# AnthonyDickson/HIVE

Measured on AMD Instinct MI355X. Metric: frames/sec (depth+TSDF integrate) @640x480, 512^3 vol, higher is better.
Workload: dtype bf16; 1 GPU; synthetic 640x480x150 RGB (seeded room trajectory), host-resident uint8 frames uploaded in the timed region, DPT-Hybrid depth (seeded random weights: depth 1-7 m, bf16, hip engine) + 512x512x512 TSDF integrate, 107 frames/step; frames_total=4066, volume=512x512x512, tsdf_overlap=True, scaling_mode=weak

## Files before the change

### hive_amd/_lib.py

```python
import atexit
import ctypes
import os
import sys
import threading

import numpy as np

_HERE = os.path.dirname(os.path.abspath(__file__))
LIB_PATH = os.environ.get("HIVE_AMD_LIB") or os.path.join(_HERE, "lib", "libhive_mi355x.so")

OK, ERR_INVALID, ERR_DEVICE, ERR_NOMEM, ERR_EMPTY, ERR_STATE = 0, -1, -2, -3, -4, -5
MEM_HOST, MEM_DEVICE = 0, 1
ROUND_HALF_EVEN, ROUND_HALF_AWAY = 0, 1
F32, F16, BF16 = 0, 1, 2
ABI_VERSION = 2

c_void_p, c_int, c_int64, c_float, c_double = ctypes.c_void_p, ctypes.c_int, ctypes.c_int64, ctypes.c_float, ctypes.c_double
P = ctypes.POINTER

SIGNATURES = {
    "hive_abi_version": (c_int, []),
    "hive_ctx_create": (c_int, [c_int, c_void_p, P(c_void_p)]),
    "hive_ctx_destroy": (c_int, [c_void_p]),
    "hive_ctx_get_stream": (c_int, [c_void_p, P(c_void_p)]),
# ... 40 lines not shown
    "hive_view_frustum": (c_int, [c_void_p, c_void_p, c_int, c_int, c_void_p, c_void_p, c_int, c_void_p]),
    "hive_view_frustum_batch": (c_int, [c_void_p, c_void_p, c_int, c_int, c_int, c_void_p, c_void_p, c_int, c_void_p]),
    "hive_depth_apply_mask": (c_int, [c_void_p, c_void_p, c_void_p, c_int, c_int, c_int, c_int, c_int, c_int, c_void_p]),
    "hive_depth_mm_to_m": (c_int, [c_void_p, c_void_p, c_int64, c_float, c_float, c_void_p]),
    "hive_unproject": (c_int, [c_void_p, c_void_p, c_void_p, c_void_p, c_int, c_int, c_void_p, c_void_p, c_void_p, c_int,
                               c_void_p, c_void_p, c_int64, P(c_int64)]),
    "hive_image2world": (c_int, [c_void_p, c_void_p, c_void_p, c_int64, c_void_p, c_void_p, c_void_p, c_double, c_int, c_void_p]),
    "hive_project": (c_int, [c_void_p, c_void_p, c_int64, c_void_p, c_void_p, c_void_p, c_double, c_int, c_void_p, c_void_p,
                             c_void_p]),
    "hive_project_bbox": (c_int, [c_void_p, c_void_p, c_int64, c_void_p, c_void_p, c_void_p, c_int, c_int, c_int, c_void_p]),
    "hive_grid_mesh": (c_int, [c_void_p, c_void_p, c_void_p, c_int, c_int, c_double, c_double, c_int, c_void_p, c_int64, P(c_int64), P(c_int64)]),
    "hive_fg_frame_mesh": (c_int, [c_void_p, c_void_p, c_void_p, c_int, c_int, c_void_p, c_void_p, c_void_p, c_void_p, c_double, c_double, c_void_p, c_int64, c_void_p, c_int64,
                                   c_void_p, P(c_int64), P(c_int64), c_void_p]),
    "hive_mesh_cleanup_cc": (c_int, [c_void_p, c_void_p, c_int64, c_int64, c_int, c_double, c_int, c_void_p, c_void_p, P(c_int64), P(c_int64)]),
    "hive_fg_frame_mesh_cc": (c_int, [c_void_p, c_void_p, c_void_p, c_int, c_int, c_void_p, c_void_p, c_void_p, c_void_p, c_double, c_double, c_int, c_double, c_void_p,
                                      c_int64, c_void_p, c_int64, c_void_p, P(c_int64), P(c_int64), c_void_p, c_void_p]),
    "hive_mesh_decimate": (c_int, [c_void_p, c_void_p, c_int64, c_void_p, c_int64, c_int64, c_double, c_int, c_void_p, c_void_p, P(c_int64), P(c_int64), c_void_p]),
    "hive_fg_frame_mesh_dec": (c_int, [c_void_p, c_void_p, c_void_p, c_int, c_int, c_void_p, c_void_p, c_void_p, c_void_p, c_double, c_double, c_int64, c_double, c_int,
                                       c_int, c_double, c_void_p, c_int64, c_void_p, c_int64, c_void_p, P(c_int64), P(c_int64), c_void_p, c_void_p, c_void_p, c_void_p]),
    "hive_filter_faces": (c_int, [c_void_p, c_void_p, c_void_p, c_int64, c_void_p, c_int64, c_double, c_double, c_int, c_void_p, P(c_int64)]),
    "hive_texture_window": (c_int, [c_void_p, c_void_p, c_int64, c_void_p, c_void_p, c_void_p, c_double, c_int, c_void_p, c_void_p]),
    "hive_fg_billboard": (c_int, [c_void_p, c_void_p, c_int64, c_void_p, c_void_p, P(c_double)]),
    "hive_fg_centroids": (c_int, [c_void_p, c_void_p, c_void_p, c_int, c_int, c_int, c_void_p, c_void_p, c_void_p]),
    "hive_fts_optimise": (c_int, [c_void_p, c_void_p, c_void_p, c_void_p, c_int, c_void_p, c_void_p, c_int, c_double, c_int, c_void_p, c_void_p]),
    "hive_dilate_mask": (c_int, [c_void_p, c_void_p, c_int, c_int, c_int, c_int, c_void_p]),
    "hive_dilate_mask_se": (c_int, [c_void_p, c_void_p, c_int, c_int, c_void_p, c_int, c_int, c_int, c_int, c_void_p]),
    "hive_inpaint_telea": (c_int, [c_void_p, c_void_p, c_int, c_int, c_int, c_int, c_void_p, c_int, c_int, c_void_p]),
    "hive_inpaint_frames": (c_int, [c_void_p, c_void_p, c_void_p, c_void_p, c_int, c_int, c_int, c_int, c_int, c_int, c_int, c_void_p, c_void_p, c_void_p]),
    "hive_depth_apply_mask_se": (c_int, [c_void_p, c_void_p, c_void_p, c_int, c_int, c_int, c_void_p, c_int, c_int, c_int, c_int, c_int, c_void_p]),
    "hive_vit_create": (c_int, [c_void_p, c_int, c_int, c_int, c_int, c_int, c_float, c_void_p, P(c_void_p)]),
    "hive_vit_weights_modified": (c_int, [c_void_p]),
    "hive_vit_destroy": (c_int, [c_void_p]),
    "hive_vit_forward": (c_int, [c_void_p, c_void_p, c_int, c_int, c_void_p, c_int, c_void_p]),
    "hive_vit_layernorm": (c_int, [c_void_p, c_void_p, c_int, c_void_p, c_void_p, c_void_p, c_int, c_int, c_float]),
    "hive_vit_linear": (c_int, [c_void_p, c_void_p, c_int, c_void_p, c_void_p, c_void_p, c_void_p, c_int, c_int, c_int, c_int]),
    "hive_vit_qkv": (c_int, [c_void_p, c_void_p, c_int, c_void_p, c_void_p, c_void_p, c_void_p, c_int, c_int, c_int, c_int]),
    "hive_vit_attention": (c_int, [c_void_p, c_void_p, c_int, c_void_p, c_void_p, c_int, c_int, c_int, c_int, c_int]),
    "hive_dpt_preprocess": (c_int, [c_void_p, c_void_p, c_int64, c_float, c_float, c_int, c_void_p]),
    "hive_dpt_head_tail": (c_int, [c_void_p, c_void_p, c_int, c_int64, c_int, c_void_p, c_int, c_void_p, c_float, c_int, c_int, c_float,
                                   c_float, c_void_p, c_float, c_float, c_void_p, c_void_p]),
    "hive_dpt_head_fused": (c_int, [c_void_p, c_void_p, c_void_p, c_int, c_int, c_int, c_int, c_int, c_int, c_void_p, c_void_p, c_void_p, c_float,
                                    c_int, c_int, c_float, c_float, c_void_p, c_float, c_float, c_void_p, c_void_p]),
    "hive_nhwc_group_norm": (c_int, [c_void_p, c_void_p, c_int, c_int, c_int, c_int, c_int, c_void_p, c_void_p, c_float, c_void_p, c_int,
                                     c_void_p]),
    "hive_nhwc_bias_act": (c_int, [c_void_p, c_void_p, c_int, c_int64, c_int, c_void_p, c_int, c_void_p, c_void_p, c_void_p, c_void_p]),
    "hive_nhwc_upsample2x": (c_int, [c_void_p, c_void_p, c_void_p, c_int, c_int, c_int, c_int, c_int, c_void_p]),
    "hive_nhwc_conv3x3": (c_int, [c_void_p, c_void_p, c_int, c_int, c_int, c_int, c_int, c_int, c_void_p, c_void_p, c_int, c_void_p, c_void_p,
                                  c_void_p, c_void_p]),
    "hive_nhwc_conv": (c_int, [c_void_p, c_void_p, c_int, c_int, c_int, c_int, c_int, c_int, c_int, c_int, c_int, c_int, c_int, c_int, c_void_p, c_void_p,
                               c_int, c_void_p, c_void_p, c_void_p, c_void_p]),
    "hive_nhwc_conv_gn_partial_floats": (c_int64, [c_int64, c_int]),
    "hive_nhwc_conv_gn": (c_int, [c_void_p, c_void_p, c_int, c_int, c_int, c_int, c_int, c_int, c_int, c_int, c_int, c_int, c_int, c_int, c_void_p, c_void_p,
                                  c_int, c_void_p, c_void_p, c_void_p, c_void_p, c_void_p, c_int64, P(c_int)]),
    "hive_nhwc_conv_gn_apply": (c_int, [c_void_p, c_void_p, c_int, c_int, c_int, c_int, c_int, c_int, c_int, c_int, c_int, c_int, c_int, c_int, c_void_p, c_int,
                                        c_void_p, c_void_p, c_float, c_void_p, c_int, c_void_p, c_void_p, c_int64, P(c_int)]),
    "hive_nhwc_group_norm_stats": (c_int, [c_void_p, c_void_p, c_int, c_int, c_int, c_int, c_int, c_void_p, c_void_p, c_float, c_void_p, c_int,
                                           c_void_p, c_void_p, c_int]),
    "hive_gn_gram_table_floats": (c_int64, [c_int, c_int]),
    "hive_gn_gram_prepare": (c_int, [c_void_p, c_void_p, c_int, c_int, c_int, c_int, c_void_p]),
    "hive_gn_gram_parts": (c_int, [c_void_p, c_int, c_int, c_int, c_int]),
    "hive_gn_gram_stats": (c_int, [c_void_p, c_void_p, c_int, c_int, c_int, c_int, c_int, c_int, c_int, c_int, c_int, c_int, c_void_p, c_float, c_void_p, c_void_p,
                                   c_void_p]),
    "hive_nhwc_conv_gn_apply_gram": (c_int, [c_void_p, c_void_p, c_int, c_int, c_int, c_int, c_int, c_int, c_int, c_int, c_int, c_void_p, c_void_p, c_int, c_void_p,
                                             c_void_p, c_float, c_void_p, c_int, c_void_p, c_void_p, c_int64, P(c_int)]),
    "hive_patch_rows": (c_int, [c_void_p, c_void_p, c_int, c_int, c_int, c_int, c_int, c_int, c_void_p]),
    "hive_nhwc_pixel_shuffle_bias": (c_int, [c_void_p, c_void_p, c_void_p, c_int, c_int, c_int, c_int, c_int, c_int, c_void_p]),
    "hive_resnet_stem_conv": (c_int, [c_void_p, c_void_p, c_int, c_int, c_int, c_int, c_void_p, c_void_p]),
    "hive_nhwc_maxpool3x3s2": (c_int, [c_void_p, c_void_p, c_int, c_int, c_int, c_int, c_int, c_void_p]),
    "hive_bneck_gn_conv3x3": (c_int, [c_void_p, c_void_p, c_int, c_int, c_int, c_int, c_int, c_void_p, c_int, c_void_p, c_void_p, c_float, c_void_p, c_void_p, c_void_p,
                                      c_int64, P(c_int), P(c_int)]),
    "hive_resnet_stem_conv_gn": (c_int, [c_void_p, c_void_p, c_int, c_int, c_int, c_int, c_void_p, c_void_p, c_void_p, c_int64, P(c_int)]),
    "hive_nhwc_group_norm_relu_maxpool": (c_int, [c_void_p, c_void_p, c_int, c_int, c_int, c_int, c_int, c_int, c_void_p, c_void_p, c_float, c_void_p, c_void_p,
                                                  c_int]),
    "hive_dpt_create": (c_int, [c_void_p, c_void_p, c_void_p, c_int, P(c_void_p)]),
    "hive_dpt_forward": (c_int, [c_void_p, c_void_p, c_int, c_int, c_int, c_void_p, c_void_p, c_float, c_void_p, c_void_p]),
    "hive_dpt_forward_frames": (c_int, [c_void_p, c_void_p, c_int, c_int, c_int, c_int, c_int, c_void_p, c_void_p, c_float, c_void_p, c_void_p]),
    "hive_dpt_resize_preprocess": (c_int, [c_void_p, c_void_p, c_int, c_int, c_int, c_int, c_int, c_float, c_float, c_int, c_void_p]),
    "hive_depth_resize_nearest": (c_int, [c_void_p, c_void_p, c_int, c_int, c_int, c_int, c_int, c_float, c_float, c_void_p, c_void_p, c_void_p]),
    "hive_dpt_arena_bytes": (c_int, [c_void_p, P(c_int64)]),
    "hive_dpt_weights_modified": (c_int, [c_void_p]),
    "hive_dpt_destroy": (c_int, [c_void_p]),
    "hive_depth_quantize": (c_int, [c_void_p, c_void_p, c_int, c_int, c_int, c_float, c_float, c_void_p, c_void_p, c_void_p]),
}

_lib = None
_lock = threading.Lock()
_shutdown = False


@atexit.register
def _mark_shutdown():
    global _shutdown
    _shutdown = True


def alive():
    return not _shutdown and not sys.is_finalizing()


class HiveError(RuntimeError):
    def __init__(self, code, message):
        super().__init__(f"libhive_mi355x error {code}: {message}")
        self.code = code


def load():
    global _lib
    with _lock:
        if _lib is not None:
            return _lib
        if not os.path.exists(LIB_PATH):
            raise ImportError(
                f"{LIB_PATH} is missing: build it with `python -c 'import __graft_entry__ as g; g.build()'` or "
                f"`make -C hive_amd/csrc`. hive_amd has no CPU fallback.")
        try:
            import torch
        except ImportError:
            pass
        lib = ctypes.CDLL(LIB_PATH, mode=ctypes.RTLD_GLOBAL)
        for name, (restype, argtypes) in SIGNATURES.items():
            fn = getattr(lib, name)
            fn.restype = restype
            fn.argtypes = argtypes
        if lib.hive_abi_version() != ABI_VERSION:
# ... 132 lines not shown
```

### hive_amd/csrc/bneck.hip

```cpp
#include "hive_internal.hpp"

#include <algorithm>

#include "mfma_pipe.hpp"

using hive_mfma::f32x4;
using hive_mfma::vec;

namespace {

constexpr int BN_TH = 16, BN_TW = 32;
constexpr int BN_PH = BN_TH + 2, BN_PW = BN_TW + 2;
constexpr int BN_K = 9 * 64;
constexpr int BN_WP = BN_K + 16;
constexpr int BN_CHUNKS = BN_PH * BN_PW * 8;
constexpr int BN_LOADS = (BN_CHUNKS + 511) / 512;
constexpr int BN_PATCH_BYTES = BN_PH * BN_PW * 128, BN_W_BYTES = 64 * BN_WP * 2, BN_SUM_BYTES = 8 * 2 * 64 * 4;
constexpr int BN_LDS = BN_PATCH_BYTES + BN_W_BYTES + BN_SUM_BYTES;

template <typename T>
struct BneckParams {
    const T *x;
    const float *stats;
    const T *gamma, *beta;
    const T *w;
    T *out;
    float *gn_partial;
    int H, W, tiles_x, tiles_y, n_tiles;
};

__device__ __forceinline__ int bn_swz(int q, int c) { return q * 128 + ((c ^ (q & 6)) << 4); }

__device__ __forceinline__ float bn_dot2(vec<__bf16, 2> a, vec<__bf16, 2> b, float c) { return __builtin_amdgcn_fdot2_f32_bf16(a, b, c, false); }
__device__ __forceinline__ float bn_dot2(vec<_Float16, 2> a, vec<_Float16, 2> b, float c) { return __builtin_amdgcn_fdot2(a, b, c, false); }
using hive_mfma::dpp_row_total;

template <typename T>
__global__ __launch_bounds__(512, 2) void bneck_conv3x3_kernel(BneckParams<T> p) {
    extern __shared__ __attribute__((aligned(16))) unsigned char lds[];
    unsigned char *patch = lds;
    T *wl = reinterpret_cast<T *>(lds + BN_PATCH_BYTES);
    float(*wsum)[2][64] = reinterpret_cast<float(*)[2][64]>(lds + BN_PATCH_BYTES + BN_W_BYTES);
    for (int i = threadIdx.x; i < 64 * (BN_K / 8); i += 512) {
        const int row = i / (BN_K / 8), c8 = i - row * (BN_K / 8);
        const int nt = row >> 4, f4 = (row >> 2) & 3, e = row & 3;
        const int ch = (nt >> 1) * 32 + f4 * 8 + (nt & 1) * 4 + e;
        *reinterpret_cast<uint4 *>(wl + row * BN_WP + c8 * 8) = reinterpret_cast<const uint4 *>(p.w)[ch * (BN_K / 8) + c8];
    }
    const int per_img = p.tiles_x * p.tiles_y;
    const int my_c = threadIdx.x & 7;
    float gam[8], bet[8];
    {
        const vec<T, 8> gv = *reinterpret_cast<const vec<T, 8> *>(p.gamma + my_c * 8), bv = *reinterpret_cast<const vec<T, 8> *>(p.beta + my_c * 8);
#pragma unroll
        for (int e = 0; e < 8; ++e) gam[e] = (float)gv[e], bet[e] = (float)bv[e];
    }
    uint4 regs[BN_LOADS];
    auto tile_origin = [&](int tile, int &img, int &oy0, int &ox0) {
        img = tile / per_img;
        const int t = tile - img * per_img;
        oy0 = (t / p.tiles_x) * BN_TH;
        ox0 = (t % p.tiles_x) * BN_TW;
    };
    auto fetch = [&](int tile) {
        int tid = threadIdx.x;
        asm volatile("" : "+v"(tid));
        int img, oy0, ox0;
        tile_origin(tile, img, oy0, ox0);
        const T *src = p.x + (size_t)img * p.H * p.W * 64;
#pragma unroll
        for (int k = 0; k < BN_LOADS; ++k) {
            const int i = tid + 512 * k, q = i >> 3, pr = q / BN_PW, pc = q - pr * BN_PW;
            const int gy = oy0 - 1 + pr, gx = ox0 - 1 + pc;
            regs[k] = make_uint4(0u, 0u, 0u, 0u);
            if (i < BN_CHUNKS && (unsigned)gy < (unsigned)p.H && (unsigned)gx < (unsigned)p.W)
                regs[k] = *reinterpret_cast<const uint4 *>(src + ((size_t)gy * p.W + gx) * 64 + (i & 7) * 8);
        }
    };
    int tile = blockIdx.x;
    if (tile < p.n_tiles) fetch(tile);
    for (; tile < p.n_tiles; tile += gridDim.x) {
// ... 49 lines not shown
#pragma unroll
                    for (int nt = 0; nt < 4; ++nt) acc[nt][mt] = hive_mfma::mfma16(wf[nt], af[mt], acc[nt][mt]);
            }
        }
        T *out = p.out + (size_t)img * p.H * p.W * 64;
#pragma unroll
        for (int mt = 0; mt < 4; ++mt) {
            const int oy = oy0 + 2 * wave + (mt >> 1), ox = ox0 + 16 * (mt & 1) + fr;
            if (oy < p.H && ox < p.W) {
#pragma unroll
                for (int h = 0; h < 2; ++h) {
                    vec<T, 8> ov;
#pragma unroll
                    for (int j = 0; j < 4; ++j) ov[j] = (T)acc[2 * h][mt][j], ov[4 + j] = (T)acc[2 * h + 1][mt][j];
                    *reinterpret_cast<vec<T, 8> *>(out + ((size_t)oy * p.W + ox) * 64 + h * 32 + fq * 8) = ov;
                }
            }
        }
        if (p.gn_partial) {
            vec<T, 2> ones, zero2;
            ones[0] = ones[1] = (T)1.0f;
            zero2[0] = zero2[1] = (T)0.0f;
            const bool row_ok[2] = {oy0 + 2 * wave < p.H, oy0 + 2 * wave + 1 < p.H};
#pragma unroll
            for (int nt = 0; nt < 4; ++nt) {
                f32x4 sv = f32x4{0.f, 0.f, 0.f, 0.f}, qv = sv;
#pragma unroll
                for (int r = 0; r < 2; ++r)
#pragma unroll
                    for (int e = 0; e < 4; ++e) {
                        vec<T, 2> y;
                        y[0] = (T)acc[nt][2 * r][e], y[1] = (T)acc[nt][2 * r + 1][e];
                        if (!row_ok[r]) y = zero2;
                        sv[e] = bn_dot2(y, ones, sv[e]);
                        qv[e] = bn_dot2(y, y, qv[e]);
                    }
#pragma unroll
                for (int e = 0; e < 4; ++e) {
                    sv[e] = dpp_row_total(sv[e]);
                    qv[e] = dpp_row_total(qv[e]);
                }
                if (fr == 0) {
                    const int ch = (nt >> 1) * 32 + fq * 8 + (nt & 1) * 4;
                    *reinterpret_cast<f32x4 *>(&wsum[wave][0][ch]) = sv;
                    *reinterpret_cast<f32x4 *>(&wsum[wave][1][ch]) = qv;
                }
            }
            __syncthreads();
            if (tix < 128) {
                const int which = tix >> 6, c = tix & 63;
                float s = 0.f;
#pragma unroll
                for (int w = 0; w < 8; ++w) s += wsum[w][which][c];
                p.gn_partial[((size_t)tile * 4 + which) * 64 + c] = s;
                p.gn_partial[((size_t)tile * 4 + 2 + which) * 64 + c] = 0.f;
            }
        }
    }
}

template <typename T>
int launch_bneck(hive_ctx *ctx, const void *d_x, int N, int H, int W, const float *stats, const void *gamma, const void *beta, const void *d_w, void *d_out,
                 float *d_gn_partial, long long gn_partial_floats, int *gn_tile_rows) {
    static hive_device_latch latch;
    if (!latch.done(ctx)) {
        HIVE_CHECK_HIP(ctx, hipFuncSetAttribute((const void *)bneck_conv3x3_kernel<T>, hipFuncAttributeMaxDynamicSharedMemorySize, BN_LDS));
        latch.mark(ctx);
    }
    BneckParams<T> p{};
    p.x = (const T *)d_x;
    p.stats = stats;
    p.gamma = (const T *)gamma;
    p.beta = (const T *)beta;
    p.w = (const T *)d_w;
    p.out = (T *)d_out;
    p.H = H;
    p.W = W;
    p.tiles_x = (W + BN_TW - 1) / BN_TW;
    p.tiles_y = (H + BN_TH - 1) / BN_TH;
    const long long tiles = (long long)N * p.tiles_x * p.tiles_y;
    HIVE_REQUIRE(ctx, tiles < (1ll << 31), "bneck_conv3x3: %lld tiles", tiles);
    p.n_tiles = (int)tiles;
    const int per_img = p.tiles_x * p.tiles_y;
    if (d_gn_partial && gn_tile_rows && W % BN_TW == 0 && (H * W) % per_img == 0 && tiles * 4 * 64 <= gn_partial_floats) {
        p.gn_partial = d_gn_partial;
        *gn_tile_rows = H * W / per_img;
    }
    const unsigned grid = (unsigned)std::min<long long>(tiles, (long long)ctx->num_cus);
    hipLaunchKernelGGL(bneck_conv3x3_kernel<T>, dim3(grid), dim3(512), BN_LDS, ctx->stream, p);
    HIVE_CHECK_HIP(ctx, hipGetLastError());
    return HIVE_OK;
}

}

extern "C" int hive_bneck_gn_conv3x3(hive_ctx *ctx, const void *d_x, int dtype, int N, int H, int W, int C, const void *d_in_partial, int in_tile_rows,
                                     const void *d_gamma, const void *d_beta, float eps, const void *d_w, void *d_out, void *d_gn_partial,
                                     int64_t gn_partial_floats, int *gn_tile_rows, int *fused) {
    HIVE_ENTER(ctx);
    if (!ctx) return hive_fail(nullptr, HIVE_ERR_INVALID, "ctx is NULL");
    HIVE_REQUIRE(ctx, d_x && d_gamma && d_beta && d_w && d_out && fused && d_out != d_x, "bneck_gn_conv3x3: bad pointers");
    HIVE_REQUIRE(ctx, dtype == HIVE_BF16 || dtype == HIVE_F16, "bneck_gn_conv3x3: dtype must be HIVE_F16 or HIVE_BF16");
    HIVE_REQUIRE(ctx, N > 0 && H > 0 && W > 0 && (long long)N * H * W < (1ll << 31), "bneck_gn_conv3x3: bad sizes %d x %d x %d", N, H, W);
    *fused = 0;
    if (gn_tile_rows) *gn_tile_rows = 0;
    if (C != 64 || !d_in_partial || in_tile_rows <= 0 || in_tile_rows > H * W) return HIVE_OK;
    int rc = hive_reserve_device(ctx, &ctx->d_scratch, &ctx->scratch_bytes, (size_t)N * 32 * 2 * sizeof(float));
    if (rc) return rc;
    float *stats = (float *)ctx->d_scratch;
    if ((rc = hive_gn_finalize_tiles(ctx, (const float *)d_in_partial, N, H * W, 64, 32, in_tile_rows, eps, stats))) return rc;
    rc = dtype == HIVE_BF16 ? launch_bneck<__bf16>(ctx, d_x, N, H, W, stats, d_gamma, d_beta, d_w, d_out, (float *)d_gn_partial, gn_partial_floats, gn_tile_rows)
                            : launch_bneck<_Float16>(ctx, d_x, N, H, W, stats, d_gamma, d_beta, d_w, d_out, (float *)d_gn_partial, gn_partial_floats, gn_tile_rows);
    if (rc) return rc;
    *fused = 1;
    return HIVE_OK;
}
```

### hive_amd/csrc/capi.hip

```cpp
#include <algorithm>

#include "hive_internal.hpp"

static thread_local std::string g_global_error;

void hive_set_global_error(const char *msg) { g_global_error = msg ? msg : ""; }

int hive_fail(hive_ctx *ctx, int code, const char *fmt, ...) {
    char buf[1024];
    va_list ap;
    va_start(ap, fmt);
    vsnprintf(buf, sizeof(buf), fmt, ap);
    va_end(ap);
    if (ctx)
        ctx->last_error = buf;
    else
        g_global_error = buf;
    return code;
}

int hive_reserve_device(hive_ctx *ctx, void **ptr, size_t *cur, size_t bytes) {
    if (*cur >= bytes && *ptr) return HIVE_OK;
    if (*ptr) {
        HIVE_CHECK_HIP(ctx, hipStreamSynchronize(ctx->stream));
        HIVE_CHECK_HIP(ctx, hipFree(*ptr));
        *ptr = nullptr;
        *cur = 0;
    }
    HIVE_CHECK_HIP(ctx, hipMalloc(ptr, bytes));
    *cur = bytes;
    return HIVE_OK;
}

int hive_splitk_workspace(hive_ctx *ctx, size_t bytes, void **ws, unsigned **count) {
    if (!ctx->d_splitk_count) {
        HIVE_CHECK_HIP(ctx, hipMalloc((void **)&ctx->d_splitk_count, HIVE_SPLITK_TILES * sizeof(unsigned)));
        HIVE_CHECK_HIP(ctx, hipMemsetAsync(ctx->d_splitk_count, 0, HIVE_SPLITK_TILES * sizeof(unsigned), ctx->stream));
    }
    int rc = hive_reserve_device(ctx, &ctx->d_splitk, &ctx->splitk_bytes, std::max(bytes, (size_t)32 << 20));
    if (rc) return rc;
    *ws = ctx->d_splitk;
    *count = ctx->d_splitk_count;
    return HIVE_OK;
}

int hive_upload(hive_ctx *ctx, void *dst, const void *src, size_t bytes) {
    hive_staging_slot &s = ctx->slots[ctx->next_slot];
    ctx->next_slot = (ctx->next_slot + 1) % hive_ctx::kSlots;
    if (s.in_flight) {
        HIVE_CHECK_HIP(ctx, hipEventSynchronize(s.done));
        s.in_flight = false;
    }
    if (s.bytes < bytes) {
        if (s.pinned) HIVE_CHECK_HIP(ctx, hipHostFree(s.pinned));
        s.pinned = nullptr;
        s.bytes = 0;
        HIVE_CHECK_HIP(ctx, hipHostMalloc(&s.pinned, bytes, hipHostMallocDefault));
        s.bytes = bytes;
    }
    if (!s.done) HIVE_CHECK_HIP(ctx, hipEventCreateWithFlags(&s.done, hipEventDisableTiming));
    memcpy(s.pinned, src, bytes);
    HIVE_CHECK_HIP(ctx, hipMemcpyAsync(dst, s.pinned, bytes, hipMemcpyHostToDevice, ctx->stream));
    HIVE_CHECK_HIP(ctx, hipEventRecord(s.done, ctx->stream));
    s.in_flight = true;
    return HIVE_OK;
}

static int next_event(hive_ctx *ctx, hipEvent_t *ev) {
    if (ctx->ev_used == ctx->ev_pool.size()) {
        hipEvent_t e;
        HIVE_CHECK_HIP(ctx, hipEventCreate(&e));
        ctx->ev_pool.push_back(e);
    }
    *ev = ctx->ev_pool[ctx->ev_used++];
    return HIVE_OK;
}

int hive_time_begin(hive_ctx *ctx) {
    if (!ctx->timing) return HIVE_OK;
    int rc = next_event(ctx, &ctx->last_start);
    if (rc) return rc;
    HIVE_CHECK_HIP(ctx, hipEventRecord(ctx->last_start, ctx->stream));
    return HIVE_OK;
}

int hive_time_end(hive_ctx *ctx) {
    if (!ctx->timing) return HIVE_OK;
    int rc = next_event(ctx, &ctx->last_stop);
    if (rc) return rc;
    HIVE_CHECK_HIP(ctx, hipEventRecord(ctx->last_stop, ctx->stream));
    return HIVE_OK;
}

extern "C" {

// ... 15 lines not shown
    if (e != hipSuccess) return hive_fail(nullptr, HIVE_ERR_DEVICE, "hipGetDeviceProperties: %s", hipGetErrorString(e));
    if (strncmp(prop.gcnArchName, "gfx950", 6) != 0)
        return hive_fail(nullptr, HIVE_ERR_DEVICE, "hive_ctx_create: device %d is %s; this library is built for gfx950 only",
                         device_id, prop.gcnArchName);
    hive_ctx *ctx = new hive_ctx();
    ctx->device = device_id;
    ctx->num_cus = prop.multiProcessorCount > 0 ? prop.multiProcessorCount : 256;
    HIVE_ENTER(ctx);
    int current = -1;
    e = hipGetDevice(&current);
    if (e == hipSuccess && current != device_id) e = hipErrorInvalidDevice;
    if (e == hipSuccess) {
        if (stream == HIVE_STREAM_OWN) {
            e = hipStreamCreateWithFlags(&ctx->stream, hipStreamNonBlocking);
            ctx->owns_stream = true;
        } else if (stream == HIVE_STREAM_OWN_LOW) {
            int least = 0, greatest = 0;
            e = hipDeviceGetStreamPriorityRange(&least, &greatest);
            if (e == hipSuccess) e = hipStreamCreateWithPriority(&ctx->stream, hipStreamNonBlocking, least);
            ctx->owns_stream = true;
        } else {
            ctx->stream = (hipStream_t)stream;
        }
    }
    if (e == hipSuccess) e = hipMalloc((void **)&ctx->d_scalars, 4096 * sizeof(unsigned));
    if (e == hipSuccess) e = hipMemset(ctx->d_scalars, 0, 4096 * sizeof(unsigned));
    if (e == hipSuccess) e = hipMalloc(&ctx->d_zeros, 256);
    if (e == hipSuccess) e = hipMemset(ctx->d_zeros, 0, 256);
    if (e != hipSuccess) {
        int rc = hive_fail(nullptr, HIVE_ERR_DEVICE, "hive_ctx_create: %s", hipGetErrorString(e));
        delete ctx;
        return rc;
    }
    *out = ctx;
    return HIVE_OK;
}

int hive_ctx_destroy(hive_ctx *ctx) {
    if (!ctx) return HIVE_OK;
    {
        HIVE_ENTER(ctx);
        (void)hipStreamSynchronize(ctx->stream);
    for (auto &s : ctx->slots) {
        if (s.pinned) (void)hipHostFree(s.pinned);
        if (s.done) (void)hipEventDestroy(s.done);
    }
    for (auto ev : ctx->ev_pool) (void)hipEventDestroy(ev);
    if (ctx->d_scratch) (void)hipFree(ctx->d_scratch);
    if (ctx->d_frame) (void)hipFree(ctx->d_frame);
    if (ctx->d_batch) (void)hipFree(ctx->d_batch);
    if (ctx->d_gram) (void)hipFree(ctx->d_gram);
    if (ctx->d_splitk) (void)hipFree(ctx->d_splitk);
    if (ctx->d_splitk_count) (void)hipFree(ctx->d_splitk_count);
    if (ctx->d_in) (void)hipFree(ctx->d_in);
    if (ctx->d_scalars) (void)hipFree(ctx->d_scalars);
    if (ctx->h_pinned_small) (void)hipHostFree(ctx->h_pinned_small);
        if (ctx->d_zeros) (void)hipFree(ctx->d_zeros);
        if (ctx->owns_stream) (void)hipStreamDestroy(ctx->stream);
    }
    delete ctx;
    return HIVE_OK;
}

int hive_ctx_release_stream(hive_ctx *ctx) {
    if (!ctx) return hive_fail(nullptr, HIVE_ERR_INVALID, "ctx is NULL");
    ctx->owns_stream = false;
    return HIVE_OK;
}

int hive_ctx_set_stream(hive_ctx *ctx, void *stream) {
    HIVE_ENTER(ctx);
    if (!ctx) return hive_fail(nullptr, HIVE_ERR_INVALID, "ctx is NULL");
    HIVE_REQUIRE(ctx, stream != HIVE_STREAM_OWN && stream != HIVE_STREAM_OWN_LOW, "hive_ctx_set_stream: pass a hipStream_t (NULL = the default stream)");
    hipStream_t next = (hipStream_t)stream;
    if (next == ctx->stream) return HIVE_OK;
    hipEvent_t ev;
    HIVE_CHECK_HIP(ctx, hipEventCreateWithFlags(&ev, hipEventDisableTiming));
    hipError_t e = hipEventRecord(ev, ctx->stream);
    if (e == hipSuccess) e = hipStreamWaitEvent(next, ev, 0);
    (void)hipEventDestroy(ev);
    HIVE_CHECK_HIP(ctx, e);
    if (ctx->owns_stream) {
        (void)hipStreamSynchronize(ctx->stream);
        (void)hipStreamDestroy(ctx->stream);
        ctx->owns_stream = false;
    }
    ctx->stream = next;
    return HIVE_OK;
}

int hive_ctx_get_stream(hive_ctx *ctx, void **stream) {
    if (!ctx || !stream) return hive_fail(ctx, HIVE_ERR_INVALID, "hive_ctx_get_stream: NULL argument");
    *stream = (void *)ctx->stream;
    return HIVE_OK;
}

int hive_ctx_synchronize(hive_ctx *ctx) {
    HIVE_ENTER(ctx);
    if (!ctx) return hive_fail(nullptr, HIVE_ERR_INVALID, "ctx is NULL");
    HIVE_CHECK_HIP(ctx, hipStreamSynchronize(ctx->stream));
    return HIVE_OK;
}

const char *hive_last_error(hive_ctx *ctx) { return ctx ? ctx->last_error.c_str() : g_global_error.c_str(); }

int hive_ctx_set_round_mode(hive_ctx *ctx, int mode) {
// ... 59 lines not shown
```

### hive_amd/csrc/conv.hip

```cpp
#include "hive_internal.hpp"
#include "mfma_pipe.hpp"

#include <algorithm>

constexpr int HIVE_CONV_AHEAD = 4;
constexpr int HIVE_CONV_AHEAD_GN2 = 4;

using hive_mfma::f32x4;
using hive_mfma::vec;

namespace {

template <typename T>
struct ConvParams {
    const T *x;
    const T *w;
    const T *bias;
    const T *res1;
    const T *res2;
    T *out;
    T *out_relu;
    const T *zeros;
    int H, W, Cin, Cout, relu;
    int Ho, Wo;
    int S, taps;
    int stride, pad_t, pad_l;
    int M;
    float *gn_partial;
    int stats_only;
    const float *gn_stats;
    const T *gn_gamma, *gn_beta;
    int gn_G, gn_cpg;
    int split_k;
    hive_mfma::f32x4 *sk_ws;
    unsigned *sk_count;
};

__device__ __forceinline__ float gn_affine_exact(float x, float rstd, float gamma, float beta, float mean) {
#pragma clang fp contract(off)
    const float a = rstd * gamma;
    const float b = beta - mean * a;
    return x * a + b;
}

template <typename T, int MT, int GN, int NRES = 1>
__device__ __forceinline__ void conv_epilogue(const ConvParams<T> &p, f32x4 (&acc)[4][MT], int m_base, int n_base, unsigned char *stage, int lane,
                                              int boundary) {
    asm volatile("" : "+v"(lane));
    const int n = n_base + (lane & 7) * 8;
    float b[8] = {0.f, 0.f, 0.f, 0.f, 0.f, 0.f, 0.f, 0.f};
    if (p.bias) {
        const vec<T, 8> bv = *reinterpret_cast<const vec<T, 8> *>(p.bias + n);
#pragma unroll
        for (int j = 0; j < 8; ++j) b[j] = (float)bv[j];
    }
    float ggam[8], gbet[8], gmean[2] = {0.f, 0.f}, grstd[2] = {0.f, 0.f};
    if (GN == 2) {
        const vec<T, 8> gv = *reinterpret_cast<const vec<T, 8> *>(p.gn_gamma + n), bv = *reinterpret_cast<const vec<T, 8> *>(p.gn_beta + n);
#pragma unroll
        for (int j = 0; j < 8; ++j) ggam[j] = (float)gv[j], gbet[j] = (float)bv[j];
        const int hw = p.Ho * p.Wo, img0 = boundary / hw - 1, n_img = p.M / hw, g = n / p.gn_cpg;
        const float *st = p.gn_stats + ((size_t)img0 * p.gn_G + g) * 2;
        gmean[0] = st[0], grstd[0] = st[1];
        if (img0 + 1 < n_img) gmean[1] = st[2 * p.gn_G], grstd[1] = st[2 * p.gn_G + 1];
    }
    constexpr int AHEAD = GN == 2 ? HIVE_CONV_AHEAD_GN2 : (NRES == 2 ? HIVE_CONV_AHEAD / 2 : HIVE_CONV_AHEAD);
    vec<T, 8> rs1[AHEAD + 1][2], rs2[NRES == 2 ? AHEAD + 1 : 1][2];
    const int row_in_frag = lane >> 3;
    auto pre = [&](int mt, int j) {
        const int m = min(m_base + mt * 16 + 8 * j + row_in_frag, p.M - 1);
        const size_t off = (size_t)m * p.Cout + n;
        if (GN != 1 && p.res1) rs1[mt % (AHEAD + 1)][j] = *reinterpret_cast<const vec<T, 8> *>(p.res1 + off);
        if (GN == 0 && NRES == 2) rs2[mt % (AHEAD + 1)][j] = *reinterpret_cast<const vec<T, 8> *>(p.res2 + off);
    };
    hive_mfma::staged_rows<MT, AHEAD>(stage, acc, lane, pre, [&](int r, int, const f32x4 &lo, const f32x4 &hi, int mt, int jrow) {
        const int m = m_base + r;
        if (m >= p.M) return;
        const size_t o_off = (size_t)m * p.Cout + n;
        float o[8];
#pragma unroll
        for (int j = 0; j < 4; ++j) o[j] = lo[j] + b[j], o[4 + j] = hi[j] + b[4 + j];
        if (GN == 0 && p.res1) {
            const vec<T, 8> rs = rs1[mt % (AHEAD + 1)][jrow];
#pragma unroll
            for (int j = 0; j < 8; ++j) o[j] += (float)rs[j];
        }
        if (GN == 0 && NRES == 2) {
            const vec<T, 8> rs = rs2[mt % (AHEAD + 1)][jrow];
// ... 63 lines not shown
#pragma unroll
            for (int mt = 0; mt < MT; mt += 2) {
                const f32x4 a0 = acc[nt][mt] + bias, a1 = acc[nt][mt + 1] + bias;
#pragma unroll
                for (int e = 0; e < 4; ++e) {
                    vec<T, 2> y;
                    y[0] = (T)a0[e], y[1] = (T)a1[e];
                    ts[e] = dot2acc(y, ones, ts[e]);
                    tq[e] = dot2acc(y, y, tq[e]);
                }
            }
            const f32x4 zero4 = f32x4{0.f, 0.f, 0.f, 0.f};
            sv[0] = second ? zero4 : ts;
            sv[1] = second ? ts : zero4;
            qv[0] = second ? zero4 : tq;
            qv[1] = second ? tq : zero4;
        } else {
#pragma unroll
            for (int mt = 0; mt < MT; mt += 2) {
                const int m0 = m_base + mt * 16 + fr, m1 = m0 + 16;
                const bool v0 = m0 < p.M, v1 = m1 < p.M, s0 = m0 >= boundary, s1 = m1 >= boundary;
                const f32x4 a0 = acc[nt][mt] + bias, a1 = acc[nt][mt + 1] + bias;
#pragma unroll
                for (int e = 0; e < 4; ++e) {
                    vec<T, 2> y, z;
                    y[0] = (T)(v0 && !s0 ? a0[e] : 0.f), y[1] = (T)(v1 && !s1 ? a1[e] : 0.f);
                    z[0] = (T)(v0 && s0 ? a0[e] : 0.f), z[1] = (T)(v1 && s1 ? a1[e] : 0.f);
                    sv[0][e] = dot2acc(y, ones, sv[0][e]);
                    qv[0][e] = dot2acc(y, y, qv[0][e]);
                    sv[1][e] = dot2acc(z, ones, sv[1][e]);
                    qv[1][e] = dot2acc(z, z, qv[1][e]);
                }
            }
        }
#pragma unroll
        for (int h = 0; h < 2; ++h) {
            f32x4 st = f32x4{0.f, 0.f, 0.f, 0.f}, qt = f32x4{0.f, 0.f, 0.f, 0.f};
            if (h == 0 || m_end > boundary) {
#pragma unroll
                for (int e = 0; e < 4; ++e) {
                    st[e] = dpp_row_total(sv[h][e]);
                    qt[e] = dpp_row_total(qv[h][e]);
                }
            }
            if (fr == 0) {
                *reinterpret_cast<f32x4 *>(wsum + (h * 2 + 0) * 64 + nt * 16 + fq * 4) = st;
                *reinterpret_cast<f32x4 *>(wsum + (h * 2 + 1) * 64 + nt * 16 + fq * 4) = qt;
            }
        }
    }
}

constexpr int BK = 64;


template <typename T, int TM, int TN, int GN>
__global__ __launch_bounds__(512, 1) void conv_kernel(ConvParams<T> p) {
    extern __shared__ __attribute__((aligned(16))) unsigned char lds[];
    constexpr int A_GROUPS = TM / 8, A_PW = A_GROUPS / 8;
    constexpr int W_GROUPS = TN / 8, GROUPS = A_GROUPS + W_GROUPS, PER_WAVE = GROUPS / 8;
    constexpr int STAGE_BYTES = GROUPS * 1024;
    constexpr int WN = TN / 64, WM = 8 / WN, RW = TM / WM, MT = RW / 16;
    const int tid = threadIdx.x;
    int lane = tid & 63;
    const int wave = __builtin_amdgcn_readfirstlane(tid >> 6);
    const int wr = wave / WN, wc = wave % WN;
    const int tiles_n = p.Cout / TN, n_tiles = ((p.M + TM - 1) / TM) * tiles_n;
    int run0, run_n, per_xcd;
    hive_mfma::xcd_run(n_tiles, run0, run_n, per_xcd);
    int tl = blockIdx.x >> 3;
    if (tl >= run_n) return;
    const int K = p.taps * p.Cin, CPT = p.Cin / BK;

    struct Tile {
        int m0, n0;
        int py[A_PW], px[A_PW];
        const T *pbase[A_PW];
    };
    int a_chunk[A_PW];
    auto lane_constants = [&]() {
#pragma unroll
        for (int j = 0; j < A_PW; ++j) {
            const int row = (wave + 8 * j) * 8 + (lane >> 3);
            a_chunk[j] = ((lane & 7) ^ ((row >> 1) & 7)) * 8;
        }
    };
    lane_constants();
    auto setup = [&](int t, Tile &tile) {
        tile.m0 = (t / tiles_n) * TM;
        tile.n0 = (t % tiles_n) * TN;
#pragma unroll
        for (int j = 0; j < A_PW; ++j) {
            const int row = (wave + 8 * j) * 8 + (lane >> 3);
            const int m = min(tile.m0 + row, p.M - 1);
            const int img = m / (p.Ho * p.Wo), rem = m - img * (p.Ho * p.Wo);
            const int oy = rem / p.Wo, ox = rem - oy * p.Wo;
            tile.py[j] = oy * p.stride - p.pad_t;
            tile.px[j] = ox * p.stride - p.pad_l;
            tile.pbase[j] = p.x + (((long long)img * p.H + tile.py[j]) * p.W + tile.px[j]) * p.Cin + a_chunk[j];
        }
    };

    auto issue_piece = [&](const Tile &tile, int stage, int tap, int cc, int j) {
        unsigned char *st = lds + stage * STAGE_BYTES;
        if (j < A_PW) {
            const int dy = tap / p.S, dx = tap - dy * p.S;
// ... 14 lines not shown
    Tile tile;
    setup(run0 + tl, tile);
#pragma unroll
    for (int j = 0; j < PER_WAVE; ++j) issue_piece(tile, 0, 0, 0, j);
    int buf = 0;
    for (;;) {
        asm volatile("" : "+v"(lane));
        lane_constants();
        const int fr = lane & 15, fq = lane >> 4;
        const bool has_next = tl + per_xcd < run_n;
        const int em0 = tile.m0, en0 = tile.n0;
        f32x4 acc[4][MT];
#pragma unroll
        for (int i = 0; i < 4; ++i)
#pragma unroll
            for (int j = 0; j < MT; ++j) acc[i][j] = f32x4{0.f, 0.f, 0.f, 0.f};
        int nx_tap = 1, nx_cc = 0;
        if (nx_tap == p.taps) nx_tap = 0, nx_cc = 1;
        for (int kt = 0; kt < KT; ++kt) {
            asm volatile("s_waitcnt vmcnt(0)" ::: "memory");
            __builtin_amdgcn_s_barrier();
            int is_tap = nx_tap, is_cc = nx_cc;
            if (kt + 1 == KT) {
                if (has_next) {
                    setup(run0 + tl + per_xcd, tile);
                    is_tap = 0, is_cc = 0;
                } else {
                    is_tap = last_tap, is_cc = CPT - 1;
                }
            }
            if (++nx_tap == p.taps) nx_tap = 0, ++nx_cc;
            const unsigned char *a_t = lds + buf * STAGE_BYTES, *w_t = a_t + A_GROUPS * 1024;
            hive_mfma::kstep64<T, MT, false>(a_t, w_t, wr * RW, wc * 64, fr, fq, acc, PER_WAVE, [&](int j) { issue_piece(tile, buf ^ 1, is_tap, is_cc, j); });
            buf ^= 1;
        }
        unsigned char *stage = lds + 2 * STAGE_BYTES + wave * 4096;
        const int hw = p.Ho * p.Wo, boundary = (em0 / hw + 1) * hw;
        if (!(GN == 1 && p.stats_only)) {
            if (GN == 0 && p.res2)
                conv_epilogue<T, MT, GN, 2>(p, acc, em0 + wr * RW, en0 + wc * 64, stage, lane, boundary);
            else
                conv_epilogue<T, MT, GN, 1>(p, acc, em0 + wr * RW, en0 + wc * 64, stage, lane, boundary);
        }
        if (GN == 1) {
            __builtin_amdgcn_wave_barrier();
            gn_sums_from_acc<T, MT>(p, acc, em0 + wr * RW, en0 + wc * 64, lane, boundary, reinterpret_cast<float *>(stage));
            __syncthreads();
            const int tile_m = em0 / TM;
            for (int t = tid; t < 4 * TN; t += 512) {
                const int hq = t / TN, ch = t - hq * TN, cw = ch >> 6, c = ch & 63;
                float a = 0.f;
#pragma unroll
                for (int w = 0; w < WM; ++w) a += reinterpret_cast<const float *>(lds + 2 * STAGE_BYTES + (w * WN + cw) * 4096)[hq * 64 + c];
                p.gn_partial[((size_t)tile_m * 4 + hq) * p.Cout + en0 + ch] = a;
            }
        }
        if (!has_next) break;
        tl += per_xcd;
    }
    asm volatile("s_waitcnt vmcnt(0)" ::: "memory");
}

template <typename T, int TN, int GN, int NST>
__global__ __launch_bounds__(512, 1) void conv_deep_kernel(ConvParams<T> p) {
    extern __shared__ __attribute__((aligned(16))) unsigned char lds[];
    constexpr int TM = 128, AHEAD = NST - 1;
    constexpr int A_GROUPS = TM / 8, A_PW = A_GROUPS / 8;
    constexpr int W_GROUPS = TN / 8, GROUPS = A_GROUPS + W_GROUPS, PER_WAVE = GROUPS / 8;
    constexpr int STAGE_BYTES = GROUPS * 1024;
    constexpr int WN = TN / 64, WM = 8 / WN, RW = TM / WM, MT = RW / 16;
    static_assert(AHEAD * PER_WAVE < 64, "vmcnt is a 6-bit counter");
    const int tid = threadIdx.x;
    int lane = tid & 63;
    const int wave = __builtin_amdgcn_readfirstlane(tid >> 6);
    const int wr = wave / WN, wc = wave % WN;
    const int S = p.split_k, KT = p.taps * (p.Cin / BK);
    const int tiles_n = p.Cout / TN, n_items = ((p.M + TM - 1) / TM) * tiles_n * S;
    int run0, run_n, per_xcd;
    hive_mfma::xcd_run(n_items, run0, run_n, per_xcd);
    int tl = blockIdx.x >> 3;
    if (tl >= run_n) return;

    struct Tile {
        int m0, n0, kt, k1, tl;
        int py[A_PW], px[A_PW];
        const T *pbase[A_PW];
    };
    int a_chunk[A_PW];
    auto lane_constants = [&]() {
#pragma unroll
        for (int j = 0; j < A_PW; ++j) {
            const int row = (wave + 8 * j) * 8 + (lane >> 3);
            a_chunk[j] = ((lane & 7) ^ ((row >> 1) & 7)) * 8;
        }
    };
    lane_constants();
    auto coords = [&](int item, int &m0, int &n0, int &k0, int &k1) {
        const int t = item / S, s = item - t * S;
        m0 = (t / tiles_n) * TM;
        n0 = (t % tiles_n) * TN;
        k0 = s * KT / S;
        k1 = (s + 1) * KT / S;
    };
    auto setup = [&](Tile &tile) {
        coords(run0 + tile.tl, tile.m0, tile.n0, tile.kt, tile.k1);
#pragma unroll
        for (int j = 0; j < A_PW; ++j) {
            const int row = (wave + 8 * j) * 8 + (lane >> 3);
            const int m = min(tile.m0 + row, p.M - 1);
            const int img = m / (p.Ho * p.Wo), rem = m - img * (p.Ho * p.Wo);
            const int oy = rem / p.Wo, ox = rem - oy * p.Wo;
            tile.py[j] = oy * p.stride - p.pad_t;
            tile.px[j] = ox * p.stride - p.pad_l;
// ... 28 lines not shown
    Tile is;
    is.tl = tl;
    setup(is);
#pragma unroll
    for (int a = 0; a < AHEAD; ++a) {
#pragma unroll
        for (int j = 0; j < PER_WAVE; ++j) issue_piece(is, a, j);
        advance(is);
    }
    int buf = 0;
    for (;;) {
        asm volatile("" : "+v"(lane));
        lane_constants();
        const int fr = lane & 15, fq = lane >> 4;
        const bool has_next = tl + per_xcd < run_n;
        int em0, en0, k0, k1;
        coords(run0 + tl, em0, en0, k0, k1);
        f32x4 acc[4][MT];
#pragma unroll
        for (int i = 0; i < 4; ++i)
#pragma unroll
            for (int j = 0; j < MT; ++j) acc[i][j] = f32x4{0.f, 0.f, 0.f, 0.f};
        for (int kt = k0; kt < k1; ++kt) {
            asm volatile("s_waitcnt vmcnt(%0)" ::"n"((AHEAD - 1) * PER_WAVE) : "memory");
            __builtin_amdgcn_s_barrier();
            const int ib = buf + AHEAD >= NST ? buf + AHEAD - NST : buf + AHEAD;
            const unsigned char *a_t = lds + buf * STAGE_BYTES, *w_t = a_t + A_GROUPS * 1024;
            hive_mfma::kstep64<T, MT, false>(a_t, w_t, wr * RW, wc * 64, fr, fq, acc, PER_WAVE, [&](int j) { issue_piece(is, ib, j); });
            advance(is);
            buf = buf + 1 == NST ? 0 : buf + 1;
        }
        unsigned char *epi = lds + NST * STAGE_BYTES;
        bool store = true;
        if (S > 1) store = hive_mfma::splitk_combine<512>(S, p.sk_ws, p.sk_count, run0 + tl, acc, tid, reinterpret_cast<int *>(epi));
        if (store) {
            unsigned char *stage = epi + wave * 4096;
            const int hw = p.Ho * p.Wo, boundary = (em0 / hw + 1) * hw;
            if (!(GN == 1 && p.stats_only)) {
                if (GN == 0 && p.res2)
                    conv_epilogue<T, MT, GN, 2>(p, acc, em0 + wr * RW, en0 + wc * 64, stage, lane, boundary);
                else
                    conv_epilogue<T, MT, GN, 1>(p, acc, em0 + wr * RW, en0 + wc * 64, stage, lane, boundary);
            }
            if (GN == 1) {
                __builtin_amdgcn_wave_barrier();
                gn_sums_from_acc<T, MT>(p, acc, em0 + wr * RW, en0 + wc * 64, lane, boundary, reinterpret_cast<float *>(stage));
                __syncthreads();
                const int tile_m = em0 / TM;
                for (int t = tid; t < 4 * TN; t += 512) {
                    const int hq = t / TN, ch = t - hq * TN, cw = ch >> 6, c = ch & 63;
                    float a = 0.f;
#pragma unroll
                    for (int w = 0; w < WM; ++w) a += reinterpret_cast<const float *>(epi + (w * WN + cw) * 4096)[hq * 64 + c];
                    p.gn_partial[((size_t)tile_m * 4 + hq) * p.Cout + en0 + ch] = a;
                }
            }
        }
        if (!has_next) break;
        __builtin_amdgcn_s_waitcnt(0x0F70);
        __syncthreads();
        tl += per_xcd;
    }
    asm volatile("s_waitcnt vmcnt(0)" ::: "memory");
}

constexpr int conv_lds(int tm, int tn, int nst = 2) { return nst * (tm / 8 + tn / 8) * 1024 + hive_mfma::STAGED_ROWS_LDS; }

constexpr int CONV_DEEP_NST = 4;

template <typename T>
int ensure_conv_attrs(hive_ctx *ctx) {
    static hive_device_latch latch;
    if (latch.done(ctx)) return HIVE_OK;
#define HIVE_CONV_ATTR(TM_, TN_, GN_) \
    HIVE_CHECK_HIP(ctx, hipFuncSetAttribute((const void *)conv_kernel<T, TM_, TN_, GN_>, hipFuncAttributeMaxDynamicSharedMemorySize, conv_lds(TM_, TN_)))
    HIVE_CONV_ATTR(256, 256, 0);
    HIVE_CONV_ATTR(256, 256, 1);
    HIVE_CONV_ATTR(256, 128, 0);
    HIVE_CONV_ATTR(256, 128, 1);
    HIVE_CONV_ATTR(256, 64, 0);
    HIVE_CONV_ATTR(256, 64, 1);
    HIVE_CONV_ATTR(128, 256, 0);
    HIVE_CONV_ATTR(128, 256, 1);
    HIVE_CONV_ATTR(128, 128, 0);
    HIVE_CONV_ATTR(128, 128, 1);
    HIVE_CONV_ATTR(256, 256, 2);
    HIVE_CONV_ATTR(128, 256, 2);
#undef HIVE_CONV_ATTR
    HIVE_CHECK_HIP(ctx, hipFuncSetAttribute((const void *)conv_deep_kernel<T, 128, 0, CONV_DEEP_NST>, hipFuncAttributeMaxDynamicSharedMemorySize, conv_lds(128, 128, CONV_DEEP_NST)));
    HIVE_CHECK_HIP(ctx, hipFuncSetAttribute((const void *)conv_deep_kernel<T, 128, 1, CONV_DEEP_NST>, hipFuncAttributeMaxDynamicSharedMemorySize, conv_lds(128, 128, CONV_DEEP_NST)));
    latch.mark(ctx);
    return HIVE_OK;
}

struct GnMode {
    int stats_only = 0;
    const float *gn_stats = nullptr;
    const void *gn_gamma = nullptr, *gn_beta = nullptr;
    int gn_G = 0, gn_cpg = 0;
};

template <typename T>
int launch_conv_t(hive_ctx *ctx, const char *what, const void *d_x, int N, int H, int W, int C_in, int C_out, int R, int stride, int pad_t,
                  int pad_l, int Ho, int Wo, const void *d_w, const void *d_bias, int relu, const void *d_residual, const void *d_residual2,
                  void *d_out, void *d_out_relu, void *d_gn_partial, long long gn_partial_floats, int *gn_tile_rows, const GnMode *gn_mode) {
    HIVE_REQUIRE(ctx, d_x && d_w && d_out, "%s: NULL argument", what);
    if (gn_tile_rows) *gn_tile_rows = 0;
    HIVE_REQUIRE(ctx, N > 0 && H > 0 && W > 0 && Ho > 0 && Wo > 0 && (long long)N * H * W < (1ll << 31) && (long long)N * Ho * Wo < (1ll << 31),
                 "%s: bad sizes %d x %d x %d -> %d x %d", what, N, H, W, Ho, Wo);
    HIVE_REQUIRE(ctx, (R == 1 || R == 3) && (stride == 1 || stride == 2) && pad_t >= 0 && pad_t < R && pad_l >= 0 && pad_l < R,
                 "%s: kernel %d, stride %d, padding (%d, %d)", what, R, stride, pad_t, pad_l);
    HIVE_REQUIRE(ctx, (long long)(Ho - 1) * stride - pad_t < H && (long long)(Wo - 1) * stride - pad_l < W, "%s: output %d x %d reaches outside the %d x %d input", what, Ho,
                 Wo, H, W);
    HIVE_REQUIRE(ctx, C_in > 0 && C_in % 64 == 0 && C_out > 0 && C_out % 64 == 0, "%s: need C_in %% 64 == 0 and C_out %% 64 == 0, got %d -> %d", what, C_in, C_out);
    HIVE_REQUIRE(ctx, (R == 1 && stride == 1) || (d_out != d_x && d_out_relu != d_x), "%s: the output must not alias the input", what);
    ConvParams<T> p{};
    p.x = (const T *)d_x;
    p.w = (const T *)d_w;
    p.bias = (const T *)d_bias;
    p.res1 = (const T *)d_residual;
    p.res2 = (const T *)d_residual2;
    p.out = (T *)d_out;
    p.out_relu = (T *)d_out_relu;
    p.zeros = (const T *)ctx->d_zeros;
    p.H = H;
    p.W = W;
    p.Cin = C_in;
    p.Cout = C_out;
    p.relu = relu;
    p.Ho = Ho;
    p.Wo = Wo;
    p.S = R;
    p.taps = R * R;
    p.stride = stride;
    p.pad_t = pad_t;
    p.pad_l = pad_l;
    p.M = N * Ho * Wo;
    int rc = ensure_conv_attrs<T>(ctx);
    if (rc) return rc;
    const int tn = C_out % 256 == 0 ? 256 : (C_out % 128 == 0 ? 128 : 64);
    int tm = 256;
    if (tn >= 128) {
        const long long per = C_out / tn, t256 = (long long)((p.M + 255) / 256) * per, t128 = (long long)((p.M + 127) / 128) * per;
        const long long r256 = (t256 + ctx->num_cus - 1) / ctx->num_cus, r128 = (t128 + ctx->num_cus - 1) / ctx->num_cus;
        if (t256 < ctx->num_cus || r128 * 128 * 100 < r256 * 256 * 85) tm = 128;
    }
    if (gn_mode) {
        p.stats_only = gn_mode->stats_only;
        p.gn_stats = gn_mode->gn_stats;
        p.gn_gamma = (const T *)gn_mode->gn_gamma;
        p.gn_beta = (const T *)gn_mode->gn_beta;
        p.gn_G = gn_mode->gn_G;
        p.gn_cpg = gn_mode->gn_cpg;
    }
    if (d_gn_partial && gn_tile_rows && (long long)Ho * Wo >= tm && !relu && !d_residual && !d_residual2 && !d_out_relu) {
        HIVE_REQUIRE(ctx, (long long)((p.M + tm - 1) / tm) * 4 * C_out <= gn_partial_floats, "%s: gn_partial holds %lld floats, %lld needed", what,
                     gn_partial_floats, (long long)((p.M + tm - 1) / tm) * 4 * C_out);
        p.gn_partial = (float *)d_gn_partial;
        *gn_tile_rows = tm;
    }
    {
        const long long tiles128 = (long long)((p.M + 127) / 128) * (C_out / 128);
        const char *deep_env = getenv("HIVE_CONV_DEEP");
        const bool allowed = !(deep_env && deep_env[0] == '0');
        if (allowed && !p.gn_stats && C_out % 128 == 0 && tiles128 <= ctx->num_cus && tiles128 <= HIVE_SPLITK_TILES) {
            const int KT = p.taps * (C_in / BK);
            const char *sk_env = getenv("HIVE_SPLITK");
            p.split_k = sk_env ? std::max(1, std::min(atoi(sk_env), KT)) : hive_mfma::splitk_ways(tiles128, KT, ctx->num_cus);
            p.split_k = (int)std::max<long long>(1, std::min<long long>(p.split_k, ctx->num_cus / tiles128));
            if (ctx->deterministic) p.split_k = 1;
            ++ctx->n_deep_ring_launches;
            if (p.split_k > 1) {
                ++ctx->n_splitk_launches;
                void *ws = nullptr;
                rc = hive_splitk_workspace(ctx, (size_t)tiles128 * p.split_k * 128 * 128 * sizeof(float), &ws, &p.sk_count);
                if (rc) return rc;
                p.sk_ws = reinterpret_cast<hive_mfma::f32x4 *>(ws);
            }
            const bool stats = d_gn_partial && gn_tile_rows && (long long)Ho * Wo >= 128 && !relu && !d_residual && !d_residual2 && !d_out_relu;
            if (stats) {
                HIVE_REQUIRE(ctx, (long long)((p.M + 127) / 128) * 4 * C_out <= gn_partial_floats, "%s: gn_partial holds %lld floats, %lld needed", what,
                             gn_partial_floats, (long long)((p.M + 127) / 128) * 4 * C_out);
                p.gn_partial = (float *)d_gn_partial;
                *gn_tile_rows = 128;
            }
            const long long items = tiles128 * p.split_k;
            const dim3 dgrid((unsigned)std::min<long long>((items + 7) / 8 * 8, (long long)ctx->num_cus / 8 * 8));
            if (stats)
                hipLaunchKernelGGL((conv_deep_kernel<T, 128, 1, CONV_DEEP_NST>), dgrid, dim3(512), (size_t)conv_lds(128, 128, CONV_DEEP_NST), ctx->stream, p);
            else
                hipLaunchKernelGGL((conv_deep_kernel<T, 128, 0, CONV_DEEP_NST>), dgrid, dim3(512), (size_t)conv_lds(128, 128, CONV_DEEP_NST), ctx->stream, p);
            HIVE_CHECK_HIP(ctx, hipGetLastError());
            return HIVE_OK;
        }
    }
    const long long tiles = (long long)((p.M + tm - 1) / tm) * (C_out / tn);
    const dim3 grid((unsigned)std::min<long long>((tiles + 7) / 8 * 8, (long long)ctx->num_cus / 8 * 8));
    const size_t lds = (size_t)conv_lds(tm, tn);
#define HIVE_CONV_LAUNCH(TM_, TN_)                                                                                   \
    do {                                                                                                             \
        if (p.gn_partial)                                                                                            \
            hipLaunchKernelGGL((conv_kernel<T, TM_, TN_, 1>), grid, dim3(512), lds, ctx->stream, p);                    \
        else                                                                                                         \
            hipLaunchKernelGGL((conv_kernel<T, TM_, TN_, 0>), grid, dim3(512), lds, ctx->stream, p);                    \
    } while (0)
    if (p.gn_stats) {
        if (tm == 256)
            hipLaunchKernelGGL((conv_kernel<T, 256, 256, 2>), grid, dim3(512), lds, ctx->stream, p);
        else
            hipLaunchKernelGGL((conv_kernel<T, 128, 256, 2>), grid, dim3(512), lds, ctx->stream, p);
    } else if (tm == 256 && tn == 256)
        HIVE_CONV_LAUNCH(256, 256);
    else if (tm == 256 && tn == 128)
        HIVE_CONV_LAUNCH(256, 128);
    else if (tm == 256)
        HIVE_CONV_LAUNCH(256, 64);
    else if (tn == 256)
        HIVE_CONV_LAUNCH(128, 256);
    else
        HIVE_CONV_LAUNCH(128, 128);
#undef HIVE_CONV_LAUNCH
    HIVE_CHECK_HIP(ctx, hipGetLastError());
    return HIVE_OK;
}

int launch_conv(hive_ctx *ctx, const char *what, const void *d_x, int dtype, int N, int H, int W, int C_in, int C_out, int R, int stride, int pad_t,
                int pad_l, int Ho, int Wo, const void *d_w, const void *d_bias, int relu, const void *d_residual, const void *d_residual2,
                void *d_out, void *d_out_relu, void *d_gn_partial = nullptr, long long gn_partial_floats = 0, int *gn_tile_rows = nullptr,
                const GnMode *gn_mode = nullptr) {
    if (dtype == HIVE_BF16)
        return launch_conv_t<__bf16>(ctx, what, d_x, N, H, W, C_in, C_out, R, stride, pad_t, pad_l, Ho, Wo, d_w, d_bias, relu, d_residual, d_residual2, d_out, d_out_relu,
                                     d_gn_partial, gn_partial_floats, gn_tile_rows, gn_mode);
    if (dtype == HIVE_F16)
        return launch_conv_t<_Float16>(ctx, what, d_x, N, H, W, C_in, C_out, R, stride, pad_t, pad_l, Ho, Wo, d_w, d_bias, relu, d_residual, d_residual2, d_out,
                                       d_out_relu, d_gn_partial, gn_partial_floats, gn_tile_rows, gn_mode);
    if (gn_tile_rows) *gn_tile_rows = 0;
    return hive_fail(ctx, HIVE_ERR_INVALID, "%s: dtype must be HIVE_F16 or HIVE_BF16", what);
}

}

extern "C" int hive_nhwc_conv3x3(hive_ctx *ctx, const void *d_x, int dtype, int N, int H, int W, int C_in, int C_out, const void *d_w,
                                 const void *d_bias, int relu, const void *d_residual, const void *d_residual2, void *d_out,
                                 void *d_out_relu) {
    HIVE_ENTER(ctx);
    if (!ctx) return hive_fail(nullptr, HIVE_ERR_INVALID, "ctx is NULL");
    HIVE_REQUIRE(ctx, C_out % 128 == 0, "nhwc_conv3x3: need C_out %% 128 == 0, got %d", C_out);
    HIVE_REQUIRE(ctx, d_out != d_x && d_out_relu != d_x, "nhwc_conv3x3: the output must not alias the input (3 x 3 halo)");
    return launch_conv(ctx, "nhwc_conv3x3", d_x, dtype, N, H, W, C_in, C_out, 3, 1, 1, 1, H, W, d_w, d_bias, relu, d_residual, d_residual2, d_out, d_out_relu);
}

extern "C" int64_t hive_nhwc_conv_gn_partial_floats(int64_t n_px, int C_out) { return (n_px / 128 + 1) * 4 * (int64_t)C_out; }

extern "C" int hive_nhwc_conv_gn(hive_ctx *ctx, const void *d_x, int dtype, int N, int H, int W, int C_in, int C_out, int kernel, int stride, int pad_top,
                                 int pad_left, int H_out, int W_out, const void *d_w, const void *d_bias, int relu, const void *d_residual,
                                 const void *d_residual2, void *d_out, void *d_out_relu, void *d_gn_partial, int64_t gn_partial_floats, int *gn_tile_rows) {
    HIVE_ENTER(ctx);
    if (!ctx) return hive_fail(nullptr, HIVE_ERR_INVALID, "ctx is NULL");
    HIVE_REQUIRE(ctx, d_gn_partial && gn_tile_rows, "nhwc_conv_gn: NULL argument");
    return launch_conv(ctx, "nhwc_conv_gn", d_x, dtype, N, H, W, C_in, C_out, kernel, stride, pad_top, pad_left, H_out, W_out, d_w, d_bias, relu, d_residual,
                       d_residual2, d_out, d_out_relu, d_gn_partial, gn_partial_floats, gn_tile_rows);
}

extern "C" int hive_nhwc_conv_gn_apply(hive_ctx *ctx, const void *d_x, int dtype, int N, int H, int W, int C_in, int C_out, int kernel, int stride,
                                       int pad_top, int pad_left, int H_out, int W_out, const void *d_w, int G, const void *d_gamma, const void *d_beta,
                                       float eps, const void *d_residual, int relu, void *d_out, void *d_scratch, int64_t scratch_floats, int *fused) {
    HIVE_ENTER(ctx);
    if (!ctx) return hive_fail(nullptr, HIVE_ERR_INVALID, "ctx is NULL");
    HIVE_REQUIRE(ctx, d_gamma && d_beta && d_scratch && fused, "nhwc_conv_gn_apply: NULL argument");
    *fused = 0;
    const long long hw = (long long)H_out * W_out;
    if (G <= 0 || C_out % 256 != 0 || C_out % G != 0 || (C_out / G) % 8 != 0 || hw < 256) return HIVE_OK;
    const int64_t partial_floats = hive_nhwc_conv_gn_partial_floats((int64_t)N * hw, C_out);
    HIVE_REQUIRE(ctx, scratch_floats >= partial_floats + 2ll * N * G, "nhwc_conv_gn_apply: scratch holds %lld floats, %lld needed", (long long)scratch_floats,
                 (long long)(partial_floats + 2ll * N * G));
    float *partial = (float *)d_scratch, *stats = partial + partial_floats;
    GnMode mode;
    mode.stats_only = 1;
    int tile_rows = 0;
    int rc = launch_conv(ctx, "nhwc_conv_gn_apply", d_x, dtype, N, H, W, C_in, C_out, kernel, stride, pad_top, pad_left, H_out, W_out, d_w, nullptr, 0, nullptr,
                         nullptr, d_out, nullptr, partial, partial_floats, &tile_rows, &mode);
    if (rc) return rc;
    HIVE_REQUIRE(ctx, tile_rows > 0, "nhwc_conv_gn_apply: no statistics from a %lld-pixel map", hw);
    rc = hive_gn_finalize_tiles(ctx, partial, N, (int)hw, C_out, G, tile_rows, eps, stats);
    if (rc) return rc;
    mode.stats_only = 0;
    mode.gn_stats = stats;
    mode.gn_gamma = d_gamma;
    mode.gn_beta = d_beta;
    mode.gn_G = G;
    mode.gn_cpg = C_out / G;
    rc = launch_conv(ctx, "nhwc_conv_gn_apply", d_x, dtype, N, H, W, C_in, C_out, kernel, stride, pad_top, pad_left, H_out, W_out, d_w, nullptr, relu, d_residual,
                     nullptr, d_out, nullptr, nullptr, 0, nullptr, &mode);
    if (rc) return rc;
    *fused = 1;
    return HIVE_OK;
}

extern "C" int hive_nhwc_conv_gn_apply_gram(hive_ctx *ctx, const void *d_x, int dtype, int N, int H, int W, int C_in, int C_out, int stride, int H_out, int W_out,
                                            const void *d_w, const float *d_tables, int G, const void *d_gamma, const void *d_beta, float eps, const void *d_residual,
                                            int relu, void *d_out, void *d_scratch, int64_t scratch_floats, int *fused) {
    HIVE_ENTER(ctx);
    if (!ctx) return hive_fail(nullptr, HIVE_ERR_INVALID, "ctx is NULL");
    HIVE_REQUIRE(ctx, d_gamma && d_beta && d_scratch && d_tables && fused, "nhwc_conv_gn_apply_gram: NULL argument");
    *fused = 0;
    const long long hw = (long long)H_out * W_out;
    if (G < 4 || 256 % G != 0 || G > 64 || C_out % 256 != 0 || C_out % G != 0 || (C_out / G) % 8 != 0 || hw < 256 || !(C_in == 64 || C_in == 128 || C_in == 256)) return HIVE_OK;
    HIVE_REQUIRE(ctx, scratch_floats >= 2ll * N * G, "nhwc_conv_gn_apply_gram: scratch holds %lld floats, %lld needed", (long long)scratch_floats, 2ll * N * G);
    HIVE_REQUIRE(ctx, (long long)(H_out - 1) * stride < H && (long long)(W_out - 1) * stride < W, "nhwc_conv_gn_apply_gram: output %d x %d reaches outside the %d x %d input", H_out,
                 W_out, H, W);
    float *stats = (float *)d_scratch;
    int rc = hive_gram_gn_stats(ctx, d_x, dtype, N, H, W, C_in, C_out, stride, H_out, W_out, G, d_tables, eps, stats, nullptr, nullptr);
    if (rc) return rc;
    GnMode mode;
    mode.gn_stats = stats;
    mode.gn_gamma = d_gamma;
    mode.gn_beta = d_beta;
    mode.gn_G = G;
    mode.gn_cpg = C_out / G;
    rc = launch_conv(ctx, "nhwc_conv_gn_apply_gram", d_x, dtype, N, H, W, C_in, C_out, 1, stride, 0, 0, H_out, W_out, d_w, nullptr, relu, d_residual, nullptr, d_out, nullptr,
                     nullptr, 0, nullptr, &mode);
    if (rc) return rc;
    *fused = 1;
    return HIVE_OK;
}

extern "C" int hive_nhwc_conv(hive_ctx *ctx, const void *d_x, int dtype, int N, int H, int W, int C_in, int C_out, int kernel, int stride, int pad_top,
                              int pad_left, int H_out, int W_out, const void *d_w, const void *d_bias, int relu, const void *d_residual,
                              const void *d_residual2, void *d_out, void *d_out_relu) {
    HIVE_ENTER(ctx);
    if (!ctx) return hive_fail(nullptr, HIVE_ERR_INVALID, "ctx is NULL");
    return launch_conv(ctx, "nhwc_conv", d_x, dtype, N, H, W, C_in, C_out, kernel, stride, pad_top, pad_left, H_out, W_out, d_w, d_bias, relu, d_residual,
                       d_residual2, d_out, d_out_relu);
}
```

### hive_amd/csrc/dpt_net.hip

```cpp
#include "hive_internal.hpp"

#include <algorithm>
#include <map>
#include <string>
#include <vector>

typedef unsigned short half_t;

namespace {

template <typename T>
__global__ __launch_bounds__(256) void assemble_tokens_kernel(const T *__restrict__ patch, const T *__restrict__ cls, const T *__restrict__ pos,
                                                              T *__restrict__ tokens, int B, int n_patch, int D) {
    const int dv = D / 8;
    const long long total = (long long)B * (n_patch + 1) * dv;
    for (long long i = (long long)blockIdx.x * 256 + threadIdx.x; i < total; i += (long long)gridDim.x * 256) {
        const int c = (int)(i % dv) * 8;
        const long long row = i / dv;
        const int t = (int)(row % (n_patch + 1)), b = (int)(row / (n_patch + 1));
        const T *src = t == 0 ? cls + c : patch + ((size_t)b * n_patch + (t - 1)) * D + c;
        const uint4 ra = *reinterpret_cast<const uint4 *>(src), rp = *reinterpret_cast<const uint4 *>(pos + (size_t)t * D + c);
        const T *a = reinterpret_cast<const T *>(&ra), *p = reinterpret_cast<const T *>(&rp);
        T o[8];
#pragma unroll
// ... 96 lines not shown

namespace {

struct Map {
    half_t *p;
    int H, W, C;
    float *gn = nullptr;
    int gn_tm = 0;
};

#define DPT_TRY(expr)              \
    do {                           \
        int _rc = (expr);          \
        if (_rc) return _rc;       \
    } while (0)

int run_forward(hive_dpt *d, bool dry, const uint8_t *d_rgb, int B, int FH, int FW, int H, int W, const void *d_pos, float *d_depth, float max_depth,
                uint16_t *d_mm, float *d_m) {
    hive_ctx *ctx = d->ctx;
    const bool resized = FH != H || FW != W;
    auto preprocess = [&](half_t *xin) -> int {
        if (resized) return hive_dpt_resize_preprocess(ctx, d_rgb, B, FH, FW, H, W, 0.5f, 0.5f, d->cfg.dtype, xin);
        return hive_dpt_preprocess(ctx, d_rgb, (int64_t)B * H * W * 3, 0.5f, 0.5f, d->cfg.dtype, xin);
    };
    const int dt = d->cfg.dtype;
    const std::string bb = "pretrained.model.patch_embed.backbone.";
    auto need = [&](const std::string &n, const void **out) -> int {
        *out = d->get(n);
        if (!*out) return hive_fail(ctx, HIVE_ERR_INVALID, "hive_dpt: tensor '%s' missing from the table", n.c_str());
        return HIVE_OK;
    };
    auto same_out = [](int i, int s) { return (i + s - 1) / s; };
    auto drop = [&](Map &m) {
        d->release(m.p);
        d->release(m.gn);
        m.p = nullptr;
        m.gn = nullptr;
    };
    auto conv = [&](const Map &x, const std::string &wname, const char *bias_name, int cout, int k, int stride, bool same_pad, int relu, const half_t *res1,
                    const half_t *res2, bool want_relu_copy, Map *out, Map *out_relu, bool gn_stats = false) -> int {
        int pt, pl, oh, ow;
        if (same_pad) {
            oh = same_out(x.H, stride);
            ow = same_out(x.W, stride);
            pt = std::max((oh - 1) * stride + k - x.H, 0) / 2;
            pl = std::max((ow - 1) * stride + k - x.W, 0) / 2;
        } else {
            pt = pl = k / 2;
            oh = (x.H + 2 * pt - k) / stride + 1;
            ow = (x.W + 2 * pl - k) / stride + 1;
        }
        *out = Map{d->alloc((size_t)B * oh * ow * cout), oh, ow, cout};
        if (out_relu) *out_relu = Map{want_relu_copy ? d->alloc((size_t)B * oh * ow * cout) : nullptr, oh, ow, cout};
        const int64_t gn_floats = gn_stats ? hive_nhwc_conv_gn_partial_floats((int64_t)B * oh * ow, cout) : 0;
        if (gn_stats) out->gn = (float *)d->alloc((size_t)gn_floats * 2);
        if (dry) return HIVE_OK;
        const void *wp, *bp = nullptr;
        DPT_TRY(need(wname, &wp));
        if (bias_name) DPT_TRY(need(bias_name, &bp));
        if (gn_stats)
            return hive_nhwc_conv_gn(ctx, x.p, dt, B, x.H, x.W, x.C, cout, k, stride, pt, pl, oh, ow, wp, bp, relu, res1, res2, out->p,
                                     out_relu ? out_relu->p : nullptr, out->gn, gn_floats, &out->gn_tm);
        return hive_nhwc_conv(ctx, x.p, dt, B, x.H, x.W, x.C, cout, k, stride, pt, pl, oh, ow, wp, bp, relu, res1, res2, out->p,
                              out_relu ? out_relu->p : nullptr);
    };
    auto conv_norm = [&](const Map &x, const std::string &wname, const std::string &norm_prefix, int cout, int stride, const half_t *residual, int relu,
                         Map *out) -> int {
        const int oh = same_out(x.H, stride), ow = same_out(x.W, stride);
        const int64_t scratch_floats = hive_nhwc_conv_gn_partial_floats((int64_t)B * oh * ow, cout) + 2ll * B * 32;
        float *scratch = (float *)d->alloc((size_t)scratch_floats * 2);
        *out = Map{d->alloc((size_t)B * oh * ow * cout), oh, ow, cout};
        const bool eligible = cout % 256 == 0 && (cout / 32) % 8 == 0 && (long long)oh * ow >= 256;
        Map t{eligible ? nullptr : d->alloc((size_t)B * oh * ow * cout), oh, ow, cout};
        auto done = [&](int rc) {
            d->release(scratch);
            d->release(t.p);
            return rc;
        };
        if (dry) return done(HIVE_OK);
        const void *wp, *g, *b;
        DPT_TRY(need(wname, &wp));
        DPT_TRY(need(norm_prefix + ".weight", &g));
        DPT_TRY(need(norm_prefix + ".bias", &b));
        int fused = 0;
        const char *gram_env = getenv("HIVE_GN_GRAM");
        const long long out_elems = (long long)B * oh * ow * cout;
        const bool gram = !(gram_env && gram_env[0] == '0') && !ctx->deterministic && eligible &&
                          (((x.C == 64 || x.C == 128) && out_elems >= 150000000ll) || (x.C == 256 && stride == 2 && out_elems >= 250000000ll));
        if (gram) {
            float *&tables = d->gram_tables[wname];
            if (!tables) {
                HIVE_CHECK_HIP(ctx, hipMalloc((void **)&tables, (size_t)hive_gn_gram_table_floats(x.C, 32) * sizeof(float)));
                DPT_TRY(hive_gn_gram_prepare(ctx, wp, dt, x.C, cout, 32, tables));
            }
            DPT_TRY(hive_nhwc_conv_gn_apply_gram(ctx, x.p, dt, B, x.H, x.W, x.C, cout, stride, oh, ow, wp, tables, 32, g, b, d->cfg.gn_eps, residual, relu, out->p, scratch,
                                                 scratch_floats, &fused));
            if (fused) return done(HIVE_OK);
        }
        DPT_TRY(hive_nhwc_conv_gn_apply(ctx, x.p, dt, B, x.H, x.W, x.C, cout, 1, stride, 0, 0, oh, ow, wp, 32, g, b, d->cfg.gn_eps, residual, relu, out->p,
                                        scratch, scratch_floats, &fused));
        if (fused) return done(HIVE_OK);
        if (eligible) return hive_fail(ctx, HIVE_ERR_INVALID, "hive_dpt: conv + GroupNorm of '%s' was not fused", wname.c_str());
        DPT_TRY(hive_nhwc_conv_gn(ctx, x.p, dt, B, x.H, x.W, x.C, cout, 1, stride, 0, 0, oh, ow, wp, nullptr, 0, nullptr, nullptr, t.p, nullptr, scratch,
                                  scratch_floats, &t.gn_tm));
        return done(hive_nhwc_group_norm_stats(ctx, t.p, dt, B, oh * ow, cout, 32, g, b, d->cfg.gn_eps, residual, relu, out->p, scratch, t.gn_tm));
    };
    auto group_norm = [&](const Map &x, const std::string &prefix, const half_t *residual, int relu, Map *out) -> int {
        *out = Map{d->alloc((size_t)B * x.H * x.W * x.C), x.H, x.W, x.C};
        if (dry) return HIVE_OK;
        const void *g, *b;
        DPT_TRY(need(prefix + ".weight", &g));
        DPT_TRY(need(prefix + ".bias", &b));
        return hive_nhwc_group_norm_stats(ctx, x.p, dt, B, x.H * x.W, x.C, 32, g, b, d->cfg.gn_eps, residual, relu, out->p, x.gn, x.gn_tm);
    };

    Map layer_1, layer_2, layer_3, layer_4;
    auto hybrid_backbone = [&]() -> int {
        half_t *xin = d->alloc((size_t)B * H * W * 3);
        Map s0{d->alloc((size_t)B * same_out(H, 2) * same_out(W, 2) * 64), same_out(H, 2), same_out(W, 2), 64};
        const int64_t stem_floats = hive_nhwc_conv_gn_partial_floats((int64_t)B * s0.H * s0.W, 64);
        s0.gn = (float *)d->alloc((size_t)stem_floats * 2);
        if (!dry) {
            DPT_TRY(preprocess(xin));
            const void *sw;
            DPT_TRY(need(bb + "stem.conv.weight", &sw));
            DPT_TRY(hive_resnet_stem_conv_gn(ctx, xin, dt, B, H, W, sw, s0.p, s0.gn, stem_floats, &s0.gn_tm));
        }
        d->release(xin);
        Map feat{d->alloc((size_t)B * same_out(s0.H, 2) * same_out(s0.W, 2) * 64), same_out(s0.H, 2), same_out(s0.W, 2), 64};
        if (!dry) {
            const void *g, *b;
            DPT_TRY(need(bb + "stem.norm.weight", &g));
            DPT_TRY(need(bb + "stem.norm.bias", &b));
            DPT_TRY(hive_nhwc_group_norm_relu_maxpool(ctx, s0.p, dt, B, s0.H, s0.W, 64, 32, g, b, d->cfg.gn_eps, feat.p, s0.gn_tm ? s0.gn : nullptr, s0.gn_tm));
        }
        drop(s0);
        const int depths[3] = {3, 4, 9}, chans[3] = {256, 512, 1024};
        Map hook[2] = {Map{nullptr, 0, 0, 0}, Map{nullptr, 0, 0, 0}};
        for (int s = 0; s < 3; ++s) {
            for (int blk = 0; blk < depths[s]; ++blk) {
                const std::string pre = bb + "stages." + std::to_string(s) + ".blocks." + std::to_string(blk) + ".";
                const int cout = chans[s], mid = cout / 4, stride = (blk == 0 && s > 0) ? 2 : 1;
                Map in = feat, shortcut = feat, t, u, t2, u2;
                if (blk == 0) DPT_TRY(conv_norm(in, pre + "downsample.conv.weight", pre + "downsample.norm", cout, stride, nullptr, 0, &shortcut));
                DPT_TRY(conv(in, pre + "conv1.weight", nullptr, mid, 1, 1, true, 0, nullptr, nullptr, false, &t, nullptr, true));
                int bneck = 0;
                if (mid == 64 && stride == 1 && (long long)t.H * t.W >= 256) {
                    t2 = Map{d->alloc((size_t)B * t.H * t.W * 64), t.H, t.W, 64};
                    const int64_t floats = hive_nhwc_conv_gn_partial_floats((int64_t)B * t.H * t.W, 64);
                    t2.gn = (float *)d->alloc((size_t)floats * 2);
                    if (dry) {
                        bneck = 1;
                    } else {
                        const void *g, *b, *w2;
                        DPT_TRY(need(pre + "norm1.weight", &g));
                        DPT_TRY(need(pre + "norm1.bias", &b));
                        DPT_TRY(need(pre + "conv2.weight", &w2));
                        DPT_TRY(hive_bneck_gn_conv3x3(ctx, t.p, dt, B, t.H, t.W, 64, t.gn, t.gn_tm, g, b, d->cfg.gn_eps, w2, t2.p, t2.gn, floats, &t2.gn_tm, &bneck));
                        if (!bneck) return hive_fail(ctx, HIVE_ERR_INVALID, "hive_dpt: the 64-channel bottleneck convolution of '%s' was not fused", pre.c_str());
                    }
                    drop(t);
                }
                if (!bneck) {
                    DPT_TRY(group_norm(t, pre + "norm1", nullptr, 1, &u));
                    drop(t);
                    DPT_TRY(conv(u, pre + "conv2.weight", nullptr, mid, 3, stride, true, 0, nullptr, nullptr, false, &t2, nullptr, true));
                    drop(u);
                }
                DPT_TRY(group_norm(t2, pre + "norm2", nullptr, 1, &u2));
                drop(t2);
                DPT_TRY(conv_norm(u2, pre + "conv3.weight", pre + "norm3", cout, 1, shortcut.p, 1, &feat));
                drop(u2);
                if (blk == 0) drop(shortcut);
                if (in.p != hook[0].p && in.p != hook[1].p) drop(in);
            }
            if (s < 2) hook[s] = feat;
        }
        layer_1 = hook[0];
        layer_2 = hook[1];

        const int gh = feat.H, gw = feat.W, n_patch = gh * gw, N = n_patch + 1, D = 768;
        Map pe;
        DPT_TRY(conv(feat, "pretrained.model.patch_embed.proj.weight", "pretrained.model.patch_embed.proj.bias", D, 1, 1, false, 0, nullptr, nullptr, false, &pe,
                     nullptr));
        half_t *tokens = d->alloc((size_t)B * N * D), *tap3 = d->alloc((size_t)B * N * D), *tap4 = d->alloc((size_t)B * N * D);
        half_t *cat = d->alloc((size_t)B * n_patch * 2 * D);
        Map map3{d->alloc((size_t)B * n_patch * D), gh, gw, D}, map4{d->alloc((size_t)B * n_patch * D), gh, gw, D};
        if (!dry) {
            const void *cls;
            DPT_TRY(need("pretrained.model.cls_token", &cls));
            const int blocks = (int)std::min<long long>(((long long)B * N * D / 8 + 255) / 256, (long long)ctx->num_cus * 16);
            launch_assemble_tokens(ctx, dt, blocks, pe.p, cls, d_pos, tokens, B, n_patch, D);
            HIVE_CHECK_HIP(ctx, hipGetLastError());
            const int taps[2] = {8, 11};
            void *tap_out[2] = {tap3, tap4};
            DPT_TRY(hive_vit_forward(d->vit, tokens, B, N, taps, 2, tap_out));
            const half_t *tap[2] = {tap3, tap4};
            Map *maps[2] = {&map3, &map4};
            for (int r = 0; r < 2; ++r) {
                hipLaunchKernelGGL(readout_concat_kernel, dim3(blocks), dim3(256), 0, ctx->stream, tap[r], cat, B, n_patch, D);
                HIVE_CHECK_HIP(ctx, hipGetLastError());
                const std::string pre = std::string("pretrained.act_postprocess") + (r == 0 ? "3" : "4") + ".0.project.0.";
// ... 253 lines not shown
```

### hive_amd/csrc/dpt_ops.hip

```cpp
#include "hive_internal.hpp"

#include <algorithm>
#include <cstdlib>

typedef __bf16 bf16;

template <typename T>
struct Vec8 {
    T v[8];
};

template <typename T>
__device__ __forceinline__ void load8(const T *p, float (&f)[8]) {
    const uint4 raw = *reinterpret_cast<const uint4 *>(p);
    const T *t = reinterpret_cast<const T *>(&raw);
#pragma unroll
    for (int j = 0; j < 8; ++j) f[j] = (float)t[j];
}

template <typename T>
__device__ __forceinline__ void store8(T *p, const float (&f)[8]) {
    Vec8<T> o;
#pragma unroll
    for (int j = 0; j < 8; ++j) o.v[j] = (T)f[j];
    *reinterpret_cast<uint4 *>(p) = *reinterpret_cast<const uint4 *>(&o);
}
template <typename T>
__device__ __forceinline__ void store8_nt(T *p, const float (&f)[8]) {
    Vec8<T> o;
#pragma unroll
    for (int j = 0; j < 8; ++j) o.v[j] = (T)f[j];
    typedef unsigned u4 __attribute__((ext_vector_type(4)));
    __builtin_nontemporal_store(*reinterpret_cast<const u4 *>(&o), reinterpret_cast<u4 *>(p));
}

template <typename T>
__global__ __launch_bounds__(256) void gn_partial_kernel(const T *__restrict__ x, int HW, int C, int slabs, float *__restrict__ partial) {
    __shared__ float red[256 * 16];
    const int VC = C >> 3, PP = 256 / VC;
    const int n = blockIdx.y, slab = blockIdx.x;
    const int v = threadIdx.x % VC, pp = threadIdx.x / VC;
    const int per = (HW + slabs - 1) / slabs;
    const int p0 = slab * per, p1 = min(p0 + per, HW);
    float s[8] = {0, 0, 0, 0, 0, 0, 0, 0}, q[8] = {0, 0, 0, 0, 0, 0, 0, 0};
    const T *base = x + (size_t)n * HW * C + v * 8;
    int p = p0 + pp;
    for (; p + 3 * PP < p1; p += 4 * PP) {
        float f[4][8];
#pragma unroll
        for (int u = 0; u < 4; ++u) load8(base + (size_t)(p + u * PP) * C, f[u]);
#pragma unroll
        for (int u = 0; u < 4; ++u)
#pragma unroll
// ... 13 lines not shown
    }
#pragma unroll
    for (int j = 0; j < 8; ++j) {
        red[threadIdx.x * 16 + j] = s[j];
        red[threadIdx.x * 16 + 8 + j] = q[j];
    }
    __syncthreads();
    for (int t = threadIdx.x; t < 2 * C; t += 256) {
        const int which = t / C, c = t % C, vv = c >> 3, j = c & 7;
        float acc = 0.f;
        for (int r = 0; r < PP; ++r) acc += red[(r * VC + vv) * 16 + which * 8 + j];
        partial[(((size_t)n * slabs + slab) * 2 + which) * C + c] = acc;
    }
}

__global__ __launch_bounds__(256) void gn_finalize_kernel(const float *__restrict__ partial, int C, int G, int slabs, int HW, float eps,
                                                          float *__restrict__ stats, int total) {
    __shared__ double red[8];
    const int i = blockIdx.x;
    if (i >= total) return;
    const int n = i / G, g = i % G, cpg = C / G;
    double s = 0.0, q = 0.0;
    for (int e = threadIdx.x; e < slabs * cpg; e += 256) {
        const int sl = e / cpg, c = e % cpg;
        const float *ps = partial + (((size_t)n * slabs + sl) * 2) * C + g * cpg + c;
        s += (double)ps[0];
        q += (double)ps[C];
    }
    for (int off = 32; off > 0; off >>= 1) {
        s += __shfl_xor(s, off);
        q += __shfl_xor(q, off);
    }
    if ((threadIdx.x & 63) == 0) {
        red[threadIdx.x >> 6] = s;
        red[4 + (threadIdx.x >> 6)] = q;
    }
    __syncthreads();
    if (threadIdx.x == 0) {
        s = ((red[0] + red[1]) + red[2]) + red[3];
        q = ((red[4] + red[5]) + red[6]) + red[7];
        const double cnt = (double)HW * cpg;
        const double mean = s / cnt;
        const double var = fmax(q / cnt - mean * mean, 0.0);
        stats[2 * i] = (float)mean;
        stats[2 * i + 1] = (float)(1.0 / sqrt(var + (double)eps));
    }
}

__global__ __launch_bounds__(256) void gn_finalize_tiles_kernel(const float *__restrict__ partial, int C, int G, int TM, int HW, float eps,
                                                                float *__restrict__ stats, int total) {
    __shared__ double red[8];
    const int i = blockIdx.x;
    if (i >= total) return;
    const int n = i / G, g = i % G, cpg = C / G;
    const long long r0 = (long long)n * HW, r1 = r0 + HW - 1;
    const int t0 = (int)(r0 / TM), nt = (int)(r1 / TM) - t0 + 1;
    double s = 0.0, q = 0.0;
    for (int e = threadIdx.x; e < nt * cpg; e += 256) {
        const int t = t0 + e / cpg, c = e % cpg;
        const int h = ((long long)t * TM) / HW == n ? 0 : 1;
        const float *ps = partial + (((size_t)t * 2 + h) * 2) * C + g * cpg + c;
        s += (double)ps[0];
        q += (double)ps[C];
    }
    for (int off = 32; off > 0; off >>= 1) {
        s += __shfl_xor(s, off);
        q += __shfl_xor(q, off);
    }
    if ((threadIdx.x & 63) == 0) {
        red[threadIdx.x >> 6] = s;
        red[4 + (threadIdx.x >> 6)] = q;
    }
    __syncthreads();
    if (threadIdx.x == 0) {
        s = ((red[0] + red[1]) + red[2]) + red[3];
        q = ((red[4] + red[5]) + red[6]) + red[7];
        const double cnt = (double)HW * cpg;
        const double mean = s / cnt;
        const double var = fmax(q / cnt - mean * mean, 0.0);
        stats[2 * i] = (float)mean;
        stats[2 * i + 1] = (float)(1.0 / sqrt(var + (double)eps));
    }
}

template <typename T>
__global__ __launch_bounds__(256) void gn_apply_kernel(const T *__restrict__ x, const T *__restrict__ gamma, const T *__restrict__ beta,
                                                       const float *__restrict__ stats, const T *__restrict__ residual, T *__restrict__ out,
                                                       int HW, int C, int G, int relu) {
    const int VC = C >> 3, PP = 256 / VC;
    const int n = blockIdx.y;
    const int v = threadIdx.x % VC, pp = threadIdx.x / VC;
    const int cpg = C / G;
    float a[8], b[8];
    {
        float gm[8], bt[8];
        load8(gamma + v * 8, gm);
        load8(beta + v * 8, bt);
#pragma unroll
        for (int j = 0; j < 8; ++j) {
            const int g = (v * 8 + j) / cpg;
            const float mean = stats[2 * (n * G + g)], rstd = stats[2 * (n * G + g) + 1];
            a[j] = rstd * gm[j];
            b[j] = bt[j] - mean * a[j];
        }
    }
    const size_t off = (size_t)n * HW * C + v * 8;
    auto finish = [&](int p, float (&f)[8], const float (&r)[8]) {
#pragma unroll
        for (int j = 0; j < 8; ++j) f[j] = f[j] * a[j] + b[j];
        if (residual) {
#pragma unroll
            for (int j = 0; j < 8; ++j) f[j] = (float)(T)f[j] + r[j];
        }
        if (relu) {
#pragma unroll
            for (int j = 0; j < 8; ++j) f[j] = fmaxf(f[j], 0.f);
        }
        store8(out + off + (size_t)p * C, f);
    };
    const int step = gridDim.x * PP;
    int p = blockIdx.x * PP + pp;
    for (; p + 3 * step < HW; p += 4 * step) {
        float f[4][8], r[4][8];
#pragma unroll
        for (int u = 0; u < 4; ++u) load8(x + off + (size_t)(p + u * step) * C, f[u]);
        if (residual) {
#pragma unroll
            for (int u = 0; u < 4; ++u) load8(residual + off + (size_t)(p + u * step) * C, r[u]);
        }
#pragma unroll
        for (int u = 0; u < 4; ++u) finish(p + u * step, f[u], r[u]);
    }
    for (; p < HW; p += step) {
        float f[8], r[8];
// ... 221 lines not shown
    const int n = blockIdx.y;
    const long long total = (long long)Ho * Wo * VC;
    const int v = threadIdx.x % VC;
    float a[8], b[8];
    {
        float gm[8], bt[8];
        load8(gamma + v * 8, gm);
        load8(beta + v * 8, bt);
#pragma unroll
        for (int j = 0; j < 8; ++j) {
            const int g = (v * 8 + j) / cpg;
            const float mean = stats[2 * (n * G + g)], rstd = stats[2 * (n * G + g) + 1];
            a[j] = rstd * gm[j];
            b[j] = bt[j] - mean * a[j];
        }
    }
    for (long long i = (long long)blockIdx.x * 256 + threadIdx.x; i < total; i += (long long)gridDim.x * 256) {
        const int pix = (int)(i / VC), ox = pix % Wo, oy = pix / Wo;
        float m[8];
#pragma unroll
        for (int j = 0; j < 8; ++j) m[j] = 0.f;
#pragma unroll
        for (int ky = 0; ky < 3; ++ky)
#pragma unroll
            for (int kx = 0; kx < 3; ++kx) {
                const int iy = 2 * oy + ky - pad_t, ix = 2 * ox + kx - pad_l;
                if ((unsigned)iy < (unsigned)H && (unsigned)ix < (unsigned)W) {
                    float f[8];
                    load8(x + (((size_t)n * H + iy) * W + ix) * C + v * 8, f);
#pragma unroll
                    for (int j = 0; j < 8; ++j) m[j] = fmaxf(m[j], f[j] * a[j] + b[j]);
                }
            }
        store8(out + (((size_t)n * Ho + oy) * Wo + ox) * C + v * 8, m);
    }
}

static bool pow2(int x) { return x > 0 && (x & (x - 1)) == 0; }

int hive_gn_finalize_tiles(hive_ctx *ctx, const float *d_partial, int N, int HW, int C, int G, int tile_rows, float eps, float *d_stats) {
    hipLaunchKernelGGL(gn_finalize_tiles_kernel, dim3(N * G), dim3(256), 0, ctx->stream, d_partial, C, G, tile_rows, HW, eps, d_stats, N * G);
    HIVE_CHECK_HIP(ctx, hipGetLastError());
    return HIVE_OK;
}

extern "C" {

static int group_norm_impl(hive_ctx *ctx, const void *d_x, int dtype, int N, int HW, int C, int G, const void *d_gamma, const void *d_beta, float eps,
                           const void *d_residual, int relu, void *d_out, const void *d_gn_partial, int gn_tile_rows) {
    HIVE_REQUIRE(ctx, d_x && d_gamma && d_beta && d_out, "group_norm: NULL argument");
    HIVE_REQUIRE(ctx, N > 0 && HW > 0 && C >= 8 && C <= 2048 && pow2(C) && G > 0 && C % G == 0,
                 "group_norm: need C a power of two in [8, 2048] and C %% G == 0 (N=%d HW=%d C=%d G=%d)", N, HW, C, G);
    HIVE_REQUIRE(ctx, dtype == HIVE_BF16 || dtype == HIVE_F16, "group_norm: dtype must be HIVE_F16 or HIVE_BF16");
    const bool from_tiles = d_gn_partial && gn_tile_rows > 0;
    HIVE_REQUIRE(ctx, !from_tiles || gn_tile_rows <= HW, "group_norm_stats: tiles of %d rows on samples of %d", gn_tile_rows, HW);
    const int VC = C / 8, PP = 256 / VC;
    const int slabs = std::max(1, std::min(64, std::min(HW / (4 * PP) + 1, (ctx->num_cus * 8 + N - 1) / N)));
    const size_t partial_floats = from_tiles ? 0 : (size_t)N * slabs * 2 * C, stats_floats = (size_t)N * G * 2;
    int rc = hive_reserve_device(ctx, &ctx->d_scratch, &ctx->scratch_bytes, (partial_floats + stats_floats) * sizeof(float));
    if (rc) return rc;
    float *partial = (float *)ctx->d_scratch, *stats = partial + partial_floats;
    const dim3 g1(slabs, N), g3(std::max(1, std::min((HW + PP - 1) / PP, (ctx->num_cus * 8 + N - 1) / N)), N);
    if (from_tiles)
        hipLaunchKernelGGL(gn_finalize_tiles_kernel, dim3(N * G), dim3(256), 0, ctx->stream, (const float *)d_gn_partial, C, G, gn_tile_rows, HW, eps, stats, N * G);
    if (dtype == HIVE_BF16) {
        if (!from_tiles) {
            hipLaunchKernelGGL(gn_partial_kernel<bf16>, g1, dim3(256), 0, ctx->stream, (const bf16 *)d_x, HW, C, slabs, partial);
            hipLaunchKernelGGL(gn_finalize_kernel, dim3(N * G), dim3(256), 0, ctx->stream, partial, C, G, slabs, HW, eps, stats, N * G);
        }
        hipLaunchKernelGGL(gn_apply_kernel<bf16>, g3, dim3(256), 0, ctx->stream, (const bf16 *)d_x, (const bf16 *)d_gamma, (const bf16 *)d_beta,
                           stats, (const bf16 *)d_residual, (bf16 *)d_out, HW, C, G, relu);
    } else {
        if (!from_tiles) {
            hipLaunchKernelGGL(gn_partial_kernel<_Float16>, g1, dim3(256), 0, ctx->stream, (const _Float16 *)d_x, HW, C, slabs, partial);
            hipLaunchKernelGGL(gn_finalize_kernel, dim3(N * G), dim3(256), 0, ctx->stream, partial, C, G, slabs, HW, eps, stats, N * G);
        }
        hipLaunchKernelGGL(gn_apply_kernel<_Float16>, g3, dim3(256), 0, ctx->stream, (const _Float16 *)d_x, (const _Float16 *)d_gamma,
                           (const _Float16 *)d_beta, stats, (const _Float16 *)d_residual, (_Float16 *)d_out, HW, C, G, relu);
    }
    HIVE_CHECK_HIP(ctx, hipGetLastError());
    return HIVE_OK;
}

int hive_nhwc_group_norm(hive_ctx *ctx, const void *d_x, int dtype, int N, int HW, int C, int G, const void *d_gamma,
                         const void *d_beta, float eps, const void *d_residual, int relu, void *d_out) {
    HIVE_ENTER(ctx);
    if (!ctx) return hive_fail(nullptr, HIVE_ERR_INVALID, "ctx is NULL");
    return group_norm_impl(ctx, d_x, dtype, N, HW, C, G, d_gamma, d_beta, eps, d_residual, relu, d_out, nullptr, 0);
}

int hive_nhwc_group_norm_stats(hive_ctx *ctx, const void *d_x, int dtype, int N, int HW, int C, int G, const void *d_gamma, const void *d_beta,
                               float eps, const void *d_residual, int relu, void *d_out, const void *d_gn_partial, int gn_tile_rows) {
    HIVE_ENTER(ctx);
    if (!ctx) return hive_fail(nullptr, HIVE_ERR_INVALID, "ctx is NULL");
    return group_norm_impl(ctx, d_x, dtype, N, HW, C, G, d_gamma, d_beta, eps, d_residual, relu, d_out, d_gn_partial, gn_tile_rows);
}

int hive_nhwc_group_norm_relu_maxpool(hive_ctx *ctx, const void *d_x, int dtype, int N, int H, int W, int C, int G, const void *d_gamma, const void *d_beta,
                                      float eps, void *d_out, const void *d_gn_partial, int gn_tile_rows) {
    HIVE_ENTER(ctx);
    if (!ctx) return hive_fail(nullptr, HIVE_ERR_INVALID, "ctx is NULL");
    HIVE_REQUIRE(ctx, d_x && d_gamma && d_beta && d_out && d_out != d_x, "group_norm_relu_maxpool: bad pointers");
    HIVE_REQUIRE(ctx, N > 0 && N <= 65535 && H > 0 && W > 0 && C >= 8 && C <= 2048 && pow2(C) && G > 0 && C % G == 0,
                 "group_norm_relu_maxpool: need C a power of two in [8, 2048], C %% G == 0, N <= 65535 (N=%d H=%d W=%d C=%d G=%d)", N, H, W, C, G);
    HIVE_REQUIRE(ctx, dtype == HIVE_BF16 || dtype == HIVE_F16, "group_norm_relu_maxpool: dtype must be HIVE_F16 or HIVE_BF16");
    const int HW = H * W;
    const bool from_tiles = d_gn_partial && gn_tile_rows > 0;
    HIVE_REQUIRE(ctx, !from_tiles || gn_tile_rows <= HW, "group_norm_relu_maxpool: tiles of %d rows on samples of %d", gn_tile_rows, HW);
    const int VC = C / 8, PP = 256 / VC;
    const int slabs = std::max(1, std::min(64, std::min(HW / (4 * PP) + 1, (ctx->num_cus * 8 + N - 1) / N)));
    const size_t partial_floats = from_tiles ? 0 : (size_t)N * slabs * 2 * C, stats_floats = (size_t)N * G * 2;
    int rc = hive_reserve_device(ctx, &ctx->d_scratch, &ctx->scratch_bytes, (partial_floats + stats_floats) * sizeof(float));
    if (rc) return rc;
    float *partial = (float *)ctx->d_scratch, *stats = partial + partial_floats;
    const int Ho = (H + 1) / 2, Wo = (W + 1) / 2;
    const int pad_t = std::max((Ho - 1) * 2 + 3 - H, 0) / 2, pad_l = std::max((Wo - 1) * 2 + 3 - W, 0) / 2;
    const long long per_img = (long long)Ho * Wo * VC;
    const dim3 g1(slabs, N), gp((unsigned)std::max<long long>(1, std::min<long long>((per_img + 255) / 256, ((long long)ctx->num_cus * 32 + N - 1) / N)), N);
    if (from_tiles)
        hipLaunchKernelGGL(gn_finalize_tiles_kernel, dim3(N * G), dim3(256), 0, ctx->stream, (const float *)d_gn_partial, C, G, gn_tile_rows, HW, eps, stats, N * G);
    if (dtype == HIVE_BF16) {
        if (!from_tiles) {
            hipLaunchKernelGGL(gn_partial_kernel<bf16>, g1, dim3(256), 0, ctx->stream, (const bf16 *)d_x, HW, C, slabs, partial);
            hipLaunchKernelGGL(gn_finalize_kernel, dim3(N * G), dim3(256), 0, ctx->stream, partial, C, G, slabs, HW, eps, stats, N * G);
        }
        hipLaunchKernelGGL(gn_relu_maxpool_kernel<bf16>, gp, dim3(256), 0, ctx->stream, (const bf16 *)d_x, (const bf16 *)d_gamma, (const bf16 *)d_beta, stats,
                           (bf16 *)d_out, H, W, C, G, Ho, Wo, pad_t, pad_l);
    } else {
        if (!from_tiles) {
            hipLaunchKernelGGL(gn_partial_kernel<_Float16>, g1, dim3(256), 0, ctx->stream, (const _Float16 *)d_x, HW, C, slabs, partial);
            hipLaunchKernelGGL(gn_finalize_kernel, dim3(N * G), dim3(256), 0, ctx->stream, partial, C, G, slabs, HW, eps, stats, N * G);
        }
        hipLaunchKernelGGL(gn_relu_maxpool_kernel<_Float16>, gp, dim3(256), 0, ctx->stream, (const _Float16 *)d_x, (const _Float16 *)d_gamma,
                           (const _Float16 *)d_beta, stats, (_Float16 *)d_out, H, W, C, G, Ho, Wo, pad_t, pad_l);
    }
    HIVE_CHECK_HIP(ctx, hipGetLastError());
    return HIVE_OK;
}

int hive_nhwc_bias_act(hive_ctx *ctx, const void *d_x, int dtype, int64_t n_px, int C, const void *d_bias, int relu,
                       const void *d_residual, const void *d_residual2, void *d_out, void *d_out_relu) {
    HIVE_ENTER(ctx);
    if (!ctx) return hive_fail(nullptr, HIVE_ERR_INVALID, "ctx is NULL");
    HIVE_REQUIRE(ctx, d_x && d_bias && d_out, "bias_act: NULL argument");
    HIVE_REQUIRE(ctx, n_px > 0 && C > 0 && C % 8 == 0, "bias_act: need C %% 8 == 0 (n_px=%lld C=%d)", (long long)n_px, C);
    const size_t n_vec = (size_t)n_px * (C / 8);
    const dim3 grid((unsigned)std::min<size_t>((n_vec + 255) / 256, (size_t)ctx->num_cus * 32));
    if (dtype == HIVE_BF16)
        hipLaunchKernelGGL(bias_act_kernel<bf16>, grid, dim3(256), 0, ctx->stream, (const bf16 *)d_x, (const bf16 *)d_bias, (const bf16 *)d_residual,
                           (const bf16 *)d_residual2, (bf16 *)d_out, (bf16 *)d_out_relu, n_vec, C / 8, relu);
    else if (dtype == HIVE_F16)
        hipLaunchKernelGGL(bias_act_kernel<_Float16>, grid, dim3(256), 0, ctx->stream, (const _Float16 *)d_x, (const _Float16 *)d_bias,
                           (const _Float16 *)d_residual, (const _Float16 *)d_residual2, (_Float16 *)d_out, (_Float16 *)d_out_relu, n_vec, C / 8, relu);
    else
        return hive_fail(ctx, HIVE_ERR_INVALID, "bias_act: dtype must be HIVE_F16 or HIVE_BF16");
    HIVE_CHECK_HIP(ctx, hipGetLastError());
    return HIVE_OK;
}

int hive_nhwc_upsample2x(hive_ctx *ctx, const void *d_in, const void *d_bias, int dtype, int N, int H, int W, int C, void *d_out) {
    HIVE_ENTER(ctx);
    if (!ctx) return hive_fail(nullptr, HIVE_ERR_INVALID, "ctx is NULL");
    HIVE_REQUIRE(ctx, d_in && d_out, "upsample2x: NULL argument");
    HIVE_REQUIRE(ctx, N > 0 && H > 0 && W > 0 && C > 0 && C % 8 == 0, "upsample2x: need C %% 8 == 0 (N=%d H=%d W=%d C=%d)", N, H, W, C);
    HIVE_REQUIRE(ctx, H <= 65535 && N <= 65535, "upsample2x: H %d / N %d too large for the launch grid", H, N);
    const bool gather_only = getenv("HIVE_UPSAMPLE_GATHER") != nullptr;
    const size_t lds = (size_t)(UP_TY + 2) * (UP_TX + 2) * C * 2;
    if (C <= 512 && !gather_only && (H + UP_TY - 1) / UP_TY <= 65535) {
        const dim3 tiles((unsigned)((W + UP_TX - 1) / UP_TX), (unsigned)((H + UP_TY - 1) / UP_TY), (unsigned)N);
        static hive_device_latch latch;
        if (!latch.done(ctx)) {
            HIVE_CHECK_HIP(ctx, hipFuncSetAttribute((const void *)upsample2x_lds_kernel<bf16>, hipFuncAttributeMaxDynamicSharedMemorySize, 64 * 1024));
            HIVE_CHECK_HIP(ctx, hipFuncSetAttribute((const void *)upsample2x_lds_kernel<_Float16>, hipFuncAttributeMaxDynamicSharedMemorySize, 64 * 1024));
            latch.mark(ctx);
        }
        if (dtype == HIVE_BF16) {
            hipLaunchKernelGGL(upsample2x_lds_kernel<bf16>, tiles, dim3(256), lds, ctx->stream, (const bf16 *)d_in, (const bf16 *)d_bias, (bf16 *)d_out, N, H, W, C);
        } else if (dtype == HIVE_F16) {
            hipLaunchKernelGGL(upsample2x_lds_kernel<_Float16>, tiles, dim3(256), lds, ctx->stream, (const _Float16 *)d_in, (const _Float16 *)d_bias, (_Float16 *)d_out,
                               N, H, W, C);
        } else {
            return hive_fail(ctx, HIVE_ERR_INVALID, "upsample2x: dtype must be HIVE_F16 or HIVE_BF16");
        }
        HIVE_CHECK_HIP(ctx, hipGetLastError());
// ... 52 lines not shown
```

### hive_amd/csrc/hive_internal.hpp

```cpp
#pragma once
#include <hip/hip_runtime.h>

#include <cstdarg>
#include <cstdint>
#include <cstdio>
#include <cstring>
#include <string>
#include <vector>

#include "../../include/hive_mi355x.h"

#define HIVE_WAVE 64

struct hive_staging_slot {
    void *pinned = nullptr;
    size_t bytes = 0;
    hipEvent_t done = nullptr;
    bool in_flight = false;
};

struct hive_ctx {
    int device = 0;
    int num_cus = 256;
    hipStream_t stream = nullptr;
    bool owns_stream = false;
    int round_mode = HIVE_ROUND_HALF_EVEN;
    std::string last_error;

    static constexpr int kSlots = 4;
    hive_staging_slot slots[kSlots];
    int next_slot = 0;

    void *d_scratch = nullptr;
    size_t scratch_bytes = 0;
    void *d_frame = nullptr;
    size_t frame_bytes = 0;
    void *d_batch = nullptr;
    size_t batch_bytes = 0;
    void *d_in = nullptr;
    size_t in_bytes = 0;
    int tsdf_scalars = 0;
    int tsdf_multi_scalars = 0;
    unsigned *d_scalars = nullptr;
    void *h_pinned_small = nullptr;
    void *d_zeros = nullptr;
    void *d_splitk = nullptr;
    size_t splitk_bytes = 0;
    unsigned *d_splitk_count = nullptr;
    void *d_gram = nullptr;
    size_t gram_bytes = 0;

    bool deterministic = false;
    int64_t n_splitk_launches = 0, n_deep_ring_launches = 0;

    bool timing = false;
    std::vector<hipEvent_t> ev_pool;
    size_t ev_used = 0;
    hipEvent_t last_start = nullptr, last_stop = nullptr;
};

int hive_fail(hive_ctx *ctx, int code, const char *fmt, ...);

struct hive_device_guard {
    int prev = -1;
    bool switched = false;
    explicit hive_device_guard(const hive_ctx *ctx) {
        if (!ctx) return;
        if (hipGetDevice(&prev) == hipSuccess && prev != ctx->device) switched = hipSetDevice(ctx->device) == hipSuccess;
    }
    ~hive_device_guard() {
        if (switched) (void)hipSetDevice(prev);
    }
    hive_device_guard(const hive_device_guard &) = delete;
    hive_device_guard &operator=(const hive_device_guard &) = delete;
};
#define HIVE_ENTER(ctx) hive_device_guard _hive_device_guard(ctx)
void hive_set_global_error(const char *msg);

#define HIVE_CHECK_HIP(ctx, expr)                                                                        \
    do {                                                                                                 \
        hipError_t _e = (expr);                                                                          \
        if (_e != hipSuccess)                                                                            \
            return hive_fail((ctx), _e == hipErrorOutOfMemory ? HIVE_ERR_NOMEM : HIVE_ERR_DEVICE,        \
                             "%s failed: %s (%s:%d)", #expr, hipGetErrorString(_e), __FILE__, __LINE__); \
    } while (0)

#define HIVE_REQUIRE(ctx, cond, ...)                                   \
    do {                                                               \
        if (!(cond)) return hive_fail((ctx), HIVE_ERR_INVALID, __VA_ARGS__); \
    } while (0)

struct hive_device_latch {
    bool set[64] = {};
    bool done(const hive_ctx *ctx) const { return ctx->device < 64 && set[ctx->device]; }
    void mark(const hive_ctx *ctx) {
        if (ctx->device < 64) set[ctx->device] = true;
    }
};

int hive_reserve_device(hive_ctx *ctx, void **ptr, size_t *cur, size_t bytes);
int hive_upload(hive_ctx *ctx, void *dst, const void *src, size_t bytes);
int hive_gn_finalize_tiles(hive_ctx *ctx, const float *d_partial, int N, int HW, int C, int G, int tile_rows, float eps, float *d_stats);
constexpr int HIVE_SPLITK_TILES = 4096;
int hive_splitk_workspace(hive_ctx *ctx, size_t bytes, void **ws, unsigned **count);
int hive_gram_gn_stats(hive_ctx *ctx, const void *d_x, int dtype, int N, int H, int W, int C_in, int C_out, int stride, int Ho, int Wo, int G, const float *d_tables,
                       float eps, float *d_stats, float *d_S_out, float *d_s_out);
__device__ __forceinline__ unsigned block_exclusive(unsigned c, unsigned *lds) {
    const int lane = threadIdx.x & 63, wave = threadIdx.x >> 6;
    unsigned inc = c;
    for (int off = 1; off < 64; off <<= 1) {
        const unsigned o = (unsigned)__shfl_up((int)inc, off);
        if (lane >= off) inc += o;
    }
    if (lane == 63) lds[wave] = inc;
    __syncthreads();
    unsigned before = 0;
    for (int w = 0; w < wave; ++w) before += lds[w];
    __syncthreads();
    return before + inc - c;
}
struct hive_scratch_layout {
    char *base = nullptr;
    size_t off = 0;
    template <class T>
    T *take(size_t count) {
        T *at = base ? (T *)(base + off) : nullptr;
        off += (count * sizeof(T) + 255) & ~(size_t)255;
        return at;
    }
    size_t bytes() const { return off; }
};
struct hive_dec_job {
    const double *pos;
    const int32_t *faces;
    const unsigned *counts;
    long long vert_cap = 0, face_cap = 0;
    long long budget = 0;
    double max_error = 0.0;
    int32_t *out_faces = nullptr;
    long long out_face_cap = 0;
    int32_t *out_vertex_index = nullptr;
    unsigned *out_counts = nullptr;
};
size_t hive_decimate_scratch_bytes(long long vert_cap, long long face_cap);
int32_t *hive_decimate_vmap(void *scratch, long long vert_cap, long long face_cap);
int hive_decimate_run(hive_ctx *ctx, const hive_dec_job &job, void *scratch, int64_t stats[3]);
int hive_dilate_frames(hive_ctx *ctx, const uint8_t *d_mask, int n, int H, int W, const uint8_t *se, int kh, int kw, int iterations, uint8_t *a, uint8_t *b,
                       const uint8_t **d_result);
int hive_time_begin(hive_ctx *ctx);
int hive_time_end(hive_ctx *ctx);

struct hive_tsdf {
    hive_ctx *ctx = nullptr;
    int64_t dim[3] = {0, 0, 0};
    int64_t n = 0;
// ... 33 lines not shown
```

### hive_amd/csrc/stem.hip

```cpp
#include "hive_internal.hpp"

#include <algorithm>

#include "mfma_pipe.hpp"

using hive_mfma::f32x4;
using hive_mfma::vec;

namespace {

constexpr int ST_TH = 8, ST_TW = 32;
constexpr int ST_PH = 2 * ST_TH + 5, ST_PW = 2 * ST_TW + 5;
constexpr int ST_ROW = 240;
constexpr int ST_RD = 104;
constexpr int ST_K = 7 * 32;
constexpr int ST_WP = ST_K + 16;
constexpr int ST_RQ = ST_RD / 4;
constexpr int ST_LOADS = (ST_PH * ST_RQ + 255) / 256;

template <typename T>
struct StemParams {
    const T *x;
    const T *w;
    T *out;
    int H, W, Ho, Wo, pad_t, pad_l;
    int tiles_x, tiles_y, n_tiles;
    int run;
    float *gn_partial;
};

__device__ __forceinline__ float stem_dot2(vec<__bf16, 2> a, vec<__bf16, 2> b, float c) { return __builtin_amdgcn_fdot2_f32_bf16(a, b, c, false); }
__device__ __forceinline__ float stem_dot2(vec<_Float16, 2> a, vec<_Float16, 2> b, float c) { return __builtin_amdgcn_fdot2(a, b, c, false); }
using hive_mfma::dpp_row_total;

template <typename T>
__global__ __launch_bounds__(256, 3) void stem_conv_kernel(StemParams<T> p) {
    __shared__ __attribute__((aligned(16))) T patch[ST_PH * ST_ROW + 64];
    __shared__ __attribute__((aligned(16))) T wl[64 * ST_WP];
    __shared__ float wsum[4][2][64];
    const int tid = threadIdx.x;
    for (int i = tid; i < 64 * ST_K / 8; i += 256) {
        const int row = i / (ST_K / 8), c8 = i - row * (ST_K / 8);
        const int nt = row >> 4, f4 = (row >> 2) & 3, e = row & 3;
        const int ch = (nt >> 1) * 32 + f4 * 8 + (nt & 1) * 4 + e;
        *reinterpret_cast<uint4 *>(wl + row * ST_WP + c8 * 8) = reinterpret_cast<const uint4 *>(p.w)[ch * (ST_K / 8) + c8];
    }
    if (tid < 64) patch[ST_PH * ST_ROW + tid] = (T)0.0f;
    for (int i = tid; i < ST_PH * (ST_ROW / 2 - ST_RD); i += 256) {
        const int r = i / (ST_ROW / 2 - ST_RD), d = i - r * (ST_ROW / 2 - ST_RD);
        reinterpret_cast<uint32_t *>(patch)[r * (ST_ROW / 2) + ST_RD + d] = 0u;
    }
    const bool even = (p.W % 2 == 0) && (p.pad_l % 2 == 0);
    const int per_img = p.tiles_x * p.tiles_y;
    typedef uint32_t u4 __attribute__((ext_vector_type(4)));
    typedef uint32_t u4u __attribute__((ext_vector_type(4), aligned(4)));
    u4 regs[ST_LOADS];
    auto fetch = [&](int tile) {
        int tid = threadIdx.x;
        asm volatile("" : "+v"(tid));
        const int img = tile / per_img, t = tile - img * per_img;
        const int oy0 = (t / p.tiles_x) * ST_TH, ox0 = (t % p.tiles_x) * ST_TW;
        const int iy0 = 2 * oy0 - p.pad_t, ix0 = 2 * ox0 - p.pad_l;
        const T *xin = p.x + (size_t)img * p.H * p.W * 3;
        const bool inside = iy0 >= 0 && iy0 + ST_PH <= p.H && ix0 >= 0 && ix0 + (2 * ST_RD + 2) / 3 <= p.W;
        if (even && inside) {
            const uint32_t *base = reinterpret_cast<const uint32_t *>(xin + ((size_t)iy0 * p.W + ix0) * 3);
            const int row_dwords = p.W * 3 / 2;
#pragma unroll
            for (int k = 0; k < ST_LOADS; ++k) {
                const int i = tid + 256 * k, r = i / ST_RQ, d = i - r * ST_RQ;
                regs[k] = u4{0u, 0u, 0u, 0u};
                if (k + 1 < ST_LOADS || i < ST_PH * ST_RQ) regs[k] = *reinterpret_cast<const u4u *>(base + (size_t)r * row_dwords + 4 * d);
            }
        } else {
#pragma unroll
            for (int k = 0; k < ST_LOADS; ++k) {
                const int i = tid + 256 * k, r = i / ST_RQ, d = i - r * ST_RQ;
                T v[8];
#pragma unroll
                for (int h = 0; h < 8; ++h) {
                    const int e = 8 * d + h, col = e / 3, c = e - col * 3;
                    const int iy = iy0 + r, ix = ix0 + col;
                    v[h] = (T)0.0f;
                    if (r < ST_PH && e < ST_PW * 3 && (unsigned)iy < (unsigned)p.H && (unsigned)ix < (unsigned)p.W) v[h] = xin[((size_t)iy * p.W + ix) * 3 + c];
                }
                regs[k] = *reinterpret_cast<const u4 *>(v);
            }
        }
    };
    auto flush_sums = [&](int run_idx) {
        if (tid < 128) {
            const int which = tid >> 6, c = tid & 63;
            const float a = ((wsum[0][which][c] + wsum[1][which][c]) + wsum[2][which][c]) + wsum[3][which][c];
            p.gn_partial[((size_t)run_idx * 4 + which) * 64 + c] = a;
            p.gn_partial[((size_t)run_idx * 4 + 2 + which) * 64 + c] = 0.f;
        }
    };
    const int n_runs = p.n_tiles / p.run;
    int run_idx = blockIdx.x, in_run = 0, pending = -1;
    if (run_idx < n_runs) fetch(run_idx * p.run);
    f32x4 rs[4], rq[4];
    for (; run_idx < n_runs;) {
        const int tile = run_idx * p.run + in_run;
        const bool last_of_run = in_run + 1 == p.run;
        const int next_tile = last_of_run ? (run_idx + (int)gridDim.x) * p.run : tile + 1;
        int tix = tid;
        asm volatile("" : "+v"(tix));
        const int lane = tix & 63, wave = __builtin_amdgcn_readfirstlane(tix >> 6), fr = lane & 15, fq = lane >> 4;
        __syncthreads();
#pragma unroll
        for (int k = 0; k < ST_LOADS; ++k) {
            const int i = tix + 256 * k, r = i / ST_RQ, d = i - r * ST_RQ;
            if (k + 1 < ST_LOADS || i < ST_PH * ST_RQ) *reinterpret_cast<u4 *>(reinterpret_cast<uint32_t *>(patch) + r * (ST_ROW / 2) + 4 * d) = regs[k];
        }
        if (pending >= 0) {
            flush_sums(pending);
            pending = -1;
        }
        __syncthreads();
        if (next_tile < p.n_tiles) fetch(next_tile);
        const int img = tile / per_img, t = tile - img * per_img;
        const int oy0 = (t / p.tiles_x) * ST_TH, ox0 = (t % p.tiles_x) * ST_TW;
        f32x4 acc[4][4];
        hive_mfma::zero_acc(acc);
#pragma unroll 1
        for (int ky = 0; ky < 7; ++ky) {
            vec<T, 8> wf[4], af[4];
#pragma unroll
            for (int nt = 0; nt < 4; ++nt) wf[nt] = *reinterpret_cast<const vec<T, 8> *>(wl + (nt * 16 + fr) * ST_WP + ky * 32 + fq * 8);
#pragma unroll
            for (int mt = 0; mt < 4; ++mt) {
                const int oy = 2 * wave + (mt >> 1), ox = 16 * (mt & 1) + fr;
                const T *src = patch + (2 * oy + ky) * ST_ROW + 6 * ox + fq * 8;
                uint32_t raw[4];
#pragma unroll
                for (int q = 0; q < 4; ++q) raw[q] = reinterpret_cast<const uint32_t *>(src)[q];
                af[mt] = *reinterpret_cast<const vec<T, 8> *>(raw);
            }
#pragma unroll
            for (int mt = 0; mt < 4; ++mt)
#pragma unroll
                for (int nt = 0; nt < 4; ++nt) acc[nt][mt] = hive_mfma::mfma16(wf[nt], af[mt], acc[nt][mt]);
        }
        T *out = p.out + (size_t)img * p.Ho * p.Wo * 64;
#pragma unroll
        for (int mt = 0; mt < 4; ++mt) {
            const int oy = oy0 + 2 * wave + (mt >> 1), ox = ox0 + 16 * (mt & 1) + fr;
            if (oy < p.Ho && ox < p.Wo) {
// ... 1 lines not shown
                for (int a = 0; a < 2; ++a) {
                    vec<T, 8> ov;
#pragma unroll
                    for (int j = 0; j < 4; ++j) ov[j] = (T)acc[2 * a][mt][j], ov[4 + j] = (T)acc[2 * a + 1][mt][j];
                    *reinterpret_cast<vec<T, 8> *>(out + ((size_t)oy * p.Wo + ox) * 64 + a * 32 + fq * 8) = ov;
                }
            }
        }
        if (p.gn_partial) {
            vec<T, 2> ones;
            ones[0] = ones[1] = (T)1.0f;
#pragma unroll
            for (int nt = 0; nt < 4; ++nt) {
                if (in_run == 0) rs[nt] = rq[nt] = f32x4{0.f, 0.f, 0.f, 0.f};
#pragma unroll
                for (int mt = 0; mt < 4; mt += 2)
#pragma unroll
                    for (int e = 0; e < 4; ++e) {
                        vec<T, 2> y;
                        y[0] = (T)acc[nt][mt][e], y[1] = (T)acc[nt][mt + 1][e];
                        rs[nt][e] = stem_dot2(y, ones, rs[nt][e]);
                        rq[nt][e] = stem_dot2(y, y, rq[nt][e]);
                    }
            }
            if (last_of_run) {
#pragma unroll
                for (int nt = 0; nt < 4; ++nt) {
                    f32x4 sv, qv;
#pragma unroll
                    for (int e = 0; e < 4; ++e) {
                        sv[e] = dpp_row_total(rs[nt][e]);
                        qv[e] = dpp_row_total(rq[nt][e]);
                    }
                    if (fr == 0) {
                        const int ch = (nt >> 1) * 32 + fq * 8 + (nt & 1) * 4;
                        *reinterpret_cast<f32x4 *>(&wsum[wave][0][ch]) = sv;
                        *reinterpret_cast<f32x4 *>(&wsum[wave][1][ch]) = qv;
                    }
                }
                pending = run_idx;
            }
        }
        if (last_of_run) {
            run_idx += gridDim.x;
            in_run = 0;
        } else {
            ++in_run;
        }
    }
    if (pending >= 0) {
        __syncthreads();
        flush_sums(pending);
    }
}

template <typename T>
__global__ __launch_bounds__(256) void maxpool3x3s2_kernel(const T *__restrict__ x, T *__restrict__ out, int N, int H, int W, int C, int Ho,
                                                           int Wo, int pad_t, int pad_l) {
    const int c8 = C / 8;
    const long long total = (long long)N * Ho * Wo * c8;
    for (long long i = (long long)blockIdx.x * 256 + threadIdx.x; i < total; i += (long long)gridDim.x * 256) {
        const int cc = (int)(i % c8);
        const long long pix = i / c8;
        const int ox = (int)(pix % Wo), oy = (int)((pix / Wo) % Ho), n = (int)(pix / ((long long)Wo * Ho));
        float m[8];
#pragma unroll
        for (int j = 0; j < 8; ++j) m[j] = -INFINITY;
#pragma unroll
        for (int ky = 0; ky < 3; ++ky)
#pragma unroll
            for (int kx = 0; kx < 3; ++kx) {
                const int iy = 2 * oy + ky - pad_t, ix = 2 * ox + kx - pad_l;
                if ((unsigned)iy < (unsigned)H && (unsigned)ix < (unsigned)W) {
                    const vec<T, 8> v = *reinterpret_cast<const vec<T, 8> *>(x + (((size_t)n * H + iy) * W + ix) * C + cc * 8);
#pragma unroll
                    for (int j = 0; j < 8; ++j) m[j] = fmaxf(m[j], (float)v[j]);
                }
            }
        vec<T, 8> o;
#pragma unroll
        for (int j = 0; j < 8; ++j) o[j] = (T)m[j];
        *reinterpret_cast<vec<T, 8> *>(out + (size_t)pix * C + cc * 8) = o;
    }
}

template <typename T>
int launch_stem(hive_ctx *ctx, const void *d_x, int N, int H, int W, const void *d_w, void *d_out, float *d_gn_partial, long long gn_partial_floats,
                int *gn_tile_rows) {
    StemParams<T> p{};
    p.x = (const T *)d_x;
    p.w = (const T *)d_w;
    p.out = (T *)d_out;
    p.H = H;
    p.W = W;
    p.Ho = (H + 1) / 2;
    p.Wo = (W + 1) / 2;
    p.pad_t = std::max((p.Ho - 1) * 2 + 7 - H, 0) / 2;
    p.pad_l = std::max((p.Wo - 1) * 2 + 7 - W, 0) / 2;
    p.tiles_x = (p.Wo + ST_TW - 1) / ST_TW;
    p.tiles_y = (p.Ho + ST_TH - 1) / ST_TH;
    const long long tiles = (long long)N * p.tiles_x * p.tiles_y;
    HIVE_REQUIRE(ctx, tiles < (1ll << 31), "resnet_stem_conv: %lld tiles", tiles);
    p.n_tiles = (int)tiles;
    if (gn_tile_rows) *gn_tile_rows = 0;
    const int per_img = p.tiles_x * p.tiles_y;
    p.run = per_img % 4 == 0 ? 4 : (per_img % 2 == 0 ? 2 : 1);
    if (d_gn_partial && gn_tile_rows && p.Ho % ST_TH == 0 && p.Wo % ST_TW == 0) {
        HIVE_REQUIRE(ctx, tiles / p.run * 4 * 64 <= gn_partial_floats, "resnet_stem_conv_gn: gn_partial holds %lld floats, %lld needed", gn_partial_floats,
                     tiles / p.run * 4 * 64);
        p.gn_partial = d_gn_partial;
        *gn_tile_rows = ST_TH * ST_TW * p.run;
    }
    const unsigned grid = (unsigned)std::min<long long>(tiles / p.run, (long long)ctx->num_cus * 3);
    hipLaunchKernelGGL(stem_conv_kernel<T>, dim3(grid), dim3(256), 0, ctx->stream, p);
    HIVE_CHECK_HIP(ctx, hipGetLastError());
    return HIVE_OK;
}

}

extern "C" {

static int stem_entry(hive_ctx *ctx, const void *d_x, int dtype, int N, int H, int W, const void *d_w, void *d_out, void *d_gn_partial, int64_t gn_partial_floats,
                      int *gn_tile_rows) {
    HIVE_REQUIRE(ctx, d_x && d_w && d_out, "resnet_stem_conv: NULL argument");
    HIVE_REQUIRE(ctx, dtype == HIVE_BF16 || dtype == HIVE_F16, "resnet_stem_conv: dtype must be HIVE_F16 or HIVE_BF16");
    HIVE_REQUIRE(ctx, N > 0 && H >= 7 && W >= 7 && (long long)N * H * W < (1ll << 31), "resnet_stem_conv: bad sizes %d x %d x %d", N, H, W);
    return dtype == HIVE_BF16 ? launch_stem<__bf16>(ctx, d_x, N, H, W, d_w, d_out, (float *)d_gn_partial, gn_partial_floats, gn_tile_rows)
                              : launch_stem<_Float16>(ctx, d_x, N, H, W, d_w, d_out, (float *)d_gn_partial, gn_partial_floats, gn_tile_rows);
}

int hive_resnet_stem_conv(hive_ctx *ctx, const void *d_x, int dtype, int N, int H, int W, const void *d_w, void *d_out) {
    HIVE_ENTER(ctx);
    if (!ctx) return hive_fail(nullptr, HIVE_ERR_INVALID, "ctx is NULL");
    return stem_entry(ctx, d_x, dtype, N, H, W, d_w, d_out, nullptr, 0, nullptr);
}

int hive_resnet_stem_conv_gn(hive_ctx *ctx, const void *d_x, int dtype, int N, int H, int W, const void *d_w, void *d_out, void *d_gn_partial,
                             int64_t gn_partial_floats, int *gn_tile_rows) {
    HIVE_ENTER(ctx);
    if (!ctx) return hive_fail(nullptr, HIVE_ERR_INVALID, "ctx is NULL");
    HIVE_REQUIRE(ctx, d_gn_partial && gn_tile_rows, "resnet_stem_conv_gn: NULL argument");
    return stem_entry(ctx, d_x, dtype, N, H, W, d_w, d_out, d_gn_partial, gn_partial_floats, gn_tile_rows);
}

int hive_nhwc_maxpool3x3s2(hive_ctx *ctx, const void *d_x, int dtype, int N, int H, int W, int C, void *d_out) {
    HIVE_ENTER(ctx);
    if (!ctx) return hive_fail(nullptr, HIVE_ERR_INVALID, "ctx is NULL");
    HIVE_REQUIRE(ctx, d_x && d_out && d_x != d_out, "nhwc_maxpool3x3s2: bad pointers");
    HIVE_REQUIRE(ctx, dtype == HIVE_BF16 || dtype == HIVE_F16, "nhwc_maxpool3x3s2: dtype must be HIVE_F16 or HIVE_BF16");
    HIVE_REQUIRE(ctx, N > 0 && H > 0 && W > 0 && C > 0 && C % 8 == 0, "nhwc_maxpool3x3s2: bad sizes %d x %d x %d x %d", N, H, W, C);
    const int Ho = (H + 1) / 2, Wo = (W + 1) / 2;
    const int pad_t = std::max((Ho - 1) * 2 + 3 - H, 0) / 2, pad_l = std::max((Wo - 1) * 2 + 3 - W, 0) / 2;
    const long long total = (long long)N * Ho * Wo * (C / 8);
    const int blocks = (int)std::min<long long>((total + 255) / 256, (long long)ctx->num_cus * 32);
    if (dtype == HIVE_BF16)
        hipLaunchKernelGGL(maxpool3x3s2_kernel<__bf16>, dim3(blocks), dim3(256), 0, ctx->stream, (const __bf16 *)d_x, (__bf16 *)d_out, N, H, W, C, Ho, Wo, pad_t, pad_l);
    else
        hipLaunchKernelGGL(maxpool3x3s2_kernel<_Float16>, dim3(blocks), dim3(256), 0, ctx->stream, (const _Float16 *)d_x, (_Float16 *)d_out, N, H, W, C, Ho, Wo, pad_t, pad_l);
    HIVE_CHECK_HIP(ctx, hipGetLastError());
    return HIVE_OK;
}

}
```

### hive_amd/dpt/ops.py

```python
import os

import torch
import torch.nn.functional as F

from hive_amd import _lib

HALF_TYPES = (torch.float16, torch.bfloat16)


def not_covered(what, why):
    raise _lib.HiveError(_lib.ERR_INVALID, f"engine='hip': {what} is not covered by the HIP kernels ({why}); the HIP engine never drops to a "
                                           f"PyTorch operator -- build the model with engine='torch' for the PyTorch formulation")


def _why_not_map(x, channels_multiple=8):
    if not x.is_cuda:
        return "the tensor is not on the GPU"
    if x.dtype not in HALF_TYPES:
        return f"dtype {x.dtype}: the kernels compute in float16 / bfloat16"
    if x.dim() != 4 or not x.is_contiguous(memory_format=torch.channels_last):
        return "the activation must be a 4-d tensor in channels_last memory format"
    if x.shape[1] % channels_multiple:
        return f"{x.shape[1]} channels: a multiple of {channels_multiple} is needed"
    return None
# ... 58 lines not shown
    if not (k[0] == k[1] and k[0] in kernels):
        return f"kernel {tuple(k)}"
    if not (conv.stride[0] == conv.stride[1] and conv.stride[0] in (1, 2)):
        return f"stride {tuple(conv.stride)}"
    if tuple(conv.dilation) != (1, 1) or conv.groups != 1:
        return "dilation / groups"
    if conv.in_channels % 64 or conv.out_channels % cout_multiple or x.shape[1] != conv.in_channels:
        return f"{conv.in_channels} -> {conv.out_channels} channels: multiples of 64 -> {cout_multiple} are needed"
    if conv.weight.dtype != x.dtype:
        return f"weights are {conv.weight.dtype}, the tensor {x.dtype}"
    if not (conv.padding[0] == conv.padding[1] and conv.padding[0] < k[0]):
        return f"padding {tuple(conv.padding)}"
    return None


def conv3x3_eligible(x, conv):
    return (_why_not_conv(x, conv, kernels=(3,), cout_multiple=128) is None and tuple(conv.stride) == (1, 1) and tuple(conv.padding) == (1, 1))


def conv3x3(x, conv, relu=False, residual=None, residual2=None, also_relu=False, with_bias=True):
    n, _, h, w = x.shape
    out = torch.empty((n, conv.out_channels, h, w), dtype=x.dtype, device=x.device, memory_format=torch.channels_last)
    out_relu = torch.empty_like(out) if also_relu else None
    for r in (residual, residual2):
        assert r is None or (r.shape == out.shape and r.dtype == out.dtype and r.is_contiguous(memory_format=torch.channels_last))
    bias = conv.bias if (with_bias and conv.bias is not None) else None
    ctx = _lib.default_context(x.device.index or 0)
    ctx.check(ctx.lib.hive_nhwc_conv3x3(ctx.handle, x.data_ptr(), _code(x.dtype), n, h, w, conv.in_channels, conv.out_channels,
                                        _conv3x3_weight(conv).data_ptr(), _lib.ptr(bias), int(bool(relu)), _lib.ptr(residual),
                                        _lib.ptr(residual2), out.data_ptr(), _lib.ptr(out_relu)))
    return (out, out_relu) if also_relu else out


def conv_geometry(conv, ih, iw, same_pad=False):
    k, st = conv.kernel_size[0], conv.stride[0]
    if same_pad:
        oh, ow = -(-ih // st), -(-iw // st)
        ph, pw = max((oh - 1) * st + k - ih, 0), max((ow - 1) * st + k - iw, 0)
        return k, st, ph // 2, pw // 2, oh, ow
    p = conv.padding[0]
    return k, st, p, p, (ih + 2 * p - k) // st + 1, (iw + 2 * p - k) // st + 1


def conv_eligible(x, conv):
    return _why_not_conv(x, conv) is None


def require_conv(x, conv, what="convolution"):
    why = _why_not_conv(x, conv)
    if why:
        not_covered(what, why)


def conv2d(x, conv, weight=None, same_pad=False, relu=False, residual=None, residual2=None, also_relu=False, with_bias=True, gn_stats=False):
    n, _, ih, iw = x.shape
    k, st, pt, pl, oh, ow = conv_geometry(conv, ih, iw, same_pad)
    w = weight if weight is not None else _conv3x3_weight(conv)
    if not w.is_contiguous(memory_format=torch.channels_last):
        w = w.contiguous(memory_format=torch.channels_last)
    out = torch.empty((n, conv.out_channels, oh, ow), dtype=x.dtype, device=x.device, memory_format=torch.channels_last)
    out_relu = torch.empty_like(out) if also_relu else None
    for r in (residual, residual2):
        assert r is None or (r.shape == out.shape and r.dtype == out.dtype and r.is_contiguous(memory_format=torch.channels_last))
    bias = conv.bias if (with_bias and conv.bias is not None) else None
    ctx = _lib.default_context(x.device.index or 0)
    if gn_stats:
        import ctypes
        partial = torch.empty(int(ctx.lib.hive_nhwc_conv_gn_partial_floats(n * oh * ow, conv.out_channels)), dtype=torch.float32, device=x.device)
        tile_rows = ctypes.c_int(0)
        ctx.check(ctx.lib.hive_nhwc_conv_gn(ctx.handle, x.data_ptr(), _code(x.dtype), n, ih, iw, conv.in_channels, conv.out_channels, k, st, pt, pl, oh, ow,
                                            w.data_ptr(), _lib.ptr(bias), int(bool(relu)), _lib.ptr(residual), _lib.ptr(residual2), out.data_ptr(),
                                            _lib.ptr(out_relu), partial.data_ptr(), partial.numel(), ctypes.byref(tile_rows)))
        out.hive_gn_stats = (partial, tile_rows.value)
    else:
        ctx.check(ctx.lib.hive_nhwc_conv(ctx.handle, x.data_ptr(), _code(x.dtype), n, ih, iw, conv.in_channels, conv.out_channels, k, st, pt, pl, oh, ow,
                                         w.data_ptr(), _lib.ptr(bias), int(bool(relu)), _lib.ptr(residual), _lib.ptr(residual2), out.data_ptr(),
                                         _lib.ptr(out_relu)))
    return (out, out_relu) if also_relu else out


def conv_gn_act(x, conv, norm, weight=None, same_pad=False, relu=True, residual=None):
    import ctypes
    if not (conv_eligible(x, conv) and conv.bias is None and norm.weight.dtype == x.dtype):
        return None
    n, _, ih, iw = x.shape
    k, st, pt, pl, oh, ow = conv_geometry(conv, ih, iw, same_pad)
    cout, g = conv.out_channels, norm.num_groups
    if cout % 256 or cout % g or (cout // g) % 8 or oh * ow < 256:
        return None
    w = weight if weight is not None else _conv3x3_weight(conv)
    if not w.is_contiguous(memory_format=torch.channels_last):
        w = w.contiguous(memory_format=torch.channels_last)
    out = torch.empty((n, cout, oh, ow), dtype=x.dtype, device=x.device, memory_format=torch.channels_last)
    assert residual is None or (residual.shape == out.shape and residual.dtype == out.dtype and residual.is_contiguous(memory_format=torch.channels_last))
    ctx = _lib.default_context(x.device.index or 0)
    scratch = torch.empty(int(ctx.lib.hive_nhwc_conv_gn_partial_floats(n * oh * ow, cout)) + 2 * n * g, dtype=torch.float32, device=x.device)
    fused = ctypes.c_int(0)
    cin = conv.in_channels
    out_elems = n * oh * ow * cout
    if k == 1 and os.environ.get("HIVE_GN_GRAM", "1") != "0" and not getattr(ctx, "deterministic", False) and g == 32 and ((cin in (64, 128) and out_elems >= 150_000_000) or
                                                                               (cin == 256 and st == 2 and out_elems >= 250_000_000)):
        def tables():
            t = torch.empty(int(ctx.lib.hive_gn_gram_table_floats(cin, g)), dtype=torch.float32, device=x.device)
            ctx.check(ctx.lib.hive_gn_gram_prepare(ctx.handle, w.data_ptr(), _code(x.dtype), cin, cout, g, t.data_ptr()))
            return t
        tab = _cached(conv, ("gram", x.dtype, weight is not None), [conv.weight], tables)
        ctx.check(ctx.lib.hive_nhwc_conv_gn_apply_gram(ctx.handle, x.data_ptr(), _code(x.dtype), n, ih, iw, cin, cout, st, oh, ow, w.data_ptr(), tab.data_ptr(), g,
                                                       norm.weight.data_ptr(), norm.bias.data_ptr(), float(norm.eps), _lib.ptr(residual), int(bool(relu)),
                                                       out.data_ptr(), scratch.data_ptr(), scratch.numel(), ctypes.byref(fused)))
        if fused.value:
            return out
    ctx.check(ctx.lib.hive_nhwc_conv_gn_apply(ctx.handle, x.data_ptr(), _code(x.dtype), n, ih, iw, conv.in_channels, cout, k, st, pt, pl, oh, ow, w.data_ptr(), g,
                                              norm.weight.data_ptr(), norm.bias.data_ptr(), float(norm.eps), _lib.ptr(residual), int(bool(relu)),
                                              out.data_ptr(), scratch.data_ptr(), scratch.numel(), ctypes.byref(fused)))
    return out if fused.value else None


def _cached(layer, what, params, build):
    stamp = tuple((p.data_ptr(), p._version, p.dtype, p.device) for p in params)
    cache = _module_cache(layer)
    hit = cache.get(what)
    if hit is None or hit[0] != stamp:
        with torch.no_grad():
            hit = cache[what] = (stamp, build())
    return hit[1]


def patch_embed_eligible(x, conv):
    k = conv.kernel_size
    return (x.is_cuda and x.dtype in HALF_TYPES and x.dim() == 4 and x.is_contiguous(memory_format=torch.channels_last) and type(conv) is torch.nn.Conv2d
            and k[0] == k[1] and tuple(conv.stride) == tuple(k) and tuple(conv.padding) == (0, 0) and conv.groups == 1 and conv.weight.dtype == x.dtype
            and x.shape[2] % k[0] == 0 and x.shape[3] % k[0] == 0 and (k[0] * k[0] * conv.in_channels) % 64 == 0 and conv.out_channels % 128 == 0)


def patch_embed(x, conv):
    n, c, h, w = x.shape
    p, d = conv.kernel_size[0], conv.out_channels
    wmat, bias = _cached(conv, "patch", (conv.weight, conv.bias) if conv.bias is not None else (conv.weight,), lambda: (
        conv.weight.permute(0, 2, 3, 1).reshape(d, p * p * c).contiguous(),
        (conv.bias.float() if conv.bias is not None else torch.zeros(d, device=x.device)).contiguous()))
    m = n * (h // p) * (w // p)
    cols = torch.empty((m, p * p * c), dtype=x.dtype, device=x.device)
    out = torch.empty((n, (h // p) * (w // p), d), dtype=x.dtype, device=x.device)
    ctx = _lib.default_context(x.device.index or 0)
    ctx.check(ctx.lib.hive_patch_rows(ctx.handle, x.data_ptr(), _code(x.dtype), n, h, w, c, p, cols.data_ptr()))
    ctx.check(ctx.lib.hive_vit_linear(ctx.handle, cols.data_ptr(), _code(x.dtype), wmat.data_ptr(), bias.data_ptr(), None, out.data_ptr(), m, d, p * p * c, 0))
    return out


def conv_transpose_eligible(x, layer):
    k = layer.kernel_size
    return (x.is_cuda and x.dtype in HALF_TYPES and x.dim() == 4 and x.is_contiguous(memory_format=torch.channels_last)
            and isinstance(layer, torch.nn.ConvTranspose2d) and k[0] == k[1] and tuple(layer.stride) == tuple(k) and tuple(layer.padding) == (0, 0)
            and tuple(layer.output_padding) == (0, 0) and layer.groups == 1 and tuple(layer.dilation) == (1, 1) and layer.weight.dtype == x.dtype
            and layer.in_channels % 64 == 0 and layer.out_channels % 64 == 0 and k[0] <= 8)


def conv_transpose(x, layer):
    n, cin, h, w = x.shape
    s_, cout = layer.kernel_size[0], layer.out_channels
    wmat = _cached(layer, "convT", (layer.weight,), lambda: layer.weight.permute(2, 3, 1, 0).reshape(s_ * s_ * cout, cin).contiguous())
    tmp = torch.empty((n * h * w, s_ * s_ * cout), dtype=x.dtype, device=x.device)
    out = torch.empty((n, cout, h * s_, w * s_), dtype=x.dtype, device=x.device, memory_format=torch.channels_last)
    ctx = _lib.default_context(x.device.index or 0)
    ctx.check(ctx.lib.hive_nhwc_conv(ctx.handle, x.data_ptr(), _code(x.dtype), n, h, w, cin, s_ * s_ * cout, 1, 1, 0, 0, h, w, wmat.data_ptr(), None, 0, None, None,
                                     tmp.data_ptr(), None))
    ctx.check(ctx.lib.hive_nhwc_pixel_shuffle_bias(ctx.handle, tmp.data_ptr(), _lib.ptr(layer.bias), _code(x.dtype), n, h, w, cout, s_, out.data_ptr()))
    return out


def stem_conv_eligible(x, conv):
    return (x.is_cuda and x.dtype in HALF_TYPES and x.dim() == 4 and x.shape[1] == 3 and x.is_contiguous(memory_format=torch.channels_last)
            and tuple(conv.kernel_size) == (7, 7) and tuple(conv.stride) == (2, 2) and conv.in_channels == 3 and conv.out_channels == 64
            and conv.bias is None and x.shape[2] >= 7 and x.shape[3] >= 7)


def stem_conv(x, conv, weight):
    stamp = (weight.data_ptr(), weight._version, weight.dtype)
    cache = _module_cache(conv)
    hit = cache.get("stem")
    if hit is None or hit[0] != stamp:
        w = torch.zeros((64, 7, 32), dtype=x.dtype, device=weight.device)
        w[:, :, :21] = weight.detach().permute(0, 2, 3, 1).reshape(64, 7, 21)
        hit = cache["stem"] = (stamp, w.contiguous())
    n, _, h, w_ = x.shape
    oh, ow = (h + 1) // 2, (w_ + 1) // 2
    out = torch.empty((n, 64, oh, ow), dtype=x.dtype, device=x.device, memory_format=torch.channels_last)
    ctx = _lib.default_context(x.device.index or 0)
    import ctypes
    partial = torch.empty(int(ctx.lib.hive_nhwc_conv_gn_partial_floats(n * oh * ow, 64)), dtype=torch.float32, device=x.device)
    tile_rows = ctypes.c_int(0)
    ctx.check(ctx.lib.hive_resnet_stem_conv_gn(ctx.handle, x.data_ptr(), _code(x.dtype), n, h, w_, hit[1].data_ptr(), out.data_ptr(), partial.data_ptr(),
                                               partial.numel(), ctypes.byref(tile_rows)))
    if tile_rows.value:
        out.hive_gn_stats = (partial, tile_rows.value)
    return out


def bneck_gn_conv3x3(t, norm, conv, weight):
    import ctypes
    stats = getattr(t, "hive_gn_stats", None)
    if (stats is None or _why_not_map(t) or t.shape[1] != 64 or conv.in_channels != 64 or conv.out_channels != 64 or tuple(conv.kernel_size) != (3, 3)
            or tuple(conv.stride) != (1, 1) or conv.bias is not None or not norm.apply_act or norm.num_groups != 32 or norm.weight.dtype != t.dtype):
        return None
    w = weight if weight.is_contiguous(memory_format=torch.channels_last) else weight.contiguous(memory_format=torch.channels_last)
    n, c, h, wd = t.shape
    out = torch.empty_like(t)
    ctx = _lib.default_context(t.device.index or 0)
    partial = torch.empty(int(ctx.lib.hive_nhwc_conv_gn_partial_floats(n * h * wd, 64)), dtype=torch.float32, device=t.device)
    tile_rows, fused = ctypes.c_int(0), ctypes.c_int(0)
    ctx.check(ctx.lib.hive_bneck_gn_conv3x3(ctx.handle, t.data_ptr(), _code(t.dtype), n, h, wd, c, stats[0].data_ptr(), int(stats[1]), norm.weight.data_ptr(),
                                            norm.bias.data_ptr(), float(norm.eps), w.data_ptr(), out.data_ptr(), partial.data_ptr(), partial.numel(),
                                            ctypes.byref(tile_rows), ctypes.byref(fused)))
    if not fused.value:
        return None
    if tile_rows.value:
        out.hive_gn_stats = (partial, tile_rows.value)
    return out


def group_norm_relu_maxpool(x, norm, stats=None):
    why = _why_not_map(x) or (None if norm.weight.dtype == x.dtype else f"affine parameters are {norm.weight.dtype}, the tensor {x.dtype}")
    n, c, h, w = x.shape
    if not why and ((c & (c - 1)) or c > 2048):
        why = f"{c} channels: a power of two <= 2048 is needed"
    if why:
        not_covered("group_norm + max pool", why)
    out = torch.empty((n, c, (h + 1) // 2, (w + 1) // 2), dtype=x.dtype, device=x.device, memory_format=torch.channels_last)
    ctx = _lib.default_context(x.device.index or 0)
    partial, tile_rows = stats if stats is not None else (None, 0)
    ctx.check(ctx.lib.hive_nhwc_group_norm_relu_maxpool(ctx.handle, x.data_ptr(), _code(x.dtype), n, h, w, c, norm.num_groups, norm.weight.data_ptr(),
                                                        norm.bias.data_ptr(), float(norm.eps), out.data_ptr(), _lib.ptr(partial), int(tile_rows)))
    return out


def maxpool3x3s2_same(x, engine="torch"):
    if engine == "hip":
        why = _why_not_map(x)
        if why:
            not_covered("max_pool 3 x 3 / 2", why)
        n, c, h, w = x.shape
        out = torch.empty((n, c, (h + 1) // 2, (w + 1) // 2), dtype=x.dtype, device=x.device, memory_format=torch.channels_last)
        ctx = _lib.default_context(x.device.index or 0)
        ctx.check(ctx.lib.hive_nhwc_maxpool3x3s2(ctx.handle, x.data_ptr(), _code(x.dtype), n, h, w, c, out.data_ptr()))
        return out
    return None


def conv_bias_act(x, conv, relu=False, residual=None, residual2=None, engine="torch", also_relu=False):
    if engine == "hip":
        why = _why_not_conv(x, conv, kernels=(3,), cout_multiple=128) or (None if conv3x3_eligible(x, conv) else "3 x 3 / stride 1 / padding 1 only") or \
            (None if conv.bias is None or conv.bias.dtype == x.dtype else f"bias is {conv.bias.dtype}, the tensor {x.dtype}")
        if why:
            not_covered("convolution of a residual unit", why)
        if residual is not None:
            residual = residual.contiguous(memory_format=torch.channels_last)
        if residual2 is not None:
            residual2 = residual2.contiguous(memory_format=torch.channels_last)
        return conv3x3(x, conv, relu=relu, residual=residual, residual2=residual2, also_relu=also_relu)
    y = conv(x)
    if residual is not None:
        y = y + residual
# ... 20 lines not shown
```

### include/hive_mi355x.h

```cpp
#ifndef HIVE_MI355X_H
#define HIVE_MI355X_H

#include <stddef.h>
#include <stdint.h>

#ifdef __cplusplus
extern "C" {
#endif

#define HIVE_ABI_VERSION 2

typedef enum hive_status {
    HIVE_OK = 0,
    HIVE_ERR_INVALID = -1,
    HIVE_ERR_DEVICE = -2,
    HIVE_ERR_NOMEM = -3,
    HIVE_ERR_EMPTY = -4,
    HIVE_ERR_STATE = -5
} hive_status;

typedef enum hive_mem_kind { HIVE_MEM_HOST = 0, HIVE_MEM_DEVICE = 1 } hive_mem_kind;

typedef enum hive_round_mode { HIVE_ROUND_HALF_EVEN = 0, HIVE_ROUND_HALF_AWAY = 1 } hive_round_mode;

// ... 138 lines not shown
int hive_vit_create(hive_ctx *ctx, int dtype, int depth, int dim, int heads, int mlp_dim, float ln_eps,
                    const hive_vit_block_weights *blocks, hive_vit **out);
int hive_vit_weights_modified(hive_vit *vit);
int hive_vit_destroy(hive_vit *vit);
int hive_vit_forward(hive_vit *vit, const void *x, int B, int N, const int *tap_blocks, int n_taps,
                     void *const *tap_out);
int hive_vit_layernorm(hive_ctx *ctx, const void *x, int dtype, const float *gamma, const float *beta, void *out,
                       int M, int D, float eps);
int hive_vit_linear(hive_ctx *ctx, const void *A, int dtype, const void *W, const float *bias, const void *residual,
                    void *C, int M, int N, int K, int epilogue);
int hive_vit_qkv(hive_ctx *ctx, const void *x, int dtype, const void *W, const float *bias, void *qk, void *vT,
                 int B, int Np, int D, int H);
int hive_vit_attention(hive_ctx *ctx, const void *qk, int dtype, const void *vT, void *out, int B, int N, int Np,
                       int D, int H);

int hive_dpt_preprocess(hive_ctx *ctx, const uint8_t *d_rgb, int64_t n_values, float mean, float std,
                        int dtype, void *d_out);
int hive_dpt_resize_preprocess(hive_ctx *ctx, const uint8_t *d_rgb, int B, int H, int W, int out_h, int out_w, float mean, float std,
                               int dtype, void *d_out);
int hive_depth_resize_nearest(hive_ctx *ctx, const float *d_depth, int B, int h, int w, int H, int W, float depth_scale, float max_depth,
                              float *d_out_depth, uint16_t *d_out_mm, float *d_out_m);
int hive_dpt_head_tail(hive_ctx *ctx, const void *d_feat, int dtype, int64_t n_px, int C,
                       const float *h_pre_bias, int pre_relu, const float *h_weight, float bias,
                       int non_negative, int invert, float scale, float shift, float *d_depth,
                       float depth_scale, float max_depth, uint16_t *d_out_mm, float *d_out_m);
int hive_dpt_head_fused(hive_ctx *ctx, const void *d_x, const float *d_b0, int dtype, int N, int H, int W, int C_in, int C_mid,
                        const void *d_w3, const float *h_b3, const float *h_w1, float b1, int non_negative, int invert,
                        float scale, float shift, float *d_depth, float depth_scale, float max_depth,
                        uint16_t *d_out_mm, float *d_out_m);

int hive_nhwc_group_norm(hive_ctx *ctx, const void *d_x, int dtype, int N, int HW, int C, int G,
                         const void *d_gamma, const void *d_beta, float eps, const void *d_residual,
                         int relu, void *d_out);
int hive_nhwc_bias_act(hive_ctx *ctx, const void *d_x, int dtype, int64_t n_px, int C, const void *d_bias, int relu,
                       const void *d_residual, const void *d_residual2, void *d_out, void *d_out_relu);
int hive_nhwc_upsample2x(hive_ctx *ctx, const void *d_in, const void *d_bias, int dtype, int N, int H, int W, int C, void *d_out);

int hive_nhwc_conv3x3(hive_ctx *ctx, const void *d_x, int dtype, int N, int H, int W, int C_in, int C_out, const void *d_w,
                      const void *d_bias, int relu, const void *d_residual, const void *d_residual2, void *d_out,
                      void *d_out_relu);

int hive_nhwc_conv(hive_ctx *ctx, const void *d_x, int dtype, int N, int H, int W, int C_in, int C_out, int kernel, int stride,
                   int pad_top, int pad_left, int H_out, int W_out, const void *d_w, const void *d_bias, int relu,
                   const void *d_residual, const void *d_residual2, void *d_out, void *d_out_relu);

int64_t hive_nhwc_conv_gn_partial_floats(int64_t n_px, int C_out);
int hive_nhwc_conv_gn(hive_ctx *ctx, const void *d_x, int dtype, int N, int H, int W, int C_in, int C_out, int kernel, int stride,
                      int pad_top, int pad_left, int H_out, int W_out, const void *d_w, const void *d_bias, int relu,
                      const void *d_residual, const void *d_residual2, void *d_out, void *d_out_relu, void *d_gn_partial,
                      int64_t gn_partial_floats, int *gn_tile_rows);
int hive_nhwc_group_norm_stats(hive_ctx *ctx, const void *d_x, int dtype, int N, int HW, int C, int G, const void *d_gamma,
                               const void *d_beta, float eps, const void *d_residual, int relu, void *d_out,
                               const void *d_gn_partial, int gn_tile_rows);

int hive_nhwc_conv_gn_apply(hive_ctx *ctx, const void *d_x, int dtype, int N, int H, int W, int C_in, int C_out, int kernel,
                            int stride, int pad_top, int pad_left, int H_out, int W_out, const void *d_w, int G,
                            const void *d_gamma, const void *d_beta, float eps, const void *d_residual, int relu, void *d_out,
                            void *d_scratch, int64_t scratch_floats, int *fused);

int64_t hive_gn_gram_table_floats(int C_in, int G);
int hive_gn_gram_prepare(hive_ctx *ctx, const void *d_w, int dtype, int C_in, int C_out, int G, float *d_tables);
int hive_gn_gram_parts(hive_ctx *ctx, int N, int C_in, int H_out, int W_out);
int hive_gn_gram_stats(hive_ctx *ctx, const void *d_x, int dtype, int N, int H, int W, int C_in, int C_out, int stride, int H_out, int W_out, int G,
                       const float *d_tables, float eps, float *d_stats, float *d_S_out, float *d_s_out);
int hive_nhwc_conv_gn_apply_gram(hive_ctx *ctx, const void *d_x, int dtype, int N, int H, int W, int C_in, int C_out, int stride, int H_out, int W_out,
                                 const void *d_w, const float *d_tables, int G, const void *d_gamma, const void *d_beta, float eps,
                                 const void *d_residual, int relu, void *d_out, void *d_scratch, int64_t scratch_floats, int *fused);

int hive_patch_rows(hive_ctx *ctx, const void *d_x, int dtype, int N, int H, int W, int C, int patch, void *d_out);
int hive_nhwc_pixel_shuffle_bias(hive_ctx *ctx, const void *d_in, const void *d_bias, int dtype, int N, int H, int W, int C, int s,
                                 void *d_out);

int hive_resnet_stem_conv(hive_ctx *ctx, const void *d_x, int dtype, int N, int H, int W, const void *d_w, void *d_out);
int hive_nhwc_maxpool3x3s2(hive_ctx *ctx, const void *d_x, int dtype, int N, int H, int W, int C, void *d_out);
int hive_bneck_gn_conv3x3(hive_ctx *ctx, const void *d_x, int dtype, int N, int H, int W, int C, const void *d_in_partial, int in_tile_rows,
                          const void *d_gamma, const void *d_beta, float eps, const void *d_w, void *d_out, void *d_gn_partial,
                          int64_t gn_partial_floats, int *gn_tile_rows, int *fused);
int hive_resnet_stem_conv_gn(hive_ctx *ctx, const void *d_x, int dtype, int N, int H, int W, const void *d_w, void *d_out, void *d_gn_partial,
                             int64_t gn_partial_floats, int *gn_tile_rows);
int hive_nhwc_group_norm_relu_maxpool(hive_ctx *ctx, const void *d_x, int dtype, int N, int H, int W, int C, int G, const void *d_gamma,
                                      const void *d_beta, float eps, void *d_out, const void *d_gn_partial, int gn_tile_rows);

typedef struct hive_dpt hive_dpt;
typedef struct hive_dpt_tensor {
    const char *name;
    const void *data;
} hive_dpt_tensor;
typedef struct hive_dpt_config {
    int backbone;
    float scale, shift;
    int invert, non_negative;
    float gn_eps, ln_eps;
    float head_b3[32], head_w1[32], head_b1;
    int dtype;
} hive_dpt_config;
int hive_dpt_create(hive_ctx *ctx, const hive_dpt_config *config, const hive_dpt_tensor *tensors, int n_tensors, hive_dpt **out);
int hive_dpt_forward(hive_dpt *dpt, const uint8_t *d_rgb, int B, int H, int W, const void *d_pos_embed, float *d_depth, float max_depth,
                     uint16_t *d_out_mm, float *d_out_m);
int hive_dpt_forward_frames(hive_dpt *dpt, const uint8_t *d_rgb, int B, int frame_h, int frame_w, int net_h, int net_w, const void *d_pos_embed,
                            float *d_depth, float max_depth, uint16_t *d_out_mm, float *d_out_m);
int hive_dpt_arena_bytes(hive_dpt *dpt, int64_t *bytes);
int hive_dpt_weights_modified(hive_dpt *dpt);
int hive_dpt_destroy(hive_dpt *dpt);

#ifdef __cplusplus
}
#endif
#endif
```

Before: 1394 frames/s.

## Fold GroupNorm statistics finalisation into conv kernels via last-arriver counters

```diff
diff --git a/hive_amd/_lib.py b/hive_amd/_lib.py
--- a/hive_amd/_lib.py
+++ b/hive_amd/_lib.py
@@ -116,6 +116,9 @@
     "hive_nhwc_conv_gn_partial_floats": (c_int64, [c_int64, c_int]),
     "hive_nhwc_conv_gn": (c_int, [c_void_p, c_void_p, c_int, c_int, c_int, c_int, c_int, c_int, c_int, c_int, c_int, c_int, c_int, c_int, c_void_p, c_void_p,
                                   c_int, c_void_p, c_void_p, c_void_p, c_void_p, c_void_p, c_int64, P(c_int)]),
+    "hive_nhwc_conv_gn_fold_floats": (c_int64, [c_int, c_int]),
+    "hive_nhwc_conv_gn_fold": (c_int, [c_void_p, c_void_p, c_int, c_int, c_int, c_int, c_int, c_int, c_int, c_int, c_int, c_int, c_int, c_int, c_void_p, c_void_p,
+                                       c_int, c_void_p, c_void_p, c_void_p, c_void_p, c_void_p, c_int64, P(c_int), c_int, c_float]),
     "hive_nhwc_conv_gn_apply": (c_int, [c_void_p, c_void_p, c_int, c_int, c_int, c_int, c_int, c_int, c_int, c_int, c_int, c_int, c_int, c_int, c_void_p, c_int,
                                         c_void_p, c_void_p, c_float, c_void_p, c_int, c_void_p, c_void_p, c_int64, P(c_int)]),
     "hive_nhwc_group_norm_stats": (c_int, [c_void_p, c_void_p, c_int, c_int, c_int, c_int, c_int, c_void_p, c_void_p, c_float, c_void_p, c_int,
@@ -134,6 +137,7 @@
     "hive_bneck_gn_conv3x3": (c_int, [c_void_p, c_void_p, c_int, c_int, c_int, c_int, c_int, c_void_p, c_int, c_void_p, c_void_p, c_float, c_void_p, c_void_p, c_void_p,
                                       c_int64, P(c_int), P(c_int)]),
     "hive_resnet_stem_conv_gn": (c_int, [c_void_p, c_void_p, c_int, c_int, c_int, c_int, c_void_p, c_void_p, c_void_p, c_int64, P(c_int)]),
+    "hive_resnet_stem_conv_gn_fold": (c_int, [c_void_p, c_void_p, c_int, c_int, c_int, c_int, c_void_p, c_void_p, c_void_p, c_int64, P(c_int), c_int, c_float]),
     "hive_nhwc_group_norm_relu_maxpool": (c_int, [c_void_p, c_void_p, c_int, c_int, c_int, c_int, c_int, c_int, c_void_p, c_void_p, c_float, c_void_p, c_void_p,
                                                   c_int]),
     "hive_dpt_create": (c_int, [c_void_p, c_void_p, c_void_p, c_int, P(c_void_p)]),
diff --git a/hive_amd/csrc/bneck.hip b/hive_amd/csrc/bneck.hip
--- a/hive_amd/csrc/bneck.hip
+++ b/hive_amd/csrc/bneck.hip
@@ -2,6 +2,7 @@
 
 #include <algorithm>
 
+#include "gn_finalize.hpp"
 #include "mfma_pipe.hpp"
 
 using hive_mfma::f32x4;
@@ -27,6 +28,7 @@
     T *out;
     float *gn_partial;
     int H, W, tiles_x, tiles_y, n_tiles;
+    hive_gn::Fold fold;
 };
 
 __device__ __forceinline__ int bn_swz(int q, int c) { return q * 128 + ((c ^ (q & 6)) << 4); }
@@ -182,16 +184,27 @@
                 float s = 0.f;
 #pragma unroll
                 for (int w = 0; w < 8; ++w) s += wsum[w][which][c];
-                p.gn_partial[((size_t)tile * 4 + which) * 64 + c] = s;
-                p.gn_partial[((size_t)tile * 4 + 2 + which) * 64 + c] = 0.f;
-            }
-        }
+                hive_gn::store_partial(p.gn_partial + ((size_t)tile * 4 + which) * 64 + c, s, p.fold.count != nullptr);
+                hive_gn::store_partial(p.gn_partial + ((size_t)tile * 4 + 2 + which) * 64 + c, 0.f, p.fold.count != nullptr);
+            }
+        }
+    }
+    if (p.fold.count) {
+        asm volatile("s_waitcnt vmcnt(0)" ::: "memory");
+        int *fin = reinterpret_cast<int *>(wsum);
+        const int my_tiles = (p.n_tiles - (int)blockIdx.x + (int)gridDim.x - 1) / (int)gridDim.x;
+        const int n_fin = hive_gn::arrive_all(p.fold.count, my_tiles, threadIdx.x, 512, fin, [&](int k, int &n, unsigned &expect) {
+            n = (blockIdx.x + k * gridDim.x) / per_img;
+            expect = (unsigned)per_img;
+            return true;
+        });
+        hive_gn::finalise_listed<8>(p.gn_partial, 64, p.fold, p.H * p.W / per_img, p.H * p.W, fin, n_fin, threadIdx.x);
     }
 }
 
 template <typename T>
 int launch_bneck(hive_ctx *ctx, const void *d_x, int N, int H, int W, const float *stats, const void *gamma, const void *beta, const void *d_w, void *d_out,
-                 float *d_gn_partial, long long gn_partial_floats, int *gn_tile_rows) {
+                 float *d_gn_partial, long long gn_partial_floats, int *gn_tile_rows, float eps) {
     static hive_device_latch latch;
     if (!latch.done(ctx)) {
         HIVE_CHECK_HIP(ctx, hipFuncSetAttribute((const void *)bneck_conv3x3_kernel<T>, hipFuncAttributeMaxDynamicSharedMemorySize, BN_LDS));
@@ -215,6 +228,15 @@
     if (d_gn_partial && gn_tile_rows && W % BN_TW == 0 && (H * W) % per_img == 0 && tiles * 4 * 64 <= gn_partial_floats) {
         p.gn_partial = d_gn_partial;
         *gn_tile_rows = H * W / per_img;
+        const long long base = hive_nhwc_conv_gn_partial_floats((int64_t)N * H * W, 64);
+        if (gn_partial_floats >= base + hive_nhwc_conv_gn_fold_floats(N, 32) && N <= 1023 && hive_finalize_fold_enabled()) {
+            int rc = hive_fold_counters(ctx, &p.fold.count);
+            if (rc) return rc;
+            p.fold.stats = d_gn_partial + base;
+            p.fold.G = 32;
+            p.fold.eps = eps;
+            *gn_tile_rows |= HIVE_GN_FOLDED;
+        }
     }
     const unsigned grid = (unsigned)std::min<long long>(tiles, (long long)ctx->num_cus);
     hipLaunchKernelGGL(bneck_conv3x3_kernel<T>, dim3(grid), dim3(512), BN_LDS, ctx->stream, p);
@@ -234,13 +256,18 @@
     HIVE_REQUIRE(ctx, N > 0 && H > 0 && W > 0 && (long long)N * H * W < (1ll << 31), "bneck_gn_conv3x3: bad sizes %d x %d x %d", N, H, W);
     *fused = 0;
     if (gn_tile_rows) *gn_tile_rows = 0;
-    if (C != 64 || !d_in_partial || in_tile_rows <= 0 || in_tile_rows > H * W) return HIVE_OK;
-    int rc = hive_reserve_device(ctx, &ctx->d_scratch, &ctx->scratch_bytes, (size_t)N * 32 * 2 * sizeof(float));
-    if (rc) return rc;
-    float *stats = (float *)ctx->d_scratch;
-    if ((rc = hive_gn_finalize_tiles(ctx, (const float *)d_in_partial, N, H * W, 64, 32, in_tile_rows, eps, stats))) return rc;
-    rc = dtype == HIVE_BF16 ? launch_bneck<__bf16>(ctx, d_x, N, H, W, stats, d_gamma, d_beta, d_w, d_out, (float *)d_gn_partial, gn_partial_floats, gn_tile_rows)
-                            : launch_bneck<_Float16>(ctx, d_x, N, H, W, stats, d_gamma, d_beta, d_w, d_out, (float *)d_gn_partial, gn_partial_floats, gn_tile_rows);
+    if (C != 64 || !d_in_partial) return HIVE_OK;
+    const float *stats = hive_gn_folded_stats(d_in_partial, &in_tile_rows, (int64_t)N * H * W, 64);
+    if (in_tile_rows <= 0 || in_tile_rows > H * W) return HIVE_OK;
+    int rc;
+    if (!stats) {
+        rc = hive_reserve_device(ctx, &ctx->d_scratch, &ctx->scratch_bytes, (size_t)N * 32 * 2 * sizeof(float));
+        if (rc) return rc;
+        if ((rc = hive_gn_finalize_tiles(ctx, (const float *)d_in_partial, N, H * W, 64, 32, in_tile_rows, eps, (float *)ctx->d_scratch))) return rc;
+        stats = (const float *)ctx->d_scratch;
+    }
+    rc = dtype == HIVE_BF16 ? launch_bneck<__bf16>(ctx, d_x, N, H, W, stats, d_gamma, d_beta, d_w, d_out, (float *)d_gn_partial, gn_partial_floats, gn_tile_rows, eps)
+                            : launch_bneck<_Float16>(ctx, d_x, N, H, W, stats, d_gamma, d_beta, d_w, d_out, (float *)d_gn_partial, gn_partial_floats, gn_tile_rows, eps);
     if (rc) return rc;
     *fused = 1;
     return HIVE_OK;
diff --git a/hive_amd/csrc/capi.hip b/hive_amd/csrc/capi.hip
--- a/hive_amd/csrc/capi.hip
+++ b/hive_amd/csrc/capi.hip
@@ -1,4 +1,5 @@
 #include <algorithm>
+#include <cstdlib>
 
 #include "hive_internal.hpp"
 
@@ -41,6 +42,20 @@
     if (rc) return rc;
     *ws = ctx->d_splitk;
     *count = ctx->d_splitk_count;
+    return HIVE_OK;
+}
+
+bool hive_finalize_fold_enabled() {
+    const char *e = getenv("HIVE_FINALIZE_FOLD");
+    return !(e && e[0] == '0');
+}
+
+int hive_fold_counters(hive_ctx *ctx, unsigned **count) {
+    if (!ctx->d_fold_count) {
+        HIVE_CHECK_HIP(ctx, hipMalloc((void **)&ctx->d_fold_count, (size_t)HIVE_FOLD_COUNTERS * HIVE_FOLD_COUNTER_STRIDE * sizeof(unsigned)));
+        HIVE_CHECK_HIP(ctx, hipMemsetAsync(ctx->d_fold_count, 0, (size_t)HIVE_FOLD_COUNTERS * HIVE_FOLD_COUNTER_STRIDE * sizeof(unsigned), ctx->stream));
+    }
+    *count = ctx->d_fold_count;
     return HIVE_OK;
 }
 
@@ -162,6 +177,7 @@
     if (ctx->d_gram) (void)hipFree(ctx->d_gram);
     if (ctx->d_splitk) (void)hipFree(ctx->d_splitk);
     if (ctx->d_splitk_count) (void)hipFree(ctx->d_splitk_count);
+    if (ctx->d_fold_count) (void)hipFree(ctx->d_fold_count);
     if (ctx->d_in) (void)hipFree(ctx->d_in);
     if (ctx->d_scalars) (void)hipFree(ctx->d_scalars);
     if (ctx->h_pinned_small) (void)hipHostFree(ctx->h_pinned_small);
diff --git a/hive_amd/csrc/conv.hip b/hive_amd/csrc/conv.hip
--- a/hive_amd/csrc/conv.hip
+++ b/hive_amd/csrc/conv.hip
@@ -1,4 +1,5 @@
 #include "hive_internal.hpp"
+#include "gn_finalize.hpp"
 #include "mfma_pipe.hpp"
 
 #include <algorithm>
@@ -34,6 +35,7 @@
     int split_k;
     hive_mfma::f32x4 *sk_ws;
     unsigned *sk_count;
+    hive_gn::Fold fold;
 };
 
 __device__ __forceinline__ float gn_affine_exact(float x, float rstd, float gamma, float beta, float mean) {
@@ -203,6 +205,46 @@
 }
 
 constexpr int BK = 64;
+static_assert(hive_gn::COUNTER_STRIDE == HIVE_FOLD_COUNTER_STRIDE, "the counters' spacing, host and device");
+
+template <int TM>
+__device__ __forceinline__ unsigned gn_tiles_of_sample(int n, int hw, int tiles_n) {
+    const unsigned r0 = (unsigned)n * (unsigned)hw;
+    return ((r0 + hw - 1) / TM - r0 / TM + 1) * tiles_n;
+}
+template <int TM>
+__device__ __forceinline__ bool gn_tile_contrib(int em0, int second, int hw, int n_img, int tiles_n, int &n, unsigned &expect) {
+    const int n0 = em0 / hw;
+    if (second && !(n0 + 1 < n_img && (unsigned)em0 + TM > (unsigned)(n0 + 1) * (unsigned)hw)) return false;
+    n = n0 + second;
+    expect = gn_tiles_of_sample<TM>(n, hw, tiles_n);
+    return true;
+}
+template <typename T, int TM>
+__device__ __forceinline__ void conv_gn_finalise_listed(const ConvParams<T> &p, const int *fin, int n_fin, int tid) {
+    hive_gn::finalise_listed<8>(p.gn_partial, p.Cout, p.fold, TM, p.Ho * p.Wo, fin, n_fin, tid);
+}
+
+template <typename T, int TM>
+__device__ __forceinline__ void conv_gn_fold_tile(const ConvParams<T> &p, int em0, int tiles_n, unsigned char *scr, int tid) {
+    asm volatile("s_waitcnt vmcnt(0)" ::: "memory");
+    int *fin = reinterpret_cast<int *>(scr);
+    const int hw = p.Ho * p.Wo, n_img = p.M / hw;
+    const int n_fin = hive_gn::arrive_all(p.fold.count, 2, tid, 512, fin, [&](int k, int &n, unsigned &expect) { return gn_tile_contrib<TM>(em0, k, hw, n_img, tiles_n, n, expect); });
+    conv_gn_finalise_listed<T, TM>(p, fin, n_fin, tid);
+}
+
+template <typename T, int TM>
+__device__ __forceinline__ void conv_gn_fold_tail(const ConvParams<T> &p, int run0, int run_n, int per_xcd, int tiles_n, unsigned char *scr, int tid) {
+    int *fin = reinterpret_cast<int *>(scr);
+    const int hw = p.Ho * p.Wo, n_img = p.M / hw, tl0 = blockIdx.x >> 3;
+    const int my_tiles = (run_n - tl0 + per_xcd - 1) / per_xcd;
+    const int n_fin = hive_gn::arrive_all(p.fold.count, 2 * my_tiles, tid, 512, fin, [&](int k, int &n, unsigned &expect) {
+        const int em0 = ((run0 + tl0 + (k >> 1) * per_xcd) / tiles_n) * TM;
+        return gn_tile_contrib<TM>(em0, k & 1, hw, n_img, tiles_n, n, expect);
+    });
+    conv_gn_finalise_listed<T, TM>(p, fin, n_fin, tid);
+}
 
 
 template <typename T, int TM, int TN, int GN>
@@ -323,13 +365,14 @@
                 float a = 0.f;
 #pragma unroll
                 for (int w = 0; w < WM; ++w) a += reinterpret_cast<const float *>(lds + 2 * STAGE_BYTES + (w * WN + cw) * 4096)[hq * 64 + c];
-                p.gn_partial[((size_t)tile_m * 4 + hq) * p.Cout + en0 + ch] = a;
+                hive_gn::store_partial(p.gn_partial + ((size_t)tile_m * 4 + hq) * p.Cout + en0 + ch, a, p.fold.count != nullptr);
             }
         }
         if (!has_next) break;
         tl += per_xcd;
     }
     asm volatile("s_waitcnt vmcnt(0)" ::: "memory");
+    if (GN == 1 && p.fold.count) conv_gn_fold_tail<T, TM>(p, run0, run_n, per_xcd, tiles_n, lds + 2 * STAGE_BYTES, tid);
 }
 
 template <typename T, int TN, int GN, int NST>
@@ -464,8 +507,9 @@
                     float a = 0.f;
 #pragma unroll
                     for (int w = 0; w < WM; ++w) a += reinterpret_cast<const float *>(epi + (w * WN + cw) * 4096)[hq * 64 + c];
-                    p.gn_partial[((size_t)tile_m * 4 + hq) * p.Cout + en0 + ch] = a;
+                    hive_gn::store_partial(p.gn_partial + ((size_t)tile_m * 4 + hq) * p.Cout + en0 + ch, a, p.fold.count != nullptr);
                 }
+                if (p.fold.count) conv_gn_fold_tile<T, TM>(p, em0, tiles_n, epi, tid);
             }
         }
         if (!has_next) break;
@@ -510,6 +554,9 @@
     const float *gn_stats = nullptr;
     const void *gn_gamma = nullptr, *gn_beta = nullptr;
     int gn_G = 0, gn_cpg = 0;
+    int fold_G = 0;
+    float fold_eps = 0.f;
+    float *fold_stats = nullptr;
 };
 
 template <typename T>
@@ -571,6 +618,15 @@
         p.gn_partial = (float *)d_gn_partial;
         *gn_tile_rows = tm;
     }
+    auto fold_setup = [&]() -> int {
+        if (!(p.gn_partial && gn_mode && gn_mode->fold_G > 0 && gn_mode->fold_stats && C_out % gn_mode->fold_G == 0 && N <= HIVE_FOLD_COUNTERS && hive_finalize_fold_enabled()))
+            return HIVE_OK;
+        p.fold.stats = gn_mode->fold_stats;
+        p.fold.G = gn_mode->fold_G;
+        p.fold.eps = gn_mode->fold_eps;
+        *gn_tile_rows |= HIVE_GN_FOLDED;
+        return hive_fold_counters(ctx, &p.fold.count);
+    };
     {
         const long long tiles128 = (long long)((p.M + 127) / 128) * (C_out / 128);
         const char *deep_env = getenv("HIVE_CONV_DEEP");
@@ -595,6 +651,7 @@
                              gn_partial_floats, (long long)((p.M + 127) / 128) * 4 * C_out);
                 p.gn_partial = (float *)d_gn_partial;
                 *gn_tile_rows = 128;
+                if ((rc = fold_setup())) return rc;
             }
             const long long items = tiles128 * p.split_k;
             const dim3 dgrid((unsigned)std::min<long long>((items + 7) / 8 * 8, (long long)ctx->num_cus / 8 * 8));
@@ -606,6 +663,7 @@
             return HIVE_OK;
         }
     }
+    if ((rc = fold_setup())) return rc;
     const long long tiles = (long long)((p.M + tm - 1) / tm) * (C_out / tn);
     const dim3 grid((unsigned)std::min<long long>((tiles + 7) / 8 * 8, (long long)ctx->num_cus / 8 * 8));
     const size_t lds = (size_t)conv_lds(tm, tn);
@@ -674,6 +732,26 @@
                        d_residual2, d_out, d_out_relu, d_gn_partial, gn_partial_floats, gn_tile_rows);
 }
 
+extern "C" int64_t hive_nhwc_conv_gn_fold_floats(int N, int G) { return ((int64_t)2 * N * G + 63) / 64 * 64; }
+
+extern "C" int hive_nhwc_conv_gn_fold(hive_ctx *ctx, const void *d_x, int dtype, int N, int H, int W, int C_in, int C_out, int kernel, int stride, int pad_top,
+                                      int pad_left, int H_out, int W_out, const void *d_w, const void *d_bias, int relu, const void *d_residual,
+                                      const void *d_residual2, void *d_out, void *d_out_relu, void *d_gn_partial, int64_t gn_partial_floats, int *gn_tile_rows, int G,
+                                      float eps) {
+    HIVE_ENTER(ctx);
+    if (!ctx) return hive_fail(nullptr, HIVE_ERR_INVALID, "ctx is NULL");
+    HIVE_REQUIRE(ctx, d_gn_partial && gn_tile_rows && G > 0, "nhwc_conv_gn_fold: NULL argument / no groups");
+    GnMode mode;
+    const int64_t base = hive_nhwc_conv_gn_partial_floats((int64_t)N * H_out * W_out, C_out);
+    if (gn_partial_floats >= base + hive_nhwc_conv_gn_fold_floats(N, G)) {
+        mode.fold_G = G;
+        mode.fold_eps = eps;
+        mode.fold_stats = (float *)d_gn_partial + base;
+    }
+    return launch_conv(ctx, "nhwc_conv_gn_fold", d_x, dtype, N, H, W, C_in, C_out, kernel, stride, pad_top, pad_left, H_out, W_out, d_w, d_bias, relu, d_residual,
+                       d_residual2, d_out, d_out_relu, d_gn_partial, std::min(gn_partial_floats, base), gn_tile_rows, &mode);
+}
+
 extern "C" int hive_nhwc_conv_gn_apply(hive_ctx *ctx, const void *d_x, int dtype, int N, int H, int W, int C_in, int C_out, int kernel, int stride,
                                        int pad_top, int pad_left, int H_out, int W_out, const void *d_w, int G, const void *d_gamma, const void *d_beta,
                                        float eps, const void *d_residual, int relu, void *d_out, void *d_scratch, int64_t scratch_floats, int *fused) {
@@ -689,14 +767,20 @@
     float *partial = (float *)d_scratch, *stats = partial + partial_floats;
     GnMode mode;
     mode.stats_only = 1;
+    mode.fold_G = G;
+    mode.fold_eps = eps;
+    mode.fold_stats = stats;
     int tile_rows = 0;
     int rc = launch_conv(ctx, "nhwc_conv_gn_apply", d_x, dtype, N, H, W, C_in, C_out, kernel, stride, pad_top, pad_left, H_out, W_out, d_w, nullptr, 0, nullptr,
                          nullptr, d_out, nullptr, partial, partial_floats, &tile_rows, &mode);
     if (rc) return rc;
     HIVE_REQUIRE(ctx, tile_rows > 0, "nhwc_conv_gn_apply: no statistics from a %lld-pixel map", hw);
-    rc = hive_gn_finalize_tiles(ctx, partial, N, (int)hw, C_out, G, tile_rows, eps, stats);
-    if (rc) return rc;
+    if (tile_rows & HIVE_GN_FOLDED)
+        tile_rows &= ~HIVE_GN_FOLDED;
+    else if ((rc = hive_gn_finalize_tiles(ctx, partial, N, (int)hw, C_out, G, tile_rows, eps, stats)))
+        return rc;
     mode.stats_only = 0;
+    mode.fold_G = 0;
     mode.gn_stats = stats;
     mode.gn_gamma = d_gamma;
     mode.gn_beta = d_beta;
diff --git a/hive_amd/csrc/dpt_net.hip b/hive_amd/csrc/dpt_net.hip
--- a/hive_amd/csrc/dpt_net.hip
+++ b/hive_amd/csrc/dpt_net.hip
@@ -172,15 +172,15 @@
         }
         *out = Map{d->alloc((size_t)B * oh * ow * cout), oh, ow, cout};
         if (out_relu) *out_relu = Map{want_relu_copy ? d->alloc((size_t)B * oh * ow * cout) : nullptr, oh, ow, cout};
-        const int64_t gn_floats = gn_stats ? hive_nhwc_conv_gn_partial_floats((int64_t)B * oh * ow, cout) : 0;
+        const int64_t gn_floats = gn_stats ? hive_nhwc_conv_gn_partial_floats((int64_t)B * oh * ow, cout) + hive_nhwc_conv_gn_fold_floats(B, 32) : 0;
         if (gn_stats) out->gn = (float *)d->alloc((size_t)gn_floats * 2);
         if (dry) return HIVE_OK;
         const void *wp, *bp = nullptr;
         DPT_TRY(need(wname, &wp));
         if (bias_name) DPT_TRY(need(bias_name, &bp));
         if (gn_stats)
-            return hive_nhwc_conv_gn(ctx, x.p, dt, B, x.H, x.W, x.C, cout, k, stride, pt, pl, oh, ow, wp, bp, relu, res1, res2, out->p,
-                                     out_relu ? out_relu->p : nullptr, out->gn, gn_floats, &out->gn_tm);
+            return hive_nhwc_conv_gn_fold(ctx, x.p, dt, B, x.H, x.W, x.C, cout, k, stride, pt, pl, oh, ow, wp, bp, relu, res1, res2, out->p,
+                                          out_relu ? out_relu->p : nullptr, out->gn, gn_floats, &out->gn_tm, 32, d->cfg.gn_eps);
         return hive_nhwc_conv(ctx, x.p, dt, B, x.H, x.W, x.C, cout, k, stride, pt, pl, oh, ow, wp, bp, relu, res1, res2, out->p,
                               out_relu ? out_relu->p : nullptr);
     };
@@ -238,13 +238,13 @@
     auto hybrid_backbone = [&]() -> int {
         half_t *xin = d->alloc((size_t)B * H * W * 3);
         Map s0{d->alloc((size_t)B * same_out(H, 2) * same_out(W, 2) * 64), same_out(H, 2), same_out(W, 2), 64};
-        const int64_t stem_floats = hive_nhwc_conv_gn_partial_floats((int64_t)B * s0.H * s0.W, 64);
+        const int64_t stem_floats = hive_nhwc_conv_gn_partial_floats((int64_t)B * s0.H * s0.W, 64) + hive_nhwc_conv_gn_fold_floats(B, 32);
         s0.gn = (float *)d->alloc((size_t)stem_floats * 2);
         if (!dry) {
             DPT_TRY(preprocess(xin));
             const void *sw;
             DPT_TRY(need(bb + "stem.conv.weight", &sw));
-            DPT_TRY(hive_resnet_stem_conv_gn(ctx, xin, dt, B, H, W, sw, s0.p, s0.gn, stem_floats, &s0.gn_tm));
+            DPT_TRY(hive_resnet_stem_conv_gn_fold(ctx, xin, dt, B, H, W, sw, s0.p, s0.gn, stem_floats, &s0.gn_tm, 32, d->cfg.gn_eps));
         }
         d->release(xin);
         Map feat{d->alloc((size_t)B * same_out(s0.H, 2) * same_out(s0.W, 2) * 64), same_out(s0.H, 2), same_out(s0.W, 2), 64};
@@ -267,7 +267,7 @@
                 int bneck = 0;
                 if (mid == 64 && stride == 1 && (long long)t.H * t.W >= 256) {
                     t2 = Map{d->alloc((size_t)B * t.H * t.W * 64), t.H, t.W, 64};
-                    const int64_t floats = hive_nhwc_conv_gn_partial_floats((int64_t)B * t.H * t.W, 64);
+                    const int64_t floats = hive_nhwc_conv_gn_partial_floats((int64_t)B * t.H * t.W, 64) + hive_nhwc_conv_gn_fold_floats(B, 32);
                     t2.gn = (float *)d->alloc((size_t)floats * 2);
                     if (dry) {
                         bneck = 1;
diff --git a/hive_amd/csrc/dpt_ops.hip b/hive_amd/csrc/dpt_ops.hip
--- a/hive_amd/csrc/dpt_ops.hip
+++ b/hive_amd/csrc/dpt_ops.hip
@@ -1,4 +1,5 @@
 #include "hive_internal.hpp"
+#include "gn_finalize.hpp"
 
 #include <algorithm>
 #include <cstdlib>
@@ -118,34 +119,17 @@
     __shared__ double red[8];
     const int i = blockIdx.x;
     if (i >= total) return;
-    const int n = i / G, g = i % G, cpg = C / G;
-    const long long r0 = (long long)n * HW, r1 = r0 + HW - 1;
-    const int t0 = (int)(r0 / TM), nt = (int)(r1 / TM) - t0 + 1;
-    double s = 0.0, q = 0.0;
-    for (int e = threadIdx.x; e < nt * cpg; e += 256) {
-        const int t = t0 + e / cpg, c = e % cpg;
-        const int h = ((long long)t * TM) / HW == n ? 0 : 1;
-        const float *ps = partial + (((size_t)t * 2 + h) * 2) * C + g * cpg + c;
-        s += (double)ps[0];
-        q += (double)ps[C];
-    }
-    for (int off = 32; off > 0; off >>= 1) {
-        s += __shfl_xor(s, off);
-        q += __shfl_xor(q, off);
-    }
+    double s, q;
+    hive_gn::tiles_thread_sums(partial, C, G, TM, HW, i / G, i % G, threadIdx.x, s, q);
+    hive_gn::wave_butterfly(s, q);
     if ((threadIdx.x & 63) == 0) {
         red[threadIdx.x >> 6] = s;
         red[4 + (threadIdx.x >> 6)] = q;
     }
     __syncthreads();
     if (threadIdx.x == 0) {
-        s = ((red[0] + red[1]) + red[2]) + red[3];
-        q = ((red[4] + red[5]) + red[6]) + red[7];
-        const double cnt = (double)HW * cpg;
-        const double mean = s / cnt;
-        const double var = fmax(q / cnt - mean * mean, 0.0);
-        stats[2 * i] = (float)mean;
-        stats[2 * i + 1] = (float)(1.0 / sqrt(var + (double)eps));
+        const double ws[4] = {red[0], red[1], red[2], red[3]}, wq[4] = {red[4], red[5], red[6], red[7]};
+        hive_gn::write_stats(ws, wq, HW, C / G, eps, stats, i);
     }
 }
 
@@ -473,6 +457,7 @@
     HIVE_REQUIRE(ctx, N > 0 && HW > 0 && C >= 8 && C <= 2048 && pow2(C) && G > 0 && C % G == 0,
                  "group_norm: need C a power of two in [8, 2048] and C %% G == 0 (N=%d HW=%d C=%d G=%d)", N, HW, C, G);
     HIVE_REQUIRE(ctx, dtype == HIVE_BF16 || dtype == HIVE_F16, "group_norm: dtype must be HIVE_F16 or HIVE_BF16");
+    const float *folded = d_gn_partial ? hive_gn_folded_stats(d_gn_partial, &gn_tile_rows, (int64_t)N * HW, C) : nullptr;
     const bool from_tiles = d_gn_partial && gn_tile_rows > 0;
     HIVE_REQUIRE(ctx, !from_tiles || gn_tile_rows <= HW, "group_norm_stats: tiles of %d rows on samples of %d", gn_tile_rows, HW);
     const int VC = C / 8, PP = 256 / VC;
@@ -480,21 +465,23 @@
     const size_t partial_floats = from_tiles ? 0 : (size_t)N * slabs * 2 * C, stats_floats = (size_t)N * G * 2;
     int rc = hive_reserve_device(ctx, &ctx->d_scratch, &ctx->scratch_bytes, (partial_floats + stats_floats) * sizeof(float));
     if (rc) return rc;
-    float *partial = (float *)ctx->d_scratch, *stats = partial + partial_floats;
+    float *partial = (float *)ctx->d_scratch;
+    float *own_stats = partial + partial_floats;
+    const float *stats = folded ? folded : own_stats;
     const dim3 g1(slabs, N), g3(std::max(1, std::min((HW + PP - 1) / PP, (ctx->num_cus * 8 + N - 1) / N)), N);
-    if (from_tiles)
-        hipLaunchKernelGGL(gn_finalize_tiles_kernel, dim3(N * G), dim3(256), 0, ctx->stream, (const float *)d_gn_partial, C, G, gn_tile_rows, HW, eps, stats, N * G);
+    if (from_tiles && !folded)
+        hipLaunchKernelGGL(gn_finalize_tiles_kernel, dim3(N * G), dim3(256), 0, ctx->stream, (const float *)d_gn_partial, C, G, gn_tile_rows, HW, eps, own_stats, N * G);
     if (dtype == HIVE_BF16) {
         if (!from_tiles) {
             hipLaunchKernelGGL(gn_partial_kernel<bf16>, g1, dim3(256), 0, ctx->stream, (const bf16 *)d_x, HW, C, slabs, partial);
-            hipLaunchKernelGGL(gn_finalize_kernel, dim3(N * G), dim3(256), 0, ctx->stream, partial, C, G, slabs, HW, eps, stats, N * G);
+            hipLaunchKernelGGL(gn_finalize_kernel, dim3(N * G), dim3(256), 0, ctx->stream, partial, C, G, slabs, HW, eps, own_stats, N * G);
         }
         hipLaunchKernelGGL(gn_apply_kernel<bf16>, g3, dim3(256), 0, ctx->stream, (const bf16 *)d_x, (const bf16 *)d_gamma, (const bf16 *)d_beta,
                            stats, (const bf16 *)d_residual, (bf16 *)d_out, HW, C, G, relu);
     } else {
         if (!from_tiles) {
             hipLaunchKernelGGL(gn_partial_kernel<_Float16>, g1, dim3(256), 0, ctx->stream, (const _Float16 *)d_x, HW, C, slabs, partial);
-            hipLaunchKernelGGL(gn_finalize_kernel, dim3(N * G), dim3(256), 0, ctx->stream, partial, C, G, slabs, HW, eps, stats, N * G);
+            hipLaunchKernelGGL(gn_finalize_kernel, dim3(N * G), dim3(256), 0, ctx->stream, partial, C, G, slabs, HW, eps, own_stats, N * G);
         }
         hipLaunchKernelGGL(gn_apply_kernel<_Float16>, g3, dim3(256), 0, ctx->stream, (const _Float16 *)d_x, (const _Float16 *)d_gamma,
                            (const _Float16 *)d_beta, stats, (const _Float16 *)d_residual, (_Float16 *)d_out, HW, C, G, relu);
@@ -526,6 +513,7 @@
                  "group_norm_relu_maxpool: need C a power of two in [8, 2048], C %% G == 0, N <= 65535 (N=%d H=%d W=%d C=%d G=%d)", N, H, W, C, G);
     HIVE_REQUIRE(ctx, dtype == HIVE_BF16 || dtype == HIVE_F16, "group_norm_relu_maxpool: dtype must be HIVE_F16 or HIVE_BF16");
     const int HW = H * W;
+    const float *folded = d_gn_partial ? hive_gn_folded_stats(d_gn_partial, &gn_tile_rows, (int64_t)N * HW, C) : nullptr;
     const bool from_tiles = d_gn_partial && gn_tile_rows > 0;
     HIVE_REQUIRE(ctx, !from_tiles || gn_tile_rows <= HW, "group_norm_relu_maxpool: tiles of %d rows on samples of %d", gn_tile_rows, HW);
     const int VC = C / 8, PP = 256 / VC;
@@ -533,24 +521,25 @@
     const size_t partial_floats = from_tiles ? 0 : (size_t)N * slabs * 2 * C, stats_floats = (size_t)N * G * 2;
     int rc = hive_reserve_device(ctx, &ctx->d_scratch, &ctx->scratch_bytes, (partial_floats + stats_floats) * sizeof(float));
     if (rc) return rc;
-    float *partial = (float *)ctx->d_scratch, *stats = partial + partial_floats;
+    float *partial = (float *)ctx->d_scratch, *own_stats = partial + partial_floats;
+    const float *stats = folded ? folded : own_stats;
     const int Ho = (H + 1) / 2, Wo = (W + 1) / 2;
     const int pad_t = std::max((Ho - 1) * 2 + 3 - H, 0) / 2, pad_l = std::max((Wo - 1) * 2 + 3 - W, 0) / 2;
     const long long per_img = (long long)Ho * Wo * VC;
     const dim3 g1(slabs, N), gp((unsigned)std::max<long long>(1, std::min<long long>((per_img + 255) / 256, ((long long)ctx->num_cus * 32 + N - 1) / N)), N);
-    if (from_tiles)
-        hipLaunchKernelGGL(gn_finalize_tiles_kernel, dim3(N * G), dim3(256), 0, ctx->stream, (const float *)d_gn_partial, C, G, gn_tile_rows, HW, eps, stats, N * G);
+    if (from_tiles && !folded)
+        hipLaunchKernelGGL(gn_finalize_tiles_kernel, dim3(N * G), dim3(256), 0, ctx->stream, (const float *)d_gn_partial, C, G, gn_tile_rows, HW, eps, own_stats, N * G);
     if (dtype == HIVE_BF16) {
         if (!from_tiles) {
             hipLaunchKernelGGL(gn_partial_kernel<bf16>, g1, dim3(256), 0, ctx->stream, (const bf16 *)d_x, HW, C, slabs, partial);
-            hipLaunchKernelGGL(gn_finalize_kernel, dim3(N * G), dim3(256), 0, ctx->stream, partial, C, G, slabs, HW, eps, stats, N * G);
+            hipLaunchKernelGGL(gn_finalize_kernel, dim3(N * G), dim3(256), 0, ctx->stream, partial, C, G, slabs, HW, eps, own_stats, N * G);
         }
         hipLaunchKernelGGL(gn_relu_maxpool_kernel<bf16>, gp, dim3(256), 0, ctx->stream, (const bf16 *)d_x, (const bf16 *)d_gamma, (const bf16 *)d_beta, stats,
                            (bf16 *)d_out, H, W, C, G, Ho, Wo, pad_t, pad_l);
     } else {
         if (!from_tiles) {
             hipLaunchKernelGGL(gn_partial_kernel<_Float16>, g1, dim3(256), 0, ctx->stream, (const _Float16 *)d_x, HW, C, slabs, partial);
-            hipLaunchKernelGGL(gn_finalize_kernel, dim3(N * G), dim3(256), 0, ctx->stream, partial, C, G, slabs, HW, eps, stats, N * G);
+            hipLaunchKernelGGL(gn_finalize_kernel, dim3(N * G), dim3(256), 0, ctx->stream, partial, C, G, slabs, HW, eps, own_stats, N * G);
         }
         hipLaunchKernelGGL(gn_relu_maxpool_kernel<_Float16>, gp, dim3(256), 0, ctx->stream, (const _Float16 *)d_x, (const _Float16 *)d_gamma,
                            (const _Float16 *)d_beta, stats, (_Float16 *)d_out, H, W, C, G, Ho, Wo, pad_t, pad_l);
diff --git a/hive_amd/csrc/gn_finalize.hpp b/hive_amd/csrc/gn_finalize.hpp
--- /dev/null
+++ b/hive_amd/csrc/gn_finalize.hpp
@@ -0,0 +1,123 @@
+#pragma once
+#include <hip/hip_runtime.h>
+
+namespace hive_gn {
+
+constexpr int COUNTER_STRIDE = 64;
+
+struct Fold {
+    float *stats;
+    unsigned *count;
+    int G;
+    float eps;
+};
+
+__device__ __forceinline__ const float *tiles_element(const float *partial, int C, int cpg, int TM, int HW, int n, int g, int e) {
+    const long long r0 = (long long)n * HW;
+    const int t = (int)(r0 / TM) + e / cpg, c = e % cpg;
+    const int h = (long long)t * TM >= r0 ? 0 : 1;
+    return partial + (((size_t)t * 2 + h) * 2) * C + g * cpg + c;
+}
+__device__ __forceinline__ int tiles_elements(int cpg, int TM, int HW, int n) {
+    const long long r0 = (long long)n * HW, r1 = r0 + HW - 1;
+    return ((int)(r1 / TM) - (int)(r0 / TM) + 1) * cpg;
+}
+
+__device__ __forceinline__ void tiles_thread_sums(const float *partial, int C, int G, int TM, int HW, int n, int g, int vt, double &s, double &q) {
+    const int cpg = C / G, cnt = tiles_elements(cpg, TM, HW, n);
+    s = 0.0, q = 0.0;
+    for (int e = vt; e < cnt; e += 256) {
+        const float *ps = tiles_element(partial, C, cpg, TM, HW, n, g, e);
+        s += (double)ps[0];
+        q += (double)ps[C];
+    }
+}
+
+__device__ __forceinline__ void wave_butterfly(double &s, double &q) {
+    for (int off = 32; off > 0; off >>= 1) {
+        s += __shfl_xor(s, off);
+        q += __shfl_xor(q, off);
+    }
+}
+
+__device__ __forceinline__ void write_stats(const double (&ws)[4], const double (&wq)[4], int HW, int cpg, float eps, float *stats, int i) {
+#pragma clang fp contract(off)
+    const double s = ((ws[0] + ws[1]) + ws[2]) + ws[3];
+    const double q = ((wq[0] + wq[1]) + wq[2]) + wq[3];
+    const double cnt = (double)HW * cpg;
+    const double mean = s / cnt;
+    const double msq = mean * mean;
+    const double var = fmax(q / cnt - msq, 0.0);
+    stats[2 * i] = (float)mean;
+    stats[2 * i + 1] = (float)(1.0 / sqrt(var + (double)eps));
+}
+
+template <int NU>
+__device__ __forceinline__ void tiles_units_on_wave(const float *partial, int C, int G, int TM, int HW, float eps, float *stats, int n, int g0, int gs, int lane) {
+    const int cpg = C / G, cnt = tiles_elements(cpg, TM, HW, n);
+    double ws[NU][4], wq[NU][4];
+#pragma unroll
+    for (int u = 0; u < NU; ++u)
+#pragma unroll
+        for (int vw = 0; vw < 4; ++vw) ws[u][vw] = 0.0, wq[u][vw] = 0.0;
+    for (int e0 = 0; e0 < cnt; e0 += 256) {
+        float ls[NU][4], lq[NU][4];
+#pragma unroll
+        for (int u = 0; u < NU; ++u)
+#pragma unroll
+            for (int vw = 0; vw < 4; ++vw) {
+                const int e = e0 + vw * 64 + lane, g = g0 + u * gs;
+                ls[u][vw] = lq[u][vw] = 0.f;
+                if (e < cnt && g < G) {
+                    const float *ps = tiles_element(partial, C, cpg, TM, HW, n, g, e);
+                    ls[u][vw] = __hip_atomic_load(ps, __ATOMIC_RELAXED, __HIP_MEMORY_SCOPE_AGENT);
+                    lq[u][vw] = __hip_atomic_load(ps + C, __ATOMIC_RELAXED, __HIP_MEMORY_SCOPE_AGENT);
+                }
+            }
+#pragma unroll
+        for (int u = 0; u < NU; ++u)
+#pragma unroll
+            for (int vw = 0; vw < 4; ++vw)
+                if (e0 + vw * 64 + lane < cnt) ws[u][vw] += (double)ls[u][vw], wq[u][vw] += (double)lq[u][vw];
+    }
+#pragma unroll
+    for (int u = 0; u < NU; ++u) {
+#pragma unroll
+        for (int vw = 0; vw < 4; ++vw) wave_butterfly(ws[u][vw], wq[u][vw]);
+        if (lane == 0 && g0 + u * gs < G) write_stats(ws[u], wq[u], HW, cpg, eps, stats, n * G + g0 + u * gs);
+    }
+}
+template <int NW>
+__device__ __forceinline__ void finalise_listed(const float *partial, int C, const Fold &f, int TM, int HW, const int *fin, int n_fin, int tid) {
+    const int lane = tid & 63, wave = tid >> 6;
+    for (int k = 1; k <= n_fin; ++k)
+        for (int g0 = wave; g0 < f.G; g0 += 4 * NW) tiles_units_on_wave<4>(partial, C, f.G, TM, HW, f.eps, f.stats, fin[k], g0, NW, lane);
+}
+
+template <typename F>
+__device__ __forceinline__ int arrive_all(unsigned *count, int n_arr, int tid, int nthreads, int *fin, F &&contrib) {
+    __syncthreads();
+    if (tid == 0) fin[0] = 0;
+    __syncthreads();
+    for (int k = tid; k < n_arr; k += nthreads) {
+        int n;
+        unsigned expect;
+        if (!contrib(k, n, expect)) continue;
+        unsigned *cn = count + (size_t)n * COUNTER_STRIDE;
+        const unsigned before = __hip_atomic_fetch_add(cn, 1u, __ATOMIC_RELAXED, __HIP_MEMORY_SCOPE_AGENT);
+        if (before + 1 == expect) {
+            __hip_atomic_store(cn, 0u, __ATOMIC_RELAXED, __HIP_MEMORY_SCOPE_AGENT);
+            fin[1 + __hip_atomic_fetch_add(fin, 1, __ATOMIC_RELAXED, __HIP_MEMORY_SCOPE_WORKGROUP)] = n;
+        }
+    }
+    __syncthreads();
+    return fin[0];
+}
+__device__ __forceinline__ void store_partial(float *p, float v, bool write_through) {
+    if (write_through)
+        __hip_atomic_store(p, v, __ATOMIC_RELAXED, __HIP_MEMORY_SCOPE_AGENT);
+    else
+        *p = v;
+}
+
+}
diff --git a/hive_amd/csrc/hive_internal.hpp b/hive_amd/csrc/hive_internal.hpp
--- a/hive_amd/csrc/hive_internal.hpp
+++ b/hive_amd/csrc/hive_internal.hpp
@@ -47,6 +47,7 @@
     void *d_splitk = nullptr;
     size_t splitk_bytes = 0;
     unsigned *d_splitk_count = nullptr;
+    unsigned *d_fold_count = nullptr;
     void *d_gram = nullptr;
     size_t gram_bytes = 0;
 
@@ -101,6 +102,16 @@
 int hive_reserve_device(hive_ctx *ctx, void **ptr, size_t *cur, size_t bytes);
 int hive_upload(hive_ctx *ctx, void *dst, const void *src, size_t bytes);
 int hive_gn_finalize_tiles(hive_ctx *ctx, const float *d_partial, int N, int HW, int C, int G, int tile_rows, float eps, float *d_stats);
+constexpr int HIVE_GN_FOLDED = 1 << 30;
+constexpr int HIVE_FOLD_COUNTERS = 4096;
+constexpr int HIVE_FOLD_COUNTER_STRIDE = 64;
+bool hive_finalize_fold_enabled();
+int hive_fold_counters(hive_ctx *ctx, unsigned **count);
+inline const float *hive_gn_folded_stats(const void *d_gn_partial, int *gn_tile_rows, int64_t n_px, int C) {
+    if (!(*gn_tile_rows & HIVE_GN_FOLDED)) return nullptr;
+    *gn_tile_rows &= ~HIVE_GN_FOLDED;
+    return (const float *)d_gn_partial + hive_nhwc_conv_gn_partial_floats(n_px, C);
+}
 constexpr int HIVE_SPLITK_TILES = 4096;
 int hive_splitk_workspace(hive_ctx *ctx, size_t bytes, void **ws, unsigned **count);
 int hive_gram_gn_stats(hive_ctx *ctx, const void *d_x, int dtype, int N, int H, int W, int C_in, int C_out, int stride, int Ho, int Wo, int G, const float *d_tables,
diff --git a/hive_amd/csrc/stem.hip b/hive_amd/csrc/stem.hip
--- a/hive_amd/csrc/stem.hip
+++ b/hive_amd/csrc/stem.hip
@@ -2,6 +2,7 @@
 
 #include <algorithm>
 
+#include "gn_finalize.hpp"
 #include "mfma_pipe.hpp"
 
 using hive_mfma::f32x4;
@@ -27,6 +28,7 @@
     int tiles_x, tiles_y, n_tiles;
     int run;
     float *gn_partial;
+    hive_gn::Fold fold;
 };
 
 __device__ __forceinline__ float stem_dot2(vec<__bf16, 2> a, vec<__bf16, 2> b, float c) { return __builtin_amdgcn_fdot2_f32_bf16(a, b, c, false); }
@@ -92,8 +94,8 @@
         if (tid < 128) {
             const int which = tid >> 6, c = tid & 63;
             const float a = ((wsum[0][which][c] + wsum[1][which][c]) + wsum[2][which][c]) + wsum[3][which][c];
-            p.gn_partial[((size_t)run_idx * 4 + which) * 64 + c] = a;
-            p.gn_partial[((size_t)run_idx * 4 + 2 + which) * 64 + c] = 0.f;
+            hive_gn::store_partial(p.gn_partial + ((size_t)run_idx * 4 + which) * 64 + c, a, p.fold.count != nullptr);
+            hive_gn::store_partial(p.gn_partial + ((size_t)run_idx * 4 + 2 + which) * 64 + c, 0.f, p.fold.count != nullptr);
         }
     };
     const int n_runs = p.n_tiles / p.run;
@@ -201,6 +203,18 @@
         __syncthreads();
         flush_sums(pending);
     }
+    if (p.fold.count) {
+        asm volatile("s_waitcnt vmcnt(0)" ::: "memory");
+        int *fin = reinterpret_cast<int *>(wsum);
+        const int runs_per_img = per_img / p.run;
+        const int my_runs = (n_runs - (int)blockIdx.x + (int)gridDim.x - 1) / (int)gridDim.x;
+        const int n_fin = hive_gn::arrive_all(p.fold.count, my_runs, tid, 256, fin, [&](int k, int &n, unsigned &expect) {
+            n = (blockIdx.x + k * gridDim.x) / runs_per_img;
+            expect = (unsigned)runs_per_img;
+            return true;
+        });
+        hive_gn::finalise_listed<4>(p.gn_partial, 64, p.fold, ST_TH * ST_TW * p.run, p.Ho * p.Wo, fin, n_fin, tid);
+    }
 }
 
 template <typename T>
@@ -235,7 +249,7 @@
 
 template <typename T>
 int launch_stem(hive_ctx *ctx, const void *d_x, int N, int H, int W, const void *d_w, void *d_out, float *d_gn_partial, long long gn_partial_floats,
-                int *gn_tile_rows) {
+                int *gn_tile_rows, int G, float eps) {
     StemParams<T> p{};
     p.x = (const T *)d_x;
     p.w = (const T *)d_w;
@@ -259,6 +273,15 @@
                      tiles / p.run * 4 * 64);
         p.gn_partial = d_gn_partial;
         *gn_tile_rows = ST_TH * ST_TW * p.run;
+        const long long base = hive_nhwc_conv_gn_partial_floats((int64_t)N * p.Ho * p.Wo, 64);
+        if (G > 0 && 64 % G == 0 && gn_partial_floats >= base + hive_nhwc_conv_gn_fold_floats(N, G) && N <= 511 && hive_finalize_fold_enabled()) {
+            int rc = hive_fold_counters(ctx, &p.fold.count);
+            if (rc) return rc;
+            p.fold.stats = d_gn_partial + base;
+            p.fold.G = G;
+            p.fold.eps = eps;
+            *gn_tile_rows |= HIVE_GN_FOLDED;
+        }
     }
     const unsigned grid = (unsigned)std::min<long long>(tiles / p.run, (long long)ctx->num_cus * 3);
     hipLaunchKernelGGL(stem_conv_kernel<T>, dim3(grid), dim3(256), 0, ctx->stream, p);
@@ -271,12 +294,12 @@
 extern "C" {
 
 static int stem_entry(hive_ctx *ctx, const void *d_x, int dtype, int N, int H, int W, const void *d_w, void *d_out, void *d_gn_partial, int64_t gn_partial_floats,
-                      int *gn_tile_rows) {
+                      int *gn_tile_rows, int G = 0, float eps = 0.f) {
     HIVE_REQUIRE(ctx, d_x && d_w && d_out, "resnet_stem_conv: NULL argument");
     HIVE_REQUIRE(ctx, dtype == HIVE_BF16 || dtype == HIVE_F16, "resnet_stem_conv: dtype must be HIVE_F16 or HIVE_BF16");
     HIVE_REQUIRE(ctx, N > 0 && H >= 7 && W >= 7 && (long long)N * H * W < (1ll << 31), "resnet_stem_conv: bad sizes %d x %d x %d", N, H, W);
-    return dtype == HIVE_BF16 ? launch_stem<__bf16>(ctx, d_x, N, H, W, d_w, d_out, (float *)d_gn_partial, gn_partial_floats, gn_tile_rows)
-                              : launch_stem<_Float16>(ctx, d_x, N, H, W, d_w, d_out, (float *)d_gn_partial, gn_partial_floats, gn_tile_rows);
+    return dtype == HIVE_BF16 ? launch_stem<__bf16>(ctx, d_x, N, H, W, d_w, d_out, (float *)d_gn_partial, gn_partial_floats, gn_tile_rows, G, eps)
+                              : launch_stem<_Float16>(ctx, d_x, N, H, W, d_w, d_out, (float *)d_gn_partial, gn_partial_floats, gn_tile_rows, G, eps);
 }
 
 int hive_resnet_stem_conv(hive_ctx *ctx, const void *d_x, int dtype, int N, int H, int W, const void *d_w, void *d_out) {
@@ -291,6 +314,14 @@
     if (!ctx) return hive_fail(nullptr, HIVE_ERR_INVALID, "ctx is NULL");
     HIVE_REQUIRE(ctx, d_gn_partial && gn_tile_rows, "resnet_stem_conv_gn: NULL argument");
     return stem_entry(ctx, d_x, dtype, N, H, W, d_w, d_out, d_gn_partial, gn_partial_floats, gn_tile_rows);
+}
+
+int hive_resnet_stem_conv_gn_fold(hive_ctx *ctx, const void *d_x, int dtype, int N, int H, int W, const void *d_w, void *d_out, void *d_gn_partial,
+                                  int64_t gn_partial_floats, int *gn_tile_rows, int G, float eps) {
+    HIVE_ENTER(ctx);
+    if (!ctx) return hive_fail(nullptr, HIVE_ERR_INVALID, "ctx is NULL");
+    HIVE_REQUIRE(ctx, d_gn_partial && gn_tile_rows && G > 0, "resnet_stem_conv_gn_fold: NULL argument / no groups");
+    return stem_entry(ctx, d_x, dtype, N, H, W, d_w, d_out, d_gn_partial, gn_partial_floats, gn_tile_rows, G, eps);
 }
 
 int hive_nhwc_maxpool3x3s2(hive_ctx *ctx, const void *d_x, int dtype, int N, int H, int W, int C, void *d_out) {
diff --git a/hive_amd/dpt/ops.py b/hive_amd/dpt/ops.py
--- a/hive_amd/dpt/ops.py
+++ b/hive_amd/dpt/ops.py
@@ -134,7 +134,7 @@
         not_covered(what, why)
 
 
-def conv2d(x, conv, weight=None, same_pad=False, relu=False, residual=None, residual2=None, also_relu=False, with_bias=True, gn_stats=False):
+def conv2d(x, conv, weight=None, same_pad=False, relu=False, residual=None, residual2=None, also_relu=False, with_bias=True, gn_stats=False, gn_fold=None):
     n, _, ih, iw = x.shape
     k, st, pt, pl, oh, ow = conv_geometry(conv, ih, iw, same_pad)
     w = weight if weight is not None else _conv3x3_weight(conv)
@@ -148,11 +148,18 @@
     ctx = _lib.default_context(x.device.index or 0)
     if gn_stats:
         import ctypes
-        partial = torch.empty(int(ctx.lib.hive_nhwc_conv_gn_partial_floats(n * oh * ow, conv.out_channels)), dtype=torch.float32, device=x.device)
+        floats = int(ctx.lib.hive_nhwc_conv_gn_partial_floats(n * oh * ow, conv.out_channels))
+        if gn_fold is not None:
+            floats += int(ctx.lib.hive_nhwc_conv_gn_fold_floats(n, int(gn_fold[0])))
+        partial = torch.empty(floats, dtype=torch.float32, device=x.device)
         tile_rows = ctypes.c_int(0)
-        ctx.check(ctx.lib.hive_nhwc_conv_gn(ctx.handle, x.data_ptr(), _code(x.dtype), n, ih, iw, conv.in_channels, conv.out_channels, k, st, pt, pl, oh, ow,
-                                            w.data_ptr(), _lib.ptr(bias), int(bool(relu)), _lib.ptr(residual), _lib.ptr(residual2), out.data_ptr(),
-                                            _lib.ptr(out_relu), partial.data_ptr(), partial.numel(), ctypes.byref(tile_rows)))
+        args = (ctx.handle, x.data_ptr(), _code(x.dtype), n, ih, iw, conv.in_channels, conv.out_channels, k, st, pt, pl, oh, ow,
+                w.data_ptr(), _lib.ptr(bias), int(bool(relu)), _lib.ptr(residual), _lib.ptr(residual2), out.data_ptr(),
+                _lib.ptr(out_relu), partial.data_ptr(), partial.numel(), ctypes.byref(tile_rows))
+        if gn_fold is not None:
+            ctx.check(ctx.lib.hive_nhwc_conv_gn_fold(*args, int(gn_fold[0]), float(gn_fold[1])))
+        else:
+            ctx.check(ctx.lib.hive_nhwc_conv_gn(*args))
         out.hive_gn_stats = (partial, tile_rows.value)
     else:
         ctx.check(ctx.lib.hive_nhwc_conv(ctx.handle, x.data_ptr(), _code(x.dtype), n, ih, iw, conv.in_channels, conv.out_channels, k, st, pt, pl, oh, ow,
@@ -257,7 +264,7 @@
             and conv.bias is None and x.shape[2] >= 7 and x.shape[3] >= 7)
 
 
-def stem_conv(x, conv, weight):
+def stem_conv(x, conv, weight, gn_fold=None):
     stamp = (weight.data_ptr(), weight._version, weight.dtype)
     cache = _module_cache(conv)
     hit = cache.get("stem")
@@ -270,16 +277,22 @@
     out = torch.empty((n, 64, oh, ow), dtype=x.dtype, device=x.device, memory_format=torch.channels_last)
     ctx = _lib.default_context(x.device.index or 0)
     import ctypes
-    partial = torch.empty(int(ctx.lib.hive_nhwc_conv_gn_partial_floats(n * oh * ow, 64)), dtype=torch.float32, device=x.device)
+    floats = int(ctx.lib.hive_nhwc_conv_gn_partial_floats(n * oh * ow, 64))
+    if gn_fold is not None:
+        floats += int(ctx.lib.hive_nhwc_conv_gn_fold_floats(n, int(gn_fold[0])))
+    partial = torch.empty(floats, dtype=torch.float32, device=x.device)
     tile_rows = ctypes.c_int(0)
-    ctx.check(ctx.lib.hive_resnet_stem_conv_gn(ctx.handle, x.data_ptr(), _code(x.dtype), n, h, w_, hit[1].data_ptr(), out.data_ptr(), partial.data_ptr(),
-                                               partial.numel(), ctypes.byref(tile_rows)))
+    args = (ctx.handle, x.data_ptr(), _code(x.dtype), n, h, w_, hit[1].data_ptr(), out.data_ptr(), partial.data_ptr(), partial.numel(), ctypes.byref(tile_rows))
+    if gn_fold is not None:
+        ctx.check(ctx.lib.hive_resnet_stem_conv_gn_fold(*args, int(gn_fold[0]), float(gn_fold[1])))
+    else:
+        ctx.check(ctx.lib.hive_resnet_stem_conv_gn(*args))
     if tile_rows.value:
         out.hive_gn_stats = (partial, tile_rows.value)
     return out
 
 
-def bneck_gn_conv3x3(t, norm, conv, weight):
+def bneck_gn_conv3x3(t, norm, conv, weight, gn_fold=False):
     import ctypes
     stats = getattr(t, "hive_gn_stats", None)
     if (stats is None or _why_not_map(t) or t.shape[1] != 64 or conv.in_channels != 64 or conv.out_channels != 64 or tuple(conv.kernel_size) != (3, 3)
@@ -289,7 +302,8 @@
     n, c, h, wd = t.shape
     out = torch.empty_like(t)
     ctx = _lib.default_context(t.device.index or 0)
-    partial = torch.empty(int(ctx.lib.hive_nhwc_conv_gn_partial_floats(n * h * wd, 64)), dtype=torch.float32, device=t.device)
+    floats = int(ctx.lib.hive_nhwc_conv_gn_partial_floats(n * h * wd, 64)) + (int(ctx.lib.hive_nhwc_conv_gn_fold_floats(n, 32)) if gn_fold else 0)
+    partial = torch.empty(floats, dtype=torch.float32, device=t.device)
     tile_rows, fused = ctypes.c_int(0), ctypes.c_int(0)
     ctx.check(ctx.lib.hive_bneck_gn_conv3x3(ctx.handle, t.data_ptr(), _code(t.dtype), n, h, wd, c, stats[0].data_ptr(), int(stats[1]), norm.weight.data_ptr(),
                                             norm.bias.data_ptr(), float(norm.eps), w.data_ptr(), out.data_ptr(), partial.data_ptr(), partial.numel(),
diff --git a/include/hive_mi355x.h b/include/hive_mi355x.h
--- a/include/hive_mi355x.h
+++ b/include/hive_mi355x.h
@@ -214,6 +214,11 @@
 int hive_nhwc_group_norm_stats(hive_ctx *ctx, const void *d_x, int dtype, int N, int HW, int C, int G, const void *d_gamma,
                                const void *d_beta, float eps, const void *d_residual, int relu, void *d_out,
                                const void *d_gn_partial, int gn_tile_rows);
+int64_t hive_nhwc_conv_gn_fold_floats(int N, int G);
+int hive_nhwc_conv_gn_fold(hive_ctx *ctx, const void *d_x, int dtype, int N, int H, int W, int C_in, int C_out, int kernel, int stride,
+                           int pad_top, int pad_left, int H_out, int W_out, const void *d_w, const void *d_bias, int relu,
+                           const void *d_residual, const void *d_residual2, void *d_out, void *d_out_relu, void *d_gn_partial,
+                           int64_t gn_partial_floats, int *gn_tile_rows, int G, float eps);
 
 int hive_nhwc_conv_gn_apply(hive_ctx *ctx, const void *d_x, int dtype, int N, int H, int W, int C_in, int C_out, int kernel,
                             int stride, int pad_top, int pad_left, int H_out, int W_out, const void *d_w, int G,
@@ -240,6 +245,8 @@
                           int64_t gn_partial_floats, int *gn_tile_rows, int *fused);
 int hive_resnet_stem_conv_gn(hive_ctx *ctx, const void *d_x, int dtype, int N, int H, int W, const void *d_w, void *d_out, void *d_gn_partial,
                              int64_t gn_partial_floats, int *gn_tile_rows);
+int hive_resnet_stem_conv_gn_fold(hive_ctx *ctx, const void *d_x, int dtype, int N, int H, int W, const void *d_w, void *d_out, void *d_gn_partial,
+                                  int64_t gn_partial_floats, int *gn_tile_rows, int G, float eps);
 int hive_nhwc_group_norm_relu_maxpool(hive_ctx *ctx, const void *d_x, int dtype, int N, int H, int W, int C, int G, const void *d_gamma,
                                       const void *d_beta, float eps, void *d_out, const void *d_gn_partial, int gn_tile_rows);
 
```

After: 1347 frames/s. -3.4%, worse.
